# leekwoon/nav-gym

Measured on AMD Instinct MI355X. Metric: env steps/sec (whole node), 4096 envs x 1081-beam lidar, higher is better.
Workload: dtype f32

## Files before the change

include/navsim.h:

```cpp
#ifndef NAVSIM_H
#define NAVSIM_H

#include <stddef.h>
#include <stdint.h>

#ifdef __cplusplus
extern "C" {
#endif

#define NAVSIM_ABI_VERSION 7

#define NAVSIM_OK            0
#define NAVSIM_E_ARG        -1
#define NAVSIM_E_LAUNCH     -2
#define NAVSIM_E_UNSUPPORTED -3
#define NAVSIM_E_NODEVICE   -4

#define NAVSIM_PED_NONE      0
#define NAVSIM_PED_EXTERNAL  1
#define NAVSIM_PED_SFM       2

#define NAVSIM_FIELD_F32     0
#define NAVSIM_FIELD_U16T    1
#define NAVSIM_FIELD_TILE    8
// ... 159 lines not shown
#define NAVSIM_COUNTER_REGEN_SHORT     6
#define NAVSIM_COUNTER_REGEN_LATE      7

#define NAVSIM_DRAWS_PER_ARENA      464
#define NAVSIM_DRAW_KIND            0
#define NAVSIM_DRAW_OBSTACLE_NUMBER 1
#define NAVSIM_DRAW_NUM_HUMANS      2
#define NAVSIM_DRAW_SCAN_NOISE_STD  3
#define NAVSIM_DRAW_OBSTACLE_WIDTH  4
#define NAVSIM_DRAW_CORRIDOR_WIDTH  5
#define NAVSIM_DRAW_ITERATIONS      6
#define NAVSIM_DRAW_MAP             8

typedef struct navsim_step_io {
    const double* action;
    const float*  obs_prev;
    float*   obs;
    float*   achieved_goal;
    float*   desired_goal;
    double*  reward;
    uint8_t* done;
    float*   is_success;
    float*   is_crash;
    double*  distance;
    float*   final_obs;
    float*   final_goals;
    const uint8_t* reset_mask;
    uint8_t* truncated;
} navsim_step_io;

int         navsim_abi_version(void);
const char* navsim_error_string(int code);
int         navsim_default_config(navsim_config* cfg);
const char* navsim_last_hip_error(void);

size_t navsim_build_dt_workspace_bytes(int32_t n_maps, int32_t map_h, int32_t map_w);
int    navsim_build_dt(const uint8_t* occ, int32_t n_maps, int32_t map_h, int32_t map_w,
                       float* field, void* workspace, size_t workspace_bytes, void* stream);

size_t navsim_field_bytes(int32_t n_maps, int32_t map_h, int32_t map_w, int32_t format);
int    navsim_build_field(const uint8_t* occ, int32_t n_maps, int32_t map_h, int32_t map_w, int32_t format,
                          void* field, float* overflow, int32_t* n_saturated,
                          void* workspace, size_t workspace_bytes, void* stream);

size_t navsim_rect_table_bytes(int32_t n_maps, int32_t map_h, int32_t map_w);
size_t navsim_rect_index_bytes(int32_t n_maps, int32_t map_h, int32_t map_w);
int    navsim_build_rect_index(const void* table, int32_t n_maps, int32_t map_h, int32_t map_w, void* index,
                               int32_t* n_rects, void* stream);
int    navsim_maps_closed(const uint8_t* occ, int32_t n_maps, int32_t map_h, int32_t map_w, int32_t* closed, void* stream);
int    navsim_world_closed(const navsim_config* cfg, const navsim_state* st, int32_t* n_open, void* stream);
size_t navsim_build_rects_workspace_bytes(int32_t n_maps, int32_t map_h, int32_t map_w);
int    navsim_build_rects(const uint8_t* occ, int32_t n_maps, int32_t map_h, int32_t map_w, const void* field,
                          int32_t format, const float* overflow, void* table, void* workspace, size_t workspace_bytes,
                          void* stream);

int navsim_cast_static(const float* field, int32_t n_envs, int32_t map_h, int32_t map_w,
                       const float* queries, int32_t n_per_env, float max_range, int32_t march_rule,
                       float* out, void* stream);

int navsim_render_polys(float* ranges, const double* angles, int32_t n_envs, int32_t n_beams,
                        const float* verts, const int32_t* n_verts, int32_t max_verts,
                        const float* origin, void* stream);

int navsim_render_legs(float* ranges, const double* angles, int32_t n_envs, int32_t n_beams,
                       const float* agents, const int32_t* n_agents, int32_t max_agents,
                       const float* origin, void* stream);

int navsim_integrate(double* pose, const double* cmd, double* vel_out, int32_t n,
                     double time_step, double axle_offset, void* stream);

int navsim_reward_done(const navsim_config* cfg, const void* obs, const void* goals,
                       int32_t obs_is_f64, int32_t n,
                       const float* scan_threshold, const float* scan_discomfort,
                       double* reward, uint8_t* done, float* is_success, float* is_crash,
                       double* distance, void* stream);

int navsim_scan_threshold(const navsim_config* cfg, const float* footprint, int32_t n_vert,
                          float* out, void* stream);

int navsim_beam_table(const navsim_config* cfg, double* table, void* stream);

int navsim_step(const navsim_config* cfg, const navsim_state* st, const navsim_step_io* io,
                void* stream);

#define NAVSIM_STEP_ALL     0
#define NAVSIM_STEP_NOT_DUE 1
#define NAVSIM_STEP_DUE     2
int navsim_step_part(const navsim_config* cfg, const navsim_state* st, const navsim_step_io* io, int32_t part,
                     void* stream);

int navsim_ped_scans(const navsim_config* cfg, const navsim_state* st, float* out, void* stream);
int navsim_ped_scans_part(const navsim_config* cfg, const navsim_state* st, float* out, int32_t e0, int32_t n_e, void* stream);

size_t navsim_regen_workspace_bytes(const navsim_config* cfg);
int    navsim_regen_swap(const navsim_config* cfg, const navsim_state* live, const navsim_state* stage,
                         const navsim_step_io* io, const float* stage_obs, const uint8_t* want, uint8_t* mark,
                         const long long* ready, void* stream);
int    navsim_regen_stage(const navsim_config* cfg, const navsim_state* stage, const navsim_step_io* io, uint8_t* want,
                          uint8_t* mark, long long* ready, void* workspace, size_t workspace_bytes, void* stream);
int    navsim_regen_stage_part(const navsim_config* cfg, const navsim_state* stage, const navsim_step_io* io, uint8_t* want,
                               uint8_t* mark, long long* ready, void* workspace, size_t workspace_bytes, int32_t part,
                               int32_t n_parts, void* stream);
int    navsim_step_install(const navsim_config* cfg, const navsim_state* st, const navsim_step_io* io,
                           const navsim_state* stage, const float* stage_obs, uint8_t* mark, const long long* ready,
                           uint8_t* late, void* stream);
int    navsim_step_install_replan(const navsim_config* cfg, const navsim_state* st, const navsim_step_io* io,
                                  const navsim_state* stage, const float* stage_obs, uint8_t* mark, const long long* ready,
                                  uint8_t* late, int32_t max_queries, void* stream);
int    navsim_step_install_next(const navsim_config* cfg, const navsim_state* st, const navsim_step_io* io,
                                const navsim_state* stage, const float* stage_obs, uint8_t* mark, const long long* ready,
                                uint8_t* late_next, const uint8_t* late_prev, int32_t max_queries, void* stream);
int    navsim_regen_helper(void* stream);
int    navsim_regen(const navsim_config* cfg, const navsim_state* st, const navsim_step_io* io,
                    void* workspace, size_t workspace_bytes, void* stream);

int navsim_costmap(const uint8_t* occ, int32_t n_maps, int32_t map_h, int32_t map_w, uint8_t* cost, void* stream);
int    navsim_plan(const uint8_t* cost, const int32_t* map_index, int32_t n_queries, int32_t cost_h, int32_t cost_w,
                   double cost_resolution, double origin_x, double origin_y, const double* start, const double* goal,
                   double interval, int32_t max_wp, double* wp, int32_t* n_wp, int32_t* path_cells, double* path_len,
                   void* stream);

size_t navsim_replan_workspace_bytes(const navsim_config* cfg, int32_t max_queries);
int    navsim_replan(const navsim_config* cfg, const navsim_state* st, int32_t max_queries, void* workspace,
                     size_t workspace_bytes, void* stream);

typedef struct navsim_policy_weights {
    const float* cv1_w;
    const float* cv1_b;
    const float* cv2_w;
    const float* cv2_b;
    const float* fc1_w;
    const float* fc1_b;
    const float* fc2_w;
    const float* fc2_b;
    const float* a1_w;
    const float* a1_b;
    const float* a2_w;
    const float* a2_b;
} navsim_policy_weights;

size_t navsim_ped_policy_workspace_bytes(const navsim_config* cfg);
int    navsim_ped_policy(const navsim_config* cfg, const navsim_state* st, const navsim_policy_weights* w,
                         const float* ped_scans, float* prev_actions, double* ped_cmd, void* workspace,
                         size_t workspace_bytes, void* stream);
int    navsim_ped_policy_part(const navsim_config* cfg, const navsim_state* st, const navsim_policy_weights* w,
                              const float* ped_scans, float* prev_actions, double* ped_cmd, void* workspace,
                              size_t workspace_bytes, int32_t e0, int32_t n_e, void* stream);
int    navsim_ped_scan_policy(const navsim_config* cfg, const navsim_state* st, const navsim_policy_weights* w,
                              float* scans_out, float* prev_actions, double* ped_cmd, void* workspace,
                              size_t workspace_bytes, void* stream);

int navsim_launch_order(const uint32_t* cost, int32_t* order, int32_t n, void* stream);

typedef struct navsim_crowd_params {
    double time_step, discomfort_dist, map_size_m, map_resolution;
    double success_reward, collision_penalty, discomfort_penalty_factor, rotation_penalty_factor, timeout_penalty;
    double time_limit;
} navsim_crowd_params;
#define NAVSIM_CROWD_NOTHING 0
#define NAVSIM_CROWD_TIMEOUT 1
#define NAVSIM_CROWD_REACH_GOAL 2
#define NAVSIM_CROWD_COLLISION 3
#define NAVSIM_CROWD_COLLISION_OTHER 4
#define NAVSIM_CROWD_DANGER 5
int navsim_crowd_check(const navsim_crowd_params* p, int32_t n_envs, int32_t max_agents, int32_t grid,
                       const uint8_t* free_map, const double* robot, const double* agents, const int32_t* n_agents,
                       const double* global_time, double* reward, uint8_t* done, int32_t* info, double* min_dist,
                       void* stream);

#define NAVSIM_CROWD_MAX_VERTS 8
typedef struct navsim_crowd_map_params {
    double angular_min, angular_max;
    double angular_max_range;
    int32_t angular_dim;
    int32_t normalize;
    double map_size_m, map_resolution, submap_size_m;
} navsim_crowd_map_params;
int navsim_crowd_angular_map(const navsim_crowd_map_params* p, int32_t n_envs, int32_t max_obst, int32_t n_vert,
                             const double* robot, const double* verts, const int32_t* n_obst, double* out, void* stream);
int navsim_crowd_local_map(const navsim_crowd_map_params* p, int32_t n_envs, int32_t grid, const uint8_t* free_map,
                           const double* robot, int32_t rotate, uint8_t* out, void* stream);

#define NAVSIM_ORCA_MAX_AGENTS 64
#define NAVSIM_ORCA_MAX_EDGES  128
typedef struct navsim_orca_params {
    float time_step;
    float neighbor_dist;
    float time_horizon;
    float time_horizon_obst;
    int32_t max_neighbors;
} navsim_orca_params;
int navsim_crowd_orca(const navsim_orca_params* p, int32_t n_queries, int32_t max_agents, const double* agents,
                      const int32_t* n_agents, const double* pref_vel, int32_t max_obst, int32_t n_vert,
                      const double* verts, const int32_t* n_obst, const int32_t* obst_set, const double* theta,
                      double* out_vel, double* out_action, void* stream);
typedef struct navsim_ped_orca_params {
    navsim_orca_params orca;
    double ped_radius, robot_radius, safety_space;
    int32_t robot_visible;
} navsim_ped_orca_params;
int navsim_ped_orca(const navsim_config* cfg, const navsim_state* st, const navsim_ped_orca_params* p,
                    double* ped_cmd , void* stream);
int navsim_crowd_agent_step(double* pose, const double* action, double* vel, int32_t n, double time_step, void* stream);

int navsim_step_replan(const navsim_config* cfg, const navsim_state* st, const navsim_step_io* io, int32_t max_queries,
                       void* stream);

int navsim_prepare(const navsim_config* cfg, const navsim_state* st, const navsim_step_io* io);

int navsim_reset_obs(const navsim_config* cfg, const navsim_state* st, const navsim_step_io* io,
                     const uint8_t* mask, void* stream);

int navsim_restart(const navsim_config* cfg, const navsim_state* st, const uint8_t* mask, void* stream);

const char* navsim_step_kernel_name(void);

size_t navsim_sizeof_config(void);
size_t navsim_sizeof_state(void);
size_t navsim_sizeof_step_io(void);
int navsim_debug_math(int32_t fn, const double* x, const double* x2, double* out, int32_t n, void* stream);
int navsim_debug_xy_to_ij(const navsim_config* cfg, const double* xy, int32_t as_f32, int32_t* ij, int32_t n, void* stream);

int navsim_debug_spawn_decisions(const navsim_config* cfg, const uint8_t* cost, int32_t Hc, int32_t Wc, int32_t n,
                                 const int32_t* kind, const double* start, const double* goal, const double* robot,
                                 double* wp_scratch, int32_t* code, void* stream);

int navsim_debug_gather(const float* x, uint64_t n_words, int32_t mode, int32_t iters, int32_t n_threads,
                        float* out, void* stream);
int navsim_debug_set_stamps(unsigned long long* buf);
int navsim_debug_kernarg_layout(void* stream);

#ifdef __cplusplus
}
#endif
#endif
```

nav-gym_amd/csrc/kernels_step.hpp:

```cpp

struct StepShared {
    double rp[3];
    double old_rp[3];
    double act[2];
    float lx, ly, lth;
    int steps_now;
    double cT, sT;
    int i0, j0;
    int nseg, ndisc;
    int rescan;
    int respawn;
    float t1;
    float r_all;
    unsigned long long step_key;
    unsigned long long rescan_key;
    int next_chunk;
    int park_count, park_next;
    int pair_done;
    int term;
    double wave_ratio[kMaxWaves];
};
struct PedShared {
    double *ax, *ay, *avx, *avy;
    float (*seg)[4];
// ... 186 lines not shown
    (void)r_all; (void)res;
    if (culled) {
#ifndef NAVSIM_DIAG_NO_MERGE
        merge_prims_culled<BLOCK>(c, sh, pr, dir, rng_rw);
#endif
        __syncthreads();
    }
    for (int k = (int)threadIdx.x; k < B; k += BLOCK) {
        float rr = rng[k];
        if (!culled && (nseg | ndisc)) {
            float dx, dy;
            if (dir) { float2 d = dir[k]; dx = d.x; dy = d.y; }
            else beam_dir_k(c, tab, k, step, (double)sh.lth, sh.cT, sh.sT, dx, dy);
            for (int p = 0; p < nseg; ++p)
                nv::seg_merge(rr, lx, ly, dx, dy, pr.seg[p][0], pr.seg[p][1], pr.seg[p][2], pr.seg[p][3]);
            for (int p = 0; p < ndisc; ++p)
                nv::circle_merge(rr, lx, ly, dx, dy, pr.disc[p][0], pr.disc[p][1], nv::kLegRadius);
        }
        rr = rr < 0.0f ? 0.0f : rr;
        rr = rr > rmax ? rmax : rr;
        if (noise_std > 0.0f && rr != rmax)
            rr = rr + noise_std * nv::gauss_noise(nkey, (uint32_t)k);
        cr |= (rr < thr[k]);
        dc |= (rr < dthr[k]);
        obs_row[(size_t)(S - 1) * B + k] = rr;
        for (int j = 0; j < S - 1; ++j)
            if (S - 1 - j > n_hist) obs_row[(size_t)j * B + k] = rr;
    }
    crash = cr;
    discomfort = dc;
}

typedef unsigned long long lanemask_t;
__device__ __forceinline__ lanemask_t mask_of(bool p) { return __builtin_amdgcn_ballot_w64(p); }
__device__ __forceinline__ lanemask_t mask_ult(unsigned a, unsigned b) { return __builtin_amdgcn_uicmp(a, b, 36); }
__device__ __forceinline__ lanemask_t mask_eq(unsigned a, unsigned b) { return __builtin_amdgcn_uicmp(a, b, 32); }
__device__ __forceinline__ lanemask_t mask_flt(float a, float b) { return __builtin_amdgcn_fcmpf(a, b, 4); }
__device__ __forceinline__ float mask_sel(lanemask_t m, float a, float b) {
    float r;
    asm("v_cndmask_b32_e64 %0, %1, %2, %3" : "=v"(r) : "v"(b), "v"(a), "s"(m));
    return r;
}
__device__ __forceinline__ int mask_sel(lanemask_t m, int a, int b) {
    int r;
    asm("v_cndmask_b32_e64 %0, %1, %2, %3" : "=v"(r) : "v"(b), "v"(a), "s"(m));
    return r;
}
__device__ __forceinline__ bool mask_lane(lanemask_t m) { return mask_sel(m, 1, 0) != 0; }

template <typename Field, int RULE, int RECT>
__device__ __forceinline__ void probe_round(const Field& field, const char* __restrict__ rects, unsigned tpr,
                                            float x0, float y0, float dx, float dy, unsigned uW, unsigned uH,
                                            float max_range, float& t, lanemask_t& active, lanemask_t& hit) {
    typedef float f32x2 __attribute__((ext_vector_type(2)));
    const f32x2 org = {x0, y0}, dir = {dx, dy};
    f32x2 pos;
    if constexpr (RULE == NAVSIM_MARCH_F32_FMA) pos = __builtin_elementwise_fma(dir, (f32x2){t, t}, org);
    else pos = org + dir * t;
    int px = (int)pos.x, py = (int)pos.y;
    const lanemask_t live = (RECT == 2) ? active : (active & mask_ult((unsigned)px, uW) & mask_ult((unsigned)py, uH));
    lanemask_t occ;
    float d;
    if constexpr (RECT == 0) {
        px = mask_sel(live, px, 0);
        py = mask_sel(live, py, 0);
    }
    if constexpr (RECT != 0) {
        const unsigned cell = rect_cell(px, py);
        unsigned tile = __umul24((unsigned)py >> kRectShift, tpr) + ((unsigned)px >> kRectShift);
        if constexpr (RECT != 2) tile = (unsigned)mask_sel(live, (int)tile, 0);
        typedef unsigned u32x4 __attribute__((ext_vector_type(4)));
        u32x4 rec;
        lanemask_t inval;
        if constexpr (RECT == 2) {
            typedef __attribute__((address_space(3))) const unsigned char lds_u8;
            typedef unsigned u32x2 __attribute__((ext_vector_type(2)));
            typedef __attribute__((address_space(3))) const u32x2 lds_u2;
            lds_u8* row = (lds_u8*)rects;
            const unsigned ia = row[kRectListLen * 8 + tile * 2u], ib = row[kRectListLen * 8 + 1 + tile * 2u];
            const u32x2 ra = *(lds_u2*)(row + ia * 8u);
            const u32x2 rb = *(lds_u2*)(row + ib * 8u);
            rec.x = ra.x; rec.y = ra.y; rec.z = rb.x; rec.w = rb.y;
            inval = live & mask_eq(ia, 0xFFu);
        } else {
            const unsigned off = tile * (unsigned)sizeof(uint4);
            unsigned long long base;
            asm volatile("s_mov_b64 %1, %3\n\tglobal_load_dwordx4 %0, %2, %1\n\ts_waitcnt vmcnt(0)"
                         : "=&v"(rec), "=&s"(base) : "v"(off), "s"(rects) : "memory");
            inval = live & mask_eq(rec.x & 0xFFFFu, (unsigned)kRectInvalid);
        }
        const int da = rect_dist2(rec.x, rec.y, cell), db = rect_dist2(rec.z, rec.w, cell);
        const int d2 = da < db ? da : db;
        occ = live & mask_eq((unsigned)d2, 0u);
        d = Field::sqrt_d2(d2);
        if (inval != 0) {
            typename Field::raw_t raw = (typename Field::raw_t)1;
            if (mask_lane(inval)) raw = field.load(px, py);
            occ = (occ & ~inval) | (inval & mask_of(field.occupied(raw)));
            d = mask_sel(inval, field.decode_nz(raw, px, py), d);
        }
    } else {
        typename Field::raw_t raw = field.load(px, py);
        occ = live & mask_of(field.occupied(raw));
        d = field.decode_nz(raw, px, py);
    }
    hit |= occ;
    const float tn = t + march_step<RULE>(d);
    const lanemask_t go = live & ~occ;
    t = mask_sel(go, tn, t);
    active = go & mask_flt(tn, max_range);
}

constexpr int kIntRangeMaxSide = 1448;
__host__ __device__ __forceinline__ bool int_range_ok(int H, int W) { return H <= kIntRangeMaxSide && W <= kIntRangeMaxSide; }
__device__ __forceinline__ float hit_range_int(int ix, int iy) {
    return nv::sqrt_small_int((float)(__mul24(ix, ix) + __mul24(iy, iy)));
}
template <int RULE>
__device__ __forceinline__ float ray_result(lanemask_t hit, bool int_range, int i0, int j0, float x0, float y0, float dx, float dy,
                                            float t, float miss) {
    const int px = (int)march_pos<RULE>(x0, dx, t), py = (int)march_pos<RULE>(y0, dy, t);
    float r;
    if (int_range) {
        r = hit_range_int(px - i0, py - j0);
    } else {
        const float xd = (float)px - x0, yd = (float)py - y0;
        r = sqrtf(xd * xd + yd * yd);
    }
    return mask_sel(hit, r, miss);
}

#ifndef NAVSIM_PARK_LANES
#define NAVSIM_PARK_LANES 16
#endif
#ifndef NAVSIM_PAIR_SHARE_MIN_BLOCK
#define NAVSIM_PAIR_SHARE_MIN_BLOCK 512
#endif
constexpr int kParkLanesMax = NAVSIM_PARK_LANES;
#ifndef NAVSIM_PARK_LANES_PEDS
#define NAVSIM_PARK_LANES_PEDS 16
#endif
#ifdef NAVSIM_PARK_512
__host__ __device__ constexpr bool step_parks(int block, bool peds) { return (block == 256 && (!peds || NAVSIM_PARK_LANES_PEDS > 0)) || (block == 512 && !peds); }
#else
__host__ __device__ constexpr bool step_parks(int block, bool peds) { return block == 256 && (!peds || NAVSIM_PARK_LANES_PEDS > 0); }
#endif
__host__ __device__ inline size_t park_lds_bytes(int B, int park_lanes, bool peds) {
    return (((size_t)((B + 63) / 64) * park_lanes * (peds ? 2 : 16)) + 15) & ~(size_t)15;
}
__device__ __forceinline__ int lanes_below(lanemask_t m) {
    return (int)__builtin_amdgcn_mbcnt_hi((unsigned)(m >> 32), __builtin_amdgcn_mbcnt_lo((unsigned)m, 0u));
}

template <int BLOCK, typename Field, bool TO_LDS, int RULE, int RECT>
__device__ __forceinline__ void scan_beams_pred(const navsim_config& c, StepShared& sh,
                                                const Field& field, const uint4* __restrict__ rects,
                                                const double* __restrict__ tab,
                                                const Prims pr, float2* __restrict__ dir_lds, float* __restrict__ rng_lds,
                                                float4* __restrict__ park, const int park_lanes,
                                                const float* __restrict__ thr, const float* __restrict__ dthr,
                                                float* __restrict__ obs_row, int n_hist, float noise_std,
                                                uint64_t noise_key, uint64_t genv,
                                                int& crash, int& discomfort, bool prepare_prims = true) {
    const int B = c.n_beams, S = c.n_scan_stack, H = c.map_h, W = c.map_w;
    const float max_range = march_limit(H, W, c.range_max, c.resolution);
    const float res = (float)c.resolution;
    const float rmax = (float)c.range_max;
    const double step = nv::linspace_step(c);
    const int i0 = sh.i0, j0 = sh.j0;
    const float x0 = (float)i0, y0 = (float)j0;
    const bool int_range = int_range_ok(H, W);
    const float lx = sh.lx, ly = sh.ly;
    const int nseg = sh.nseg, ndisc = sh.ndisc;
    const unsigned uW = (unsigned)W, uH = (unsigned)H;
    const unsigned tpr = (unsigned)((W + 7) >> kRectShift);
    const float t1 = sh.t1, r_all = sh.r_all;
    const uint64_t nkey = (noise_std > 0.0f) ? nv::noise_stream(c.seed, genv, noise_key) : 0;
    int cr = 0, dc = 0;
    auto finish = [&](int k, float dx, float dy, float rr) {
        if (TO_LDS) {
            rng_lds[k] = rr * res;
            dir_lds[k] = make_float2(dx, dy);
            return;
        }
        rr = rr * res;
        for (int p = 0; p < nseg; ++p)
            nv::seg_merge(rr, lx, ly, dx, dy, pr.seg[p][0], pr.seg[p][1], pr.seg[p][2], pr.seg[p][3]);
        for (int p = 0; p < ndisc; ++p)
            nv::circle_merge(rr, lx, ly, dx, dy, pr.disc[p][0], pr.disc[p][1], nv::kLegRadius);
        rr = rr < 0.0f ? 0.0f : rr;
        rr = rr > rmax ? rmax : rr;
        if (noise_std > 0.0f && rr != rmax)
            rr = rr + noise_std * nv::gauss_noise(nkey, (uint32_t)k);
        cr |= (rr < thr[k]);
        dc |= (rr < dthr[k]);
        obs_row[(size_t)(S - 1) * B + k] = rr;
        for (int j = 0; j < S - 1; ++j)
            if (S - 1 - j > n_hist) obs_row[(size_t)j * B + k] = rr;
    };
    const float miss = (r_all >= 0.0f) ? r_all : max_range;
    if constexpr (TO_LDS) { if (prepare_prims) prims_prepare<BLOCK>(c, sh, pr); }
    constexpr bool kPark = step_parks(BLOCK, TO_LDS);
    int own_chunk = 0;
    const int lane = (int)threadIdx.x & 63;
    for (;;) {
        int chunk = 0;
        if (BLOCK > 64) {
            if (lane == 0) chunk = atomicAdd(&sh.next_chunk, 1);
            chunk = __builtin_amdgcn_readfirstlane(chunk);
        } else {
            chunk = own_chunk++;
        }
        if (chunk * 64 >= B) break;
        const int k = chunk * 64 + lane;
        const bool valid = k < B;
        float dx, dy;
        beam_dir_k(c, tab, valid ? k : B - 1, step, (double)sh.lth, sh.cT, sh.sT, dx, dy);
        float t = t1;
        lanemask_t active = mask_of(valid & (r_all < 0.0f));
        lanemask_t hit = 0;
        if constexpr (!kPark) {
            while (active != 0)
                probe_round<Field, RULE, RECT>(field, (const char*)rects, tpr, x0, y0, dx, dy, uW, uH, max_range, t, active, hit);
            if (valid) finish(k, dx, dy, ray_result<RULE>(hit, int_range, i0, j0, x0, y0, dx, dy, t, miss));
        } else {
            while ((int)__builtin_popcountll(active) > park_lanes)
                probe_round<Field, RULE, RECT>(field, (const char*)rects, tpr, x0, y0, dx, dy, uW, uH, max_range, t, active, hit);
            const bool marching = mask_lane(active);
            if (active != 0) {
                int base = 0;
                if (lane == 0) base = atomicAdd(&sh.park_count, (int)__builtin_popcountll(active));
                base = __builtin_amdgcn_readfirstlane(base);
                if (marching) {
                    if constexpr (TO_LDS) {
                        ((unsigned short*)park)[base + lanes_below(active)] = (unsigned short)k;
                        rng_lds[k] = t;
                        dir_lds[k] = make_float2(dx, dy);
                    } else {
                        park[base + lanes_below(active)] = make_float4(__int_as_float(k), t, dx, dy);
                    }
                }
            }
            if (valid & !marching) finish(k, dx, dy, ray_result<RULE>(hit, int_range, i0, j0, x0, y0, dx, dy, t, miss));
        }
    }
    if constexpr (kPark) __syncthreads();
    const int n_parked = kPark ? sh.park_count : 0;
    for (;;) {
        if (!kPark || n_parked == 0) break;
        int g = 0;
        if (lane == 0) g = atomicAdd(&sh.park_next, 64);
        g = __builtin_amdgcn_readfirstlane(g);
        if (g >= n_parked) break;
        const bool valid = g + lane < n_parked;
        int k;
        float t, dx, dy;
        if constexpr (TO_LDS) {
            k = (int)((const unsigned short*)park)[valid ? g + lane : g];
            t = rng_lds[k];
            const float2 d = dir_lds[k];
            dx = d.x; dy = d.y;
        } else {
            const float4 r = park[valid ? g + lane : g];
            k = __float_as_int(r.x);
            t = r.y; dx = r.z; dy = r.w;
        }
        lanemask_t active = mask_of(valid);
        lanemask_t hit = 0;
        while (active != 0)
            probe_round<Field, RULE, RECT>(field, (const char*)rects, tpr, x0, y0, dx, dy, uW, uH, max_range, t, active, hit);
        if (valid) finish(k, dx, dy, ray_result<RULE>(hit, int_range, i0, j0, x0, y0, dx, dy, t, miss));
    }
    if (TO_LDS) {
        __syncthreads();
        finish_beams<BLOCK>(c, sh, pr, tab, dir_lds, rng_lds, rng_lds, thr, dthr, obs_row, n_hist, noise_std,
                            noise_key, genv, cr, dc);
    }
    crash = cr;
    discomfort = dc;
}

__device__ __forceinline__ int ped_pop_waypoints(const double* wp, int head, int nw, const double (&pp)[3]) {
    while (head + 1 < nw) {
        double ddx = pp[0] - wp[2 * head], ddy = pp[1] - wp[2 * head + 1];
        if (sqrt(ddx * ddx + ddy * ddy) < 1.0) ++head;
        else break;
    }
    return head;
}
__device__ __forceinline__ void ped_pair_index(int t, int n, int& i, int& j) {
    const int n_pp = n * (n - 1) / 2;
    if (t < n_pp) {
        i = 0;
        int rem = t;
        while (rem >= n - 1 - i) { rem -= n - 1 - i; ++i; }
        j = i + 1 + rem;
    } else {
        i = t - n_pp; j = n;
    }
}
__device__ __forceinline__ void ped_pair_term(const navsim_config& c, const PedShared& ps, double2* pair, int n, int t) {
    int i, j;
    ped_pair_index(t, n, i, j);
    double fx, fy;
    sfm_pair(c, ps.ax[i], ps.ay[i], ps.avx[i], ps.avy[i], ps.ax[j], ps.ay[j], ps.avx[j], ps.avy[j], fx, fy);
    pair[t] = make_double2(fx, fy);
}
template <typename Field>
__device__ __forceinline__ void ped_sfm_step(const navsim_config& c, const Field& field, const PedShared& ps,
                                             const double2* pair, int n, int i, double vpref, const double* wp, double dt,
                                             double (&pp)[3], double (&pvel)[2]) {
    double ex = wp[0] - ps.ax[i], ey = wp[1] - ps.ay[i];
    double L = sqrt(ex * ex + ey * ey);
    if (L > 1e-9) { ex = ex / L; ey = ey / L; } else { ex = 0.0; ey = 0.0; }
    double fdx = (vpref * ex - ps.avx[i]) / c.sfm_tau;
    double fdy = (vpref * ey - ps.avy[i]) / c.sfm_tau;
    double fsx = 0.0, fsy = 0.0;
    {
        int slot = i - 1;
        for (int j = 0; j < i; ++j) {
            const double2 f = pair[slot];
            fsx -= f.x;
            fsy -= f.y;
            slot += n - 2 - j;
        }
        slot = i * (n - 1) - i * (i - 1) / 2;
        for (int j = i + 1; j < n; ++j, ++slot) {
            const double2 f = pair[slot];
            fsx += f.x;
            fsy += f.y;
        }
        const double2 f = pair[n * (n - 1) / 2 + i];
        fsx += f.x;
        fsy += f.y;
    }
    double fox = 0.0, foy = 0.0;
    {
        const int H = c.map_h, W = c.map_w;
        int ci, cj;
        nv::xy_to_ij(ps.ax[i], ps.ay[i], c, ci, cj);
        ci = ci > W - 1 ? W - 1 : ci;
        cj = cj > H - 1 ? H - 1 : cj;
        int il_ = ci > 0 ? ci - 1 : 0, ir = ci < W - 1 ? ci + 1 : W - 1;
        int jl = cj > 0 ? cj - 1 : 0, jr = cj < H - 1 ? cj + 1 : H - 1;
        double d = (double)field.at(ci, cj) * c.resolution;
        double gx = (double)field.at(ir, cj) - (double)field.at(il_, cj);
        double gy = (double)field.at(ci, jr) - (double)field.at(ci, jl);
        double gl = sqrt(gx * gx + gy * gy);
        if (gl > 0.0) {
            double mag = nv::exp_neg(-(d - c.sfm_agent_radius) / c.sfm_sigma_obstacle);
            fox = mag * (gx / gl);
            foy = mag * (gy / gl);
        }
    }
    double accx = c.sfm_k_desired * fdx + c.sfm_k_social * fsx + c.sfm_k_obstacle * fox;
    double accy = c.sfm_k_desired * fdy + c.sfm_k_social * fsy + c.sfm_k_obstacle * foy;
    double vx = ps.avx[i] + accx * dt;
    double vy = ps.avy[i] + accy * dt;
    double sp = sqrt(vx * vx + vy * vy);
    if (sp > vpref) {
        double k = (sp > 0.0) ? vpref / sp : 0.0;
        vx = vx * k; vy = vy * k;
    }
    pp[0] = pp[0] + vx * dt;
    pp[1] = pp[1] + vy * dt;
    double sp2 = sqrt(vx * vx + vy * vy);
    if (sp2 > 1e-6) pp[2] = nv::mod_2pi(nv::atan2_(vy, vx));
    pvel[0] = vx; pvel[1] = vy;
}
__device__ __forceinline__ bool ped_finish(const navsim_config& c, const navsim_state& st, int e, int i, size_t pq, double* wp,
                                           int head, int nw, double dt, uint64_t genv, uint64_t steps_now, const double (&pp)[3],
                                           const double (&pvel)[2]) {
    double ddx = pp[0] - wp[2 * (nw - 1)], ddy = pp[1] - wp[2 * (nw - 1) + 1];
    const bool at_final = sqrt(ddx * ddx + ddy * ddy) < 0.5;
    if (at_final && c.n_spawn > 0 && st.spawn_pose && !st.costmap) {
        uint64_t h = nv::hash4(c.seed, genv, (uint64_t)i + 1000, steps_now);
        for (int tries = 0; tries < c.n_spawn; ++tries) {
            int idx = (int)((h + (uint64_t)tries) % (uint64_t)c.n_spawn);
            const double* cand = st.spawn_pose + ((size_t)e * c.n_spawn + idx) * 3;
            double gx = cand[0] - pp[0], gy = cand[1] - pp[1];
            if (sqrt(gx * gx + gy * gy) > 10.0) {
                wp[0] = cand[0]; wp[1] = cand[1]; head = 0;
                st.ped_n_waypoints[pq] = 1;
                if (st.ped_goal) { st.ped_goal[pq * 2] = cand[0]; st.ped_goal[pq * 2 + 1] = cand[1]; }
                break;
            }
        }
    }
    st.ped_wp_head[pq] = head;
    double dist[3] = {st.ped_dist[pq * 3], st.ped_dist[pq * 3 + 1], st.ped_dist[pq * 3 + 2]};
    nv::leg_odometry(pp, pvel, st.ped_prev_yaw[pq], dt, dist);
    st.ped_dist[pq * 3] = dist[0]; st.ped_dist[pq * 3 + 1] = dist[1]; st.ped_dist[pq * 3 + 2] = dist[2];
    st.ped_prev_yaw[pq] = nv::wrap_pi(pp[2]);
    st.ped_pose[pq * 3] = pp[0]; st.ped_pose[pq * 3 + 1] = pp[1]; st.ped_pose[pq * 3 + 2] = pp[2];
    st.ped_vel[pq * 2] = pvel[0]; st.ped_vel[pq * 2 + 1] = pvel[1];
    return at_final;
}

__device__ __forceinline__ void wave_lds_sync() {
    __builtin_amdgcn_fence(__ATOMIC_RELEASE, "workgroup");
    __builtin_amdgcn_wave_barrier();
    __builtin_amdgcn_fence(__ATOMIC_ACQUIRE, "workgroup");
}

__device__ __forceinline__ int ped_stage_wave(const navsim_config& c, const navsim_state& st, int n, int lane, bool is_ped,
                                              size_t pq, const double* rp_t, double prev_v, const PedShared& ps,
                                              const double (&pp)[3], const double (&pvel)[2], int& nw) {
    const int P = c.max_waypoints;
    const double* wp = st.ped_waypoints + (pq * P) * 2;
    int head = 0;
    nw = 1;
    if (is_ped) {
        nw = st.ped_n_waypoints[pq];
        head = ped_pop_waypoints(wp, st.ped_wp_head[pq], nw, pp);
    }
    if (c.ped_model == NAVSIM_PED_SFM) {
        if (is_ped) { ps.ax[lane] = pp[0]; ps.ay[lane] = pp[1]; ps.avx[lane] = pvel[0]; ps.avy[lane] = pvel[1]; }
        if (lane == 0) {
            double s, cs;
            nv::sincos(rp_t[2], s, cs);
            ps.ax[n] = rp_t[0]; ps.ay[n] = rp_t[1];
            ps.avx[n] = prev_v * cs; ps.avy[n] = prev_v * s;
        }
    }
// ... 145 lines not shown
            if (w == 0ull) continue;
            if (pos++ == slot) { e_s = e; before_s = pos_p; break; }
            pos_p += __popcll(w);
        }
    __syncthreads();
    const int e = e_s;
    if (peds_before) *peds_before = before_s;
    if (n_peds) *n_peds = all_p;
    __syncthreads();
    return e;
}

template <int BLOCK>
__device__ __forceinline__ int due_arena_rank(const unsigned long long* __restrict__ due, int e, int* peds_before) {
    __shared__ int wave_a[kMaxWaves], wave_p[kMaxWaves];
    const int tid = threadIdx.x, lane = tid & 63, nthr = block_threads<BLOCK>();
    int n = 0, m = 0;
    for (int k = tid; k < e; k += nthr) { const unsigned long long w = due[k]; n += w != 0ull; m += __popcll(w); }
    for (int off = 32; off > 0; off >>= 1) { n += __shfl_down(n, off, 64); m += __shfl_down(m, off, 64); }
    if (lane == 0) { wave_a[tid >> 6] = n; wave_p[tid >> 6] = m; }
    __syncthreads();
    int rank = 0, before = 0;
    for (int w = 0; w < (nthr + 63) / 64; ++w) { rank += wave_a[w]; before += wave_p[w]; }
    *peds_before = before;
    __syncthreads();
    return rank;
}

#ifndef NAVSIM_INSTALL_UNROLL
#define NAVSIM_INSTALL_UNROLL 8
#endif
struct StepInstallBig { char* dst; const char* src; size_t bytes; };
struct StepInstall {
    navsim_state stage;
    const float* stage_obs;
    uint8_t* mark;
    const long long* ready;
    uint8_t* late_next;
    const uint8_t* late_prev;
    int lone;
    uint8_t* late;
    StepInstallBig big[5];
};
__device__ __forceinline__ void stage_request(int64_t* stage_episode, uint8_t* mark, int e, int64_t ep) {
    __hip_atomic_store(&stage_episode[e], ep, __ATOMIC_RELAXED, __HIP_MEMORY_SCOPE_AGENT);
    __threadfence();
    atomicOr((unsigned*)(mark + (e & ~3)), 1u << (8 * (e & 3)));
}
__device__ __forceinline__ long long stage_ready(const long long* ready, int e) {
    return __hip_atomic_load(&ready[e], __ATOMIC_ACQUIRE, __HIP_MEMORY_SCOPE_AGENT);
}
__device__ __forceinline__ void install_publish(const StepInstall& in, const navsim_state& live, int e) {
    __syncthreads();
    if (threadIdx.x == 0) {
        __threadfence();
        stage_request(in.stage.episode, in.mark, e, live.episode[e] + 1);
    }
}
template <int BLOCK>
__device__ __forceinline__ void install_arena(const navsim_config& c, const navsim_state& live, const navsim_step_io& io,
                                              const StepInstall& in, const int e, float* __restrict__ obs_row) {
    const int tid = threadIdx.x;
    const bool by_slot = live.map_slot && in.stage.map_slot;
    if (by_slot && tid == 0) {
        const int32_t a = live.map_slot[e], b = in.stage.map_slot[e];
        live.map_slot[e] = b; in.stage.map_slot[e] = a;
    }
    for (int k = 0; k < 5 && !by_slot; ++k) {
        if (!in.big[k].dst) continue;
        const size_t bytes = in.big[k].bytes;
        const char* src = in.big[k].src + (size_t)e * bytes;
        char* dst = in.big[k].dst + (size_t)e * bytes;
        if ((((size_t)(uintptr_t)src | (size_t)(uintptr_t)dst | bytes) & 15) == 0) {
            const size_t n16 = bytes / 16;
            size_t i = tid;
#ifndef NAVSIM_DIAG_INSTALL_NO_BIG
            constexpr int U = NAVSIM_INSTALL_UNROLL;
            for (; i + (U - 1) * BLOCK < n16; i += U * BLOCK) {
                typedef unsigned int u32x4 __attribute__((ext_vector_type(4)));
                u32x4 v[U];
#pragma unroll
                for (int u = 0; u < U; ++u) v[u] = __builtin_nontemporal_load((const u32x4*)src + i + u * BLOCK);
#pragma unroll
                for (int u = 0; u < U; ++u) ((u32x4*)dst)[i + u * BLOCK] = v[u];
            }
            for (; i < n16; i += BLOCK) ((uint4*)dst)[i] = ((const uint4*)src)[i];
#endif
        } else {
            for (size_t i = tid; i < bytes; i += BLOCK) dst[i] = src[i];
        }
    }
    const navsim_state& stage = in.stage;
    const int N = c.max_peds, K = c.n_spawn, P = c.max_waypoints, D = c.n_scan_stack * c.n_beams + NAVSIM_OBS_TAIL;
    const bool peds = c.ped_model != NAVSIM_PED_NONE;
#define NAVSIM_ROW_LOAD(name, dstp, srcp, cnt) \
    const size_t n_##name = ((dstp) && (srcp)) ? (size_t)(cnt) : 0; \
    auto v_##name = (srcp)[tid < (int)n_##name ? (size_t)e * n_##name + tid : 0];
#define NAVSIM_ROW_STORE(name, dstp, srcp) \
    if (tid < (int)n_##name) (dstp)[(size_t)e * n_##name + tid] = v_##name; \
    for (size_t i = (size_t)tid + BLOCK; i < n_##name; i += BLOCK) (dstp)[(size_t)e * n_##name + i] = (srcp)[(size_t)e * n_##name + i];
#define NAVSIM_ROW_SRC(p) ((p) ? (p) : (decltype(p))live.steps)
    NAVSIM_ROW_LOAD(noise, live.scan_noise_std, NAVSIM_ROW_SRC(stage.scan_noise_std), 1)
    NAVSIM_ROW_LOAD(pose, live.robot_pose, NAVSIM_ROW_SRC(stage.robot_pose), 3)
    NAVSIM_ROW_LOAD(goal, live.robot_goal, NAVSIM_ROW_SRC(stage.robot_goal), 2)
    NAVSIM_ROW_LOAD(pact, live.prev_action, NAVSIM_ROW_SRC(stage.prev_action), 2)
    NAVSIM_ROW_LOAD(ppose, live.prev_pose, NAVSIM_ROW_SRC(stage.prev_pose), 3)
    NAVSIM_ROW_LOAD(nhist, live.n_hist, NAVSIM_ROW_SRC(stage.n_hist), 1)
    NAVSIM_ROW_LOAD(steps, live.steps, NAVSIM_ROW_SRC(stage.steps), 1)
    NAVSIM_ROW_LOAD(spose, live.spawn_pose, NAVSIM_ROW_SRC(stage.spawn_pose), (size_t)K * 3)
    NAVSIM_ROW_LOAD(sgoal, live.spawn_goal, NAVSIM_ROW_SRC(stage.spawn_goal), (size_t)K * 2)
    NAVSIM_ROW_LOAD(npeds, peds ? live.n_peds : nullptr, NAVSIM_ROW_SRC(stage.n_peds), 1)
    NAVSIM_ROW_LOAD(ppos, peds ? live.ped_pose : nullptr, NAVSIM_ROW_SRC(stage.ped_pose), (size_t)N * 3)
    NAVSIM_ROW_LOAD(pvel, peds ? live.ped_vel : nullptr, NAVSIM_ROW_SRC(stage.ped_vel), (size_t)N * 2)
    NAVSIM_ROW_LOAD(pyaw, peds ? live.ped_prev_yaw : nullptr, NAVSIM_ROW_SRC(stage.ped_prev_yaw), N)
    NAVSIM_ROW_LOAD(pdist, peds ? live.ped_dist : nullptr, NAVSIM_ROW_SRC(stage.ped_dist), (size_t)N * 3)
    NAVSIM_ROW_LOAD(pvpref, peds ? (double*)live.ped_v_pref : nullptr, NAVSIM_ROW_SRC(stage.ped_v_pref), N)
    NAVSIM_ROW_LOAD(plegs, peds ? (uint8_t*)live.ped_has_legs : nullptr, NAVSIM_ROW_SRC(stage.ped_has_legs), N)
    NAVSIM_ROW_LOAD(pwp, peds ? live.ped_waypoints : nullptr, NAVSIM_ROW_SRC(stage.ped_waypoints), (size_t)N * P * 2)
    NAVSIM_ROW_LOAD(pnwp, peds ? live.ped_n_waypoints : nullptr, NAVSIM_ROW_SRC(stage.ped_n_waypoints), N)
    NAVSIM_ROW_LOAD(phead, peds ? live.ped_wp_head : nullptr, NAVSIM_ROW_SRC(stage.ped_wp_head), N)
    NAVSIM_ROW_LOAD(pgoal, peds ? live.ped_goal : nullptr, NAVSIM_ROW_SRC(stage.ped_goal), (size_t)N * 2)
    NAVSIM_ROW_LOAD(obs, obs_row - (size_t)e * D, in.stage_obs, D)
    NAVSIM_ROW_STORE(noise, live.scan_noise_std, stage.scan_noise_std)
    NAVSIM_ROW_STORE(pose, live.robot_pose, stage.robot_pose)
    NAVSIM_ROW_STORE(goal, live.robot_goal, stage.robot_goal)
    NAVSIM_ROW_STORE(pact, live.prev_action, stage.prev_action)
    NAVSIM_ROW_STORE(ppose, live.prev_pose, stage.prev_pose)
    NAVSIM_ROW_STORE(nhist, live.n_hist, stage.n_hist)
    NAVSIM_ROW_STORE(steps, live.steps, stage.steps)
    NAVSIM_ROW_STORE(spose, (double*)live.spawn_pose, stage.spawn_pose)
    NAVSIM_ROW_STORE(sgoal, (double*)live.spawn_goal, stage.spawn_goal)
    NAVSIM_ROW_STORE(npeds, live.n_peds, stage.n_peds)
    NAVSIM_ROW_STORE(ppos, live.ped_pose, stage.ped_pose)
    NAVSIM_ROW_STORE(pvel, live.ped_vel, stage.ped_vel)
    NAVSIM_ROW_STORE(pyaw, live.ped_prev_yaw, stage.ped_prev_yaw)
    NAVSIM_ROW_STORE(pdist, live.ped_dist, stage.ped_dist)
    NAVSIM_ROW_STORE(pvpref, (double*)live.ped_v_pref, stage.ped_v_pref)
    NAVSIM_ROW_STORE(plegs, (uint8_t*)live.ped_has_legs, stage.ped_has_legs)
    NAVSIM_ROW_STORE(pwp, live.ped_waypoints, stage.ped_waypoints)
    NAVSIM_ROW_STORE(pnwp, live.ped_n_waypoints, stage.ped_n_waypoints)
    NAVSIM_ROW_STORE(phead, live.ped_wp_head, stage.ped_wp_head)
    NAVSIM_ROW_STORE(pgoal, live.ped_goal, stage.ped_goal)
    NAVSIM_ROW_STORE(obs, obs_row - (size_t)e * D, in.stage_obs)
#undef NAVSIM_ROW_LOAD
#undef NAVSIM_ROW_STORE
#undef NAVSIM_ROW_SRC
    if (tid == 0) {
        if (io.achieved_goal) { io.achieved_goal[2 * e] = (float)stage.robot_pose[3 * (size_t)e]; io.achieved_goal[2 * e + 1] = (float)stage.robot_pose[3 * (size_t)e + 1]; }
        if (io.desired_goal) { io.desired_goal[2 * e] = (float)stage.robot_goal[2 * (size_t)e]; io.desired_goal[2 * e + 1] = (float)stage.robot_goal[2 * (size_t)e + 1]; }
        if (live.ped_due) live.ped_due[e] = 0ull;
    }
}

template <int BLOCK, bool PEDS, typename Field, int RULE, int RECT, bool PINL, bool INSTALL = false, bool FEAT = true>
__device__ __forceinline__ void step_arena(const navsim_config& c, const navsim_state& st, const navsim_step_io& io, const int e,
                                           int reset_only, const int peds_done, const uint8_t* __restrict__ reset_mask,
                                           unsigned dyn_lds_bytes, int park_lanes, unsigned rect_lds_offset,
                                           const StepInstall* in = nullptr, const int base_prio = 0) {
    __shared__ StepShared sh;
    extern __shared__ __attribute__((aligned(16))) char dyn_lds_all[];
    char* dyn_lds = dyn_lds_all + (RECT == 2 ? rect_lds_offset : 0u);
    PedShared ps = {};
    if constexpr (PEDS) ps = ped_lds_carve(dyn_lds + ((dyn_lds_bytes + 15u) & ~15u), c.max_peds);
    const Prims prims = {ps.seg, ps.disc, ps.info};
    const int tid = threadIdx.x;
    constexpr int kMarchPrio = (BLOCK == 256 && !PEDS) ? 2 : 0;
    __builtin_amdgcn_s_setprio(3);
    unsigned long long t_begin = 0;
    if (st.arena_cost && tid == 0) t_begin = __builtin_amdgcn_s_memrealtime();
    const int B = c.n_beams, S = c.n_scan_stack, N = c.max_peds, D = S * B + 7;
    const double dt = c.time_step;
    const uint64_t genv = (uint64_t)(c.env_index_base + e);
    const int ms = INSTALL ? map_slot_of(c, st, e) : (c.shared_field ? 0 : e);
    const Field field(st.field, st.field_overflow, ms, c.map_h, c.map_w);
    const uint4* rects = RECT ? (const uint4*)st.rect_table + (size_t)ms * rect_tiles_per_map(c.map_h, c.map_w)
                              : nullptr;
    if constexpr (RECT == 2) {
        const size_t row_bytes = rect_index_row_bytes(c.map_h, c.map_w);
        const uint4* src = (const uint4*)((const char*)st.rect_index + (size_t)ms * row_bytes);
        uint4* tab_lds = (uint4*)dyn_lds_all;
        for (int i = threadIdx.x; i < (int)(row_bytes / 16); i += BLOCK) tab_lds[i] = src[i];
        rects = tab_lds;
    }
    float* obs_row = io.obs + (size_t)e * D;
    const float* obs_prev = io.obs_prev ? io.obs_prev + (size_t)e * D : nullptr;
    double* rp_g = st.robot_pose + 3 * (size_t)e;
    double* goal_g = st.robot_goal + 2 * (size_t)e;
    double* pa_g = st.prev_action + 2 * (size_t)e;
    double* pv_g = st.prev_pose + 3 * (size_t)e;

    constexpr bool kFeat = PEDS || FEAT;
    const bool pending = kFeat && !reset_only && io.reset_mask && io.reset_mask[e] != 0;
    if (pending) {
        reset_only = 1;
        if (tid == 0) {
            io.reward[e] = 0.0; io.done[e] = 0; io.is_success[e] = 0.0f; io.is_crash[e] = 0.0f; io.distance[e] = 0.0;
            if (c.max_episode_steps > 0 && io.truncated) io.truncated[e] = 0;
            if (st.ped_due) st.ped_due[e] = 0ull;
        }
        if (c.defer_reset_scan) return;
        if constexpr (INSTALL && BLOCK >= 256 && RULE == NAVSIM_MARCH_F32) {
            if (in->lone && in->ready) {
                if (tid == 0) {
                    const bool lng = c.regen_min_steps <= 0 || st.done_steps[e] >= c.regen_min_steps;
                    const bool rdy = stage_ready(in->ready, e) == (long long)st.episode[e];
                    sh.respawn = lng ? (rdy ? 3 : 5) : 0;
                    if (!(lng && rdy)) stage_request(in->stage.episode, in->mark, e, st.episode[e] + 1);
                    if (st.counters) {
                        atomicAdd(&st.counters[lng ? (rdy ? NAVSIM_COUNTER_REGEN_SERVED : NAVSIM_COUNTER_REGEN_LATE) : NAVSIM_COUNTER_REGEN_SHORT], 1ull);
                        if (lng && !rdy) atomicAdd(&st.counters[NAVSIM_COUNTER_REGEN_SERVED], 1ull);
                    }
                }
                __syncthreads();
                const int verdict = sh.respawn;
                __syncthreads();
                if (verdict == 3) {
                    install_arena<BLOCK>(c, st, io, *in, e, obs_row);
                    install_publish(*in, st, e);
                    return;
                }
                if (verdict == 5) {
                    regen_lone<Field, BLOCK>(c, st, e);
                    if constexpr (RECT == 2) {
                        const size_t row_bytes = rect_index_row_bytes(c.map_h, c.map_w);
                        const uint4* src = (const uint4*)((const char*)st.rect_index + (size_t)ms * row_bytes);
                        uint4* tab_lds = (uint4*)dyn_lds_all;
                        for (int i = threadIdx.x; i < (int)(row_bytes / 16); i += BLOCK) tab_lds[i] = src[i];
                    }
                }
            }
        }
    }
    if (reset_only && reset_mask && !reset_mask[e]) {
        if (obs_prev && obs_prev != obs_row)
            for (int k = tid; k < D; k += BLOCK) obs_row[k] = obs_prev[k];
        return;
    }

    int n = (!PEDS || c.ped_model == NAVSIM_PED_NONE) ? 0 : st.n_peds[e];
    n = n > N ? N : n;
    const float noise_std = (c.add_scan_noise && st.scan_noise_std) ? st.scan_noise_std[e] : 0.0f;

    NAVSIM_STAMP(0);
    double pp[3] = {0.0, 0.0, 0.0};
    double pvel[2] = {0.0, 0.0};
    const bool is_ped = PEDS && tid < n;
    const size_t pq = (size_t)e * N + (is_ped ? tid : 0);
    const bool ped_advance = PEDS && PINL && !reset_only && !peds_done;
    int ped_head = 0, ped_nw = 1;
    if constexpr (PEDS) {
        if (tid < 64) {
            if (is_ped) {
                pp[0] = st.ped_pose[pq * 3]; pp[1] = st.ped_pose[pq * 3 + 1]; pp[2] = st.ped_pose[pq * 3 + 2];
                pvel[0] = st.ped_vel[pq * 2]; pvel[1] = st.ped_vel[pq * 2 + 1];
            }
            if constexpr (PINL) {
                if (ped_advance) ped_head = ped_stage_wave(c, st, n, tid, is_ped, pq, rp_g, pa_g[0], ps, pp, pvel, ped_nw);
            }
        }
    }
    constexpr int kPhase0Thread = (PEDS && BLOCK > 64) ? 64 : 0;
    const int l0 = tid - kPhase0Thread;
    if (l0 >= 0 && l0 < 3) {
        const double th_old = rp_g[2];
        double a0 = 0.0, a1 = 0.0;
        if (!reset_only) {
            a0 = io.action[2 * e]; a1 = io.action[2 * e + 1];
            if (c.action_kind == NAVSIM_ACTION_WHEELS) {
                const double wl = a0, wr = a1;
                a0 = c.wheel_radius * (wl + wr) * 0.5;
                a1 = c.wheel_radius * (wr - wl) / c.wheel_track;
            }
            if (c.clamp_action) {
                a0 = a0 < c.linvel_lo ? c.linvel_lo : (a0 > c.linvel_hi ? c.linvel_hi : a0);
                a1 = a1 < c.rotvel_lo ? c.rotvel_lo : (a1 > c.rotvel_hi ? c.rotvel_hi : a1);
            }
            if (c.min_turning_radius > 0.0) {
                double lim = fabs(a1) * c.min_turning_radius;
                if (a0 >= 0.0) a0 = (a0 > lim) ? a0 : lim;
                else           a0 = (a0 < -lim) ? a0 : -lim;
            }
        }
        const double th = th_old + a1 * dt;
        const double th_new = reset_only ? th_old : nv::mod_2pi(th);
        const float lth = (float)th_new;
        const double ang = (l0 == 0) ? th_old : ((l0 == 1) ? th : (double)lth);
        double sn, cs;
        nv::sincos(ang, sn, cs);
        const int w0 = kPhase0Thread & 63;
        const double s0 = __shfl(sn, w0), c0 = __shfl(cs, w0), s1 = __shfl(sn, w0 + 1), c1 = __shfl(cs, w0 + 1);
        const double sT = __shfl(sn, w0 + 2), cT = __shfl(cs, w0 + 2);
        if (l0 == 0) {
            sh.old_rp[0] = rp_g[0]; sh.old_rp[1] = rp_g[1]; sh.old_rp[2] = th_old;
            sh.nseg = 0; sh.ndisc = 0; sh.rescan = 0; sh.respawn = 0; sh.term = 0;
            if constexpr (INSTALL) {
                if (pending && !in->lone) {
                    if (in->late) in->late[e] = 0;
                    if (in->late_next) in->late_next[e] = 0;
                    if (in->late_prev && in->late_prev[e]) {
                        sh.respawn = 4;
                        stage_request(in->stage.episode, in->mark, e, st.episode[e] + 1);
                        if (st.counters) atomicAdd(&st.counters[NAVSIM_COUNTER_REGEN_LATE], 1ull);
                    } else if (in->ready) {
                        const bool lng = c.regen_min_steps <= 0 || st.done_steps[e] >= c.regen_min_steps;
                        const bool rdy = stage_ready(in->ready, e) == (long long)st.episode[e];
                        if (lng && rdy) sh.respawn = 3;
                        else {
                            if (lng && in->late) in->late[e] = 1;
                            stage_request(in->stage.episode, in->mark, e, st.episode[e] + 1);
                        }
                        if (st.counters)
                            atomicAdd(&st.counters[lng ? (rdy ? NAVSIM_COUNTER_REGEN_SERVED : NAVSIM_COUNTER_REGEN_LATE) : NAVSIM_COUNTER_REGEN_SHORT], 1ull);
                    }
                }
            }
            if (!reset_only) {
                const int64_t steps_now = st.steps[e] + 1;
                st.steps[e] = steps_now;
                sh.steps_now = (int)steps_now;
                sh.act[0] = a0; sh.act[1] = a1;
                double p[3] = {sh.old_rp[0], sh.old_rp[1], sh.old_rp[2]};
                nv::set_vel_with(p, a0, a1, dt, c.axle_offset, s0, c0, s1, c1, nullptr);
                sh.rp[0] = p[0]; sh.rp[1] = p[1]; sh.rp[2] = p[2];
            } else {
                sh.rp[0] = sh.old_rp[0]; sh.rp[1] = sh.old_rp[1]; sh.rp[2] = sh.old_rp[2];
            }
            sh.lx = (float)sh.rp[0]; sh.ly = (float)sh.rp[1]; sh.lth = (float)sh.rp[2];
            nv::xy_to_ij_f32(sh.lx, sh.ly, c, sh.i0, sh.j0);
            sh.sT = sT; sh.cT = cT;
            first_probe<RULE>(field, sh.i0, sh.j0, (float)((long long)c.map_h * c.map_w), sh.t1, sh.r_all);
            sh.step_key = (unsigned long long)st.episode[e] * 0x100000000ULL +
                          (unsigned long long)(reset_only ? 0 : st.steps[e]) * 2ULL;
            sh.rescan_key = sh.step_key + 1;
            sh.next_chunk = 0; sh.park_count = 0; sh.park_next = 0; sh.pair_done = 0;
        }
    }
    __syncthreads();
    if constexpr (INSTALL) {
        if (pending && sh.respawn == 3) {
            install_arena<BLOCK>(c, st, io, *in, e, obs_row);
            install_publish(*in, st, e);
            return;
        }
        if (pending && sh.respawn == 4) return;
    }

    NAVSIM_STAMP(1);
    if constexpr (PEDS) {
        double2* pair = (double2*)(dyn_lds + ((dyn_lds_bytes + 15u) & ~15u) + ((ped_lds_bytes(N) + 15) & ~(size_t)15));
#ifdef NAVSIM_PAIR_SHARE_ALL
        constexpr int kPairWaves = (BLOCK >= NAVSIM_PAIR_SHARE_MIN_BLOCK) ? 4 : 1;
#else
        constexpr int kPairWaves = (INSTALL && BLOCK >= NAVSIM_PAIR_SHARE_MIN_BLOCK) ? 4 : 1;
#endif
        const bool pair_shared = PINL && kPairWaves > 1 && ped_advance && c.ped_model == NAVSIM_PED_SFM;
        if constexpr (PINL && kPairWaves > 1) {
            if (pair_shared && tid < kPairWaves * 64) ped_pair_share(c, ps, pair, n, tid, kPairWaves, &sh.pair_done);
        }
        if (tid < 64) {
            const int lane = tid;
            if constexpr (PINL) {
                if (ped_advance)
                    ped_advance_wave<Field>(c, st, field, e, n, lane, is_ped, pq, dt, genv, (uint64_t)st.steps[e], ps, pair,
                                            ped_head, ped_nw, pp, pvel, &sh.pair_done, pair_shared ? kPairWaves : 1);
            }
            if (reset_only && is_ped) {
                st.ped_dist[pq * 3] = 0.0; st.ped_dist[pq * 3 + 1] = 0.0; st.ped_dist[pq * 3 + 2] = 0.0;
                st.ped_prev_yaw[pq] = nv::wrap_pi(pp[2]);
            }
            if (is_ped) {
                float dist3[3];
                if (reset_only) { dist3[0] = dist3[1] = dist3[2] = 0.0f; }
                else { dist3[0] = (float)st.ped_dist[pq * 3]; dist3[1] = (float)st.ped_dist[pq * 3 + 1];
                       dist3[2] = (float)st.ped_dist[pq * 3 + 2]; }
                if (st.ped_has_legs[pq] && c.lidar_legs) {
                    float cc[4];
                    nv::leg_centres((float)pp[0], (float)pp[1], (float)pp[2], dist3[0], dist3[1], dist3[2], cc);
                    int q = atomicAdd(&sh.ndisc, 2);
                    ps.disc[q][0] = cc[0]; ps.disc[q][1] = cc[1];
                    ps.disc[q + 1][0] = cc[2]; ps.disc[q + 1][1] = cc[3];
                } else {
                    const double fpx[4] = {0.22, -0.22, -0.22, 0.22};
                    const double fpy[4] = {0.19, 0.19, -0.19, -0.19};
                    double s, cs;
                    nv::sincos(pp[2], s, cs);
                    float vx[4], vy[4];
#pragma unroll
                    for (int v = 0; v < 4; ++v) {
                        vx[v] = (float)((cs * fpx[v] - s * fpy[v]) + pp[0]);
                        vy[v] = (float)((s * fpx[v] + cs * fpy[v]) + pp[1]);
                    }
                    int q = atomicAdd(&sh.nseg, 4);
#pragma unroll
                    for (int v = 0; v < 4; ++v) {
                        int w = (v + 1) & 3;
                        ps.seg[q + v][0] = vx[v]; ps.seg[q + v][1] = vy[v];
                        ps.seg[q + v][2] = vx[w]; ps.seg[q + v][3] = vy[w];
                    }
                }
            }
            wave_lds_sync();
            prims_prepare<64>(c, sh, prims);
        }
    }

    NAVSIM_STAMP(2);
    if (kMarchPrio == 2 || base_prio == 2) __builtin_amdgcn_s_setprio(2);
    else if (base_prio == 1) __builtin_amdgcn_s_setprio(1);
    else __builtin_amdgcn_s_setprio(0);
    int n_hist = reset_only ? 0 : st.n_hist[e];
    int crash = 0, discomfort = 0;
    const uint64_t step_key = sh.step_key;
    float4* park = (float4*)dyn_lds;
    char* scan_lds = dyn_lds + park_lds_bytes(B, park_lanes, PEDS);
    float2* dir_lds = (float2*)scan_lds;
    float* rng_lds = (float*)(scan_lds + sizeof(float2) * (size_t)B);
    scan_beams_pred<BLOCK, Field, PEDS, RULE, RECT>(c, sh, field, rects, st.beam_table, prims, dir_lds, rng_lds, park, park_lanes, st.scan_threshold,
                                                         st.scan_discomfort, obs_row, n_hist, noise_std, step_key, genv, crash, discomfort, false);

    NAVSIM_STAMP(3);
    bool restart_next = false;
    if (!reset_only) {
        crash = __syncthreads_or(crash);
        discomfort = __syncthreads_or(discomfort);
        double rmin = 1.0e300;
        if (discomfort && !crash) {
            for (int k = tid; k < B; k += BLOCK)
            {
                double ratio = nv::discomfort_ratio((double)obs_row[(size_t)(S - 1) * B + k],
                                                    st.scan_threshold[k], st.scan_discomfort[k]);
                rmin = ratio < rmin ? ratio : rmin;
            }
            rmin = wave_min_f64(rmin);
            if ((tid & 63) == 0) sh.wave_ratio[tid >> 6] = rmin;
            __syncthreads();
        }
        NAVSIM_STAMP(4);
        if (tid == 0) {
            if (discomfort && !crash)
                for (int w = 1; w < (BLOCK + 63) / 64; ++w) rmin = sh.wave_ratio[w] < rmin ? sh.wave_ratio[w] : rmin;
            double prev_xy[2] = {pv_g[0], pv_g[1]};
            double pose[2] = {sh.rp[0], sh.rp[1]};
            double vel[2] = {pa_g[0], pa_g[1]};
            double goal[2] = {goal_g[0], goal_g[1]};
            nv::RewardOut o = nv::reward_scalar(c, prev_xy, pose, vel, goal, crash != 0, discomfort != 0, rmin);
            if constexpr (kFeat) {
                if (c.max_episode_steps > 0) {
                    const bool trunc = !o.done && sh.steps_now >= c.max_episode_steps;
                    if (io.truncated) io.truncated[e] = (uint8_t)trunc;
                    if (trunc) o.done = 1;
                }
            }
            io.reward[e] = o.reward;
            io.done[e] = (uint8_t)o.done;
            if constexpr (INSTALL) { if (in->late) in->late[e] = 0; if (in->late_next) in->late_next[e] = 0; }
            io.is_success[e] = o.success;
            io.is_crash[e] = o.crash;
            io.distance[e] = o.distance;
            const bool restart = o.done && c.auto_reset != NAVSIM_AUTORESET_NONE && c.n_spawn > 0;
            if (restart && c.auto_reset == NAVSIM_AUTORESET_SAME_STEP) {
                if (kFeat && io.final_obs) {
                    const bool crashed = o.crash != 0.0f;
                    const double tx = crashed ? pv_g[0] : sh.rp[0], ty = crashed ? pv_g[1] : sh.rp[1];
                    const double tyaw = nv::wrap_pi(crashed ? pv_g[2] : sh.rp[2]);
                    float* ft = io.final_obs + (size_t)e * D + (size_t)S * B;
                    ft[0] = (float)pv_g[0]; ft[1] = (float)pv_g[1];
                    ft[2] = (float)tx; ft[3] = (float)ty;
                    ft[4] = (float)pa_g[0]; ft[5] = (float)pa_g[1];
                    ft[6] = (float)tyaw;
                    if (io.final_goals) {
                        float* fg = io.final_goals + 4 * (size_t)e;
                        fg[0] = (float)tx; fg[1] = (float)ty; fg[2] = (float)goal_g[0]; fg[3] = (float)goal_g[1];
                    }
                    sh.term = crashed ? 2 : 1;
                }
                uint64_t h = nv::hash4(c.seed, genv, (uint64_t)st.episode[e], 0x5eedULL);
                int idx = (int)(h % (uint64_t)c.n_spawn);
                const double* sp = st.spawn_pose + ((size_t)e * c.n_spawn + idx) * 3;
                const double* sg = st.spawn_goal + ((size_t)e * c.n_spawn + idx) * 2;
                sh.rp[0] = sp[0]; sh.rp[1] = sp[1]; sh.rp[2] = sp[2];
                goal_g[0] = sg[0]; goal_g[1] = sg[1];
#ifndef NAVSIM_DIAG_NO_DONE_STEPS
                if (st.done_steps) st.done_steps[e] = sh.steps_now;
#endif
                st.episode[e] += 1;
                st.steps[e] = 0;
                sh.rescan_key = (unsigned long long)st.episode[e] * 0x100000000ULL;
                sh.respawn = 1; sh.rescan = c.defer_reset_scan ? 0 : 1;
                if constexpr (INSTALL) if (in->ready) {
                    const bool lng = c.regen_min_steps <= 0 || st.done_steps[e] >= c.regen_min_steps;
                    const bool rdy = stage_ready(in->ready, e) == (long long)st.episode[e];
                    if (lng && rdy) { sh.respawn = 3; sh.rescan = 0; }
                    else if (lng && in->late) in->late[e] = 1;
                    if (st.counters)
                        atomicAdd(&st.counters[lng ? (rdy ? NAVSIM_COUNTER_REGEN_SERVED : NAVSIM_COUNTER_REGEN_LATE) : NAVSIM_COUNTER_REGEN_SHORT], 1ull);
                    if (!(lng && rdy)) stage_request(in->stage.episode, in->mark, e, st.episode[e] + 1);
                }
            } else {
                restart_next = kFeat && restart;
                if (o.crash != 0.0f) {
                    sh.rp[0] = pv_g[0]; sh.rp[1] = pv_g[1]; sh.rp[2] = pv_g[2];
                    sh.rescan = 1;
                }
            }
#ifdef NAVSIM_DIAG_NO_RESCAN
            sh.rescan = 0;
#endif
            if constexpr (!kFeat) {
                if (sh.rescan) {
                    sh.next_chunk = 0; sh.park_count = 0; sh.park_next = 0;
                    sh.lx = (float)sh.rp[0]; sh.ly = (float)sh.rp[1]; sh.lth = (float)sh.rp[2];
                    nv::xy_to_ij_f32(sh.lx, sh.ly, c, sh.i0, sh.j0);
                    nv::sincos((double)sh.lth, sh.sT, sh.cT);
                    first_probe<RULE>(field, sh.i0, sh.j0, (float)((long long)c.map_h * c.map_w), sh.t1, sh.r_all);
                }
            }
        }
        __syncthreads();
        if constexpr (!kFeat) {
            if (sh.rescan) {
                if (sh.respawn) n_hist = 0;
                int c2, d2;
                scan_beams_pred<BLOCK, Field, PEDS, RULE, RECT>(c, sh, field, rects, st.beam_table, prims, dir_lds, rng_lds, park, park_lanes, st.scan_threshold,
                                                                     st.scan_discomfort, obs_row, n_hist, noise_std, sh.rescan_key, genv, c2, d2);
            }
        } else {
            float* final_row = io.final_obs ? io.final_obs + (size_t)e * D : nullptr;
            const int term = sh.term;
            if (term == 1) {
                for (int j = 0; j < S; ++j) {
                    const bool old = j < S - 1 && S - 1 - j <= n_hist;
                    for (int k = tid; k < B; k += BLOCK)
                        final_row[(size_t)j * B + k] = old ? obs_prev[(size_t)(j + 1) * B + k] : obs_row[(size_t)(S - 1) * B + k];
                }
                __syncthreads();
            }
            for (int pass = (term == 2) ? 0 : 1; pass < 2; ++pass) {
                if (pass == 1 && !sh.rescan) break;
                if (tid == 0) {
                    const double* at = (pass == 0) ? pv_g : sh.rp;
                    sh.next_chunk = 0; sh.park_count = 0; sh.park_next = 0;
                    sh.lx = (float)at[0]; sh.ly = (float)at[1]; sh.lth = (float)at[2];
                    nv::xy_to_ij_f32(sh.lx, sh.ly, c, sh.i0, sh.j0);
                    nv::sincos((double)sh.lth, sh.sT, sh.cT);
                    first_probe<RULE>(field, sh.i0, sh.j0, (float)((long long)c.map_h * c.map_w), sh.t1, sh.r_all);
                }
                __syncthreads();
                if (pass == 1 && sh.respawn) n_hist = 0;
                int c2, d2;
                scan_beams_pred<BLOCK, Field, PEDS, RULE, RECT>(c, sh, field, rects, st.beam_table, prims, dir_lds, rng_lds, park, park_lanes, st.scan_threshold,
                                                                     st.scan_discomfort, pass == 0 ? final_row : obs_row, n_hist, noise_std,
                                                                     pass == 0 ? step_key + 1 : sh.rescan_key, genv, c2, d2);
                if (pass == 0) {
                    for (int j = 0; j < S - 1; ++j)
                        if (S - 1 - j <= n_hist)
                            for (int k = tid; k < B; k += BLOCK) final_row[(size_t)j * B + k] = obs_prev[(size_t)(j + 1) * B + k];
                    __syncthreads();
                }
            }
        }
    }

    NAVSIM_STAMP(5);
    if (kMarchPrio != 0 && base_prio < kMarchPrio) {
        if (base_prio == 1) __builtin_amdgcn_s_setprio(1);
        else __builtin_amdgcn_s_setprio(0);
    }
    const bool fresh = reset_only || sh.respawn;
    if (!fresh && obs_prev) {
        for (int j = 0; j < S - 1; ++j)
            if (S - 1 - j <= n_hist)
                for (int k = tid; k < B; k += BLOCK) obs_row[(size_t)j * B + k] = obs_prev[(size_t)(j + 1) * B + k];
    }
    if (tid == 0) {
        float* tail = obs_row + (size_t)S * B;
        double yaw = nv::wrap_pi(sh.rp[2]);
        double pxy0 = fresh ? sh.rp[0] : pv_g[0];
        double pxy1 = fresh ? sh.rp[1] : pv_g[1];
        double v0 = fresh ? 0.0 : pa_g[0], v1 = fresh ? 0.0 : pa_g[1];
        tail[0] = (float)pxy0; tail[1] = (float)pxy1;
        tail[2] = (float)sh.rp[0]; tail[3] = (float)sh.rp[1];
        tail[4] = (float)v0; tail[5] = (float)v1;
        tail[6] = (float)yaw;
        if (io.achieved_goal) { io.achieved_goal[2 * e] = (float)sh.rp[0]; io.achieved_goal[2 * e + 1] = (float)sh.rp[1]; }
        if (io.desired_goal) { io.desired_goal[2 * e] = (float)goal_g[0]; io.desired_goal[2 * e + 1] = (float)goal_g[1]; }
        rp_g[0] = sh.rp[0]; rp_g[1] = sh.rp[1]; rp_g[2] = sh.rp[2];
        if (fresh) { pa_g[0] = 0.0; pa_g[1] = 0.0; st.n_hist[e] = (S - 1 < 1) ? S - 1 : 1; }
        else       { pa_g[0] = sh.act[0]; pa_g[1] = sh.act[1]; st.n_hist[e] = (n_hist + 1 < S - 1) ? n_hist + 1 : S - 1; }
        if (reset_only) st.steps[e] = 0;
        pv_g[0] = sh.rp[0]; pv_g[1] = sh.rp[1]; pv_g[2] = yaw;
        if (restart_next) {
            uint64_t h = nv::hash4(c.seed, genv, (uint64_t)st.episode[e], 0x5eedULL);
            int idx = (int)(h % (uint64_t)c.n_spawn);
            const double* sp = st.spawn_pose + ((size_t)e * c.n_spawn + idx) * 3;
            const double* sg = st.spawn_goal + ((size_t)e * c.n_spawn + idx) * 2;
            rp_g[0] = sp[0]; rp_g[1] = sp[1]; rp_g[2] = sp[2];
            goal_g[0] = sg[0]; goal_g[1] = sg[1];
            if (st.done_steps) st.done_steps[e] = sh.steps_now;
            st.episode[e] += 1;
            st.steps[e] = 0;
            if constexpr (INSTALL) {
                if (in->late_next && in->ready) {
                    const bool lng = c.regen_min_steps <= 0 || sh.steps_now >= c.regen_min_steps;
                    const bool rdy = stage_ready(in->ready, e) == (long long)st.episode[e];
                    in->late_next[e] = (lng && !rdy) ? 1 : 0;
                }
            }
        }
        if (st.arena_cost && !reset_only)
            st.arena_cost[e] = (uint32_t)(__builtin_amdgcn_s_memrealtime() - t_begin);
    }
    NAVSIM_STAMP(6);
    if constexpr (INSTALL) {
        __syncthreads();
        if (sh.respawn == 3) {
            install_arena<BLOCK>(c, st, io, *in, e, obs_row);
            install_publish(*in, st, e);
        }
        NAVSIM_STAMP(7);
    }
}

#ifndef NAVSIM_KARG_VIEW
#define NAVSIM_KARG_VIEW 1
#endif
struct StepKernargs { navsim_config c; navsim_state st; navsim_step_io io; };
struct StepInstallKernargs { navsim_config c; navsim_state st; navsim_step_io io; StepInstall in; };
#if NAVSIM_KARG_VIEW
#define NAVSIM_KERNARGS(View, ...) const View& ka = *(const View*)__builtin_amdgcn_kernarg_segment_ptr()
#else
#define NAVSIM_KERNARGS(View, ...) const View ka = {__VA_ARGS__}
#endif
constexpr int kStepWordResetOnly = 1, kStepWordPedsDoneBit = 1, kStepWordPartShift = 2, kStepWordPartMask = 3;
constexpr int kStepPartReplan = 3;
template <int BLOCK, bool PEDS, typename Field, int RULE, int RECT, bool PINL, bool FEAT = true>
#ifndef NAVSIM_PEDS_WAVES_MIN
#define NAVSIM_PEDS_WAVES_MIN 5
#endif
#ifndef NAVSIM_NOPEDS_WAVES_MIN
#define NAVSIM_NOPEDS_WAVES_MIN 8
#endif
__global__ __launch_bounds__(BLOCK) __attribute__((amdgpu_waves_per_eu((PEDS && PINL && RECT == 2 && BLOCK == 256) ? NAVSIM_PEDS_WAVES_MIN : (!PEDS ? NAVSIM_NOPEDS_WAVES_MIN : 8), 8)))
void navsim_step_kernel(navsim_config c_, navsim_state st_,
                                                            navsim_step_io io_, int reset_only,
                                                            const uint8_t* __restrict__ reset_mask,
                                                            unsigned dyn_lds_bytes, int park_lanes, unsigned rect_lds_offset) {
    NAVSIM_KERNARGS(StepKernargs, c_, st_, io_);
    const navsim_config& c = ka.c; const navsim_state& st = ka.st; const navsim_step_io& io = ka.io;
    const int peds_done = (reset_only >> kStepWordPedsDoneBit) & 1;
    const int part = (reset_only >> kStepWordPartShift) & kStepWordPartMask;
    reset_only &= kStepWordResetOnly;
    const int e = st.launch_order ? st.launch_order[blockIdx.x] : (int)blockIdx.x;
    if (e < 0) return;
    if (part == NAVSIM_STEP_NOT_DUE && st.ped_due_prev[e] != 0ull) return;
    step_arena<BLOCK, PEDS, Field, RULE, RECT, PINL, false, FEAT>(c, st, io, e, reset_only, peds_done, reset_mask, dyn_lds_bytes, park_lanes, rect_lds_offset);
}

template <int BLOCK, bool PEDS, typename Field, int RULE, int RECT>
__global__ __launch_bounds__(BLOCK) __attribute__((amdgpu_waves_per_eu((PEDS && RECT == 2 && BLOCK == 256) ? NAVSIM_PEDS_WAVES_MIN : (!PEDS ? NAVSIM_NOPEDS_WAVES_MIN : 8), 8)))
void navsim_step_install_kernel(navsim_config c_, navsim_state st_, navsim_step_io io_, StepInstall in_, int reset_only,
                                const uint8_t* __restrict__ reset_mask,
                                unsigned dyn_lds_bytes, int park_lanes, unsigned rect_lds_offset) {
    NAVSIM_KERNARGS(StepInstallKernargs, c_, st_, io_, in_);
    const navsim_config& c = ka.c; const navsim_state& st = ka.st; const navsim_step_io& io = ka.io; const StepInstall& in = ka.in;
    const int e = st.launch_order ? st.launch_order[blockIdx.x] : (int)blockIdx.x;
    if (e < 0) return;
    step_arena<BLOCK, PEDS, Field, RULE, RECT, PEDS, true>(c, st, io, e, reset_only & kStepWordResetOnly, 0, reset_mask, dyn_lds_bytes, park_lanes, rect_lds_offset, &in);
}

template <int BLOCK, typename Field, int RULE, int RECT>
__global__ __launch_bounds__(BLOCK) __attribute__((amdgpu_waves_per_eu(8, 8))) void navsim_step_due_kernel(navsim_config c_, navsim_state st_,
                                                            navsim_step_io io_, unsigned dyn_lds_bytes, int park_lanes,
                                                            unsigned rect_lds_offset) {
    NAVSIM_KERNARGS(StepKernargs, c_, st_, io_);
    const navsim_config& c = ka.c; const navsim_state& st = ka.st; const navsim_step_io& io = ka.io;
    __builtin_amdgcn_s_setprio(2);
    for (int slot = (int)blockIdx.x;; slot += (int)gridDim.x) {
        const int e = due_arena_pick<BLOCK>(st.ped_due_prev, c.n_envs, slot);
        if (e < 0) return;
        step_arena<BLOCK, true, Field, RULE, RECT, true>(c, st, io, e, 0, 0, nullptr, dyn_lds_bytes, park_lanes, rect_lds_offset, nullptr, 2);
        __syncthreads();
    }
}

template <int BLOCK>
__device__ __forceinline__ bool step_replan_pick(const navsim_config& c, const navsim_state& st, int G, int cap, int& e, bool& plan, int& before) {
    before = 0;
    plan = false;
    if ((int)blockIdx.x < G) {
        int n_peds;
        e = due_arena_pick<BLOCK>(st.ped_due_prev, c.n_envs, (int)blockIdx.x, &before, &n_peds);
        if (blockIdx.x == 0 && threadIdx.x == 0 && st.counters && n_peds > 0) {
            const int served = n_peds < cap ? n_peds : cap;
            if (served > 0) atomicAdd(&st.counters[NAVSIM_COUNTER_REPLAN_SERVED], (unsigned long long)served);
            if (n_peds > served) atomicAdd(&st.counters[NAVSIM_COUNTER_REPLAN_UNSERVED], (unsigned long long)(n_peds - served));
        }
        if (e < 0) return false;
        plan = true;
    } else {
        const int b = (int)blockIdx.x - G;
        e = st.launch_order ? st.launch_order[b] : b;
        if (e < 0) return false;
        if (st.ped_due_prev[e] != 0ull) {
            if (due_arena_rank<BLOCK>(st.ped_due_prev, e, &before) < G) return false;
            plan = true;
        }
    }
    return true;
}
template <int BLOCK, typename Field, int RULE, int RECT>
__global__ __launch_bounds__(BLOCK) __attribute__((amdgpu_waves_per_eu((RECT == 2 && BLOCK == 256) ? NAVSIM_PEDS_WAVES_MIN : 8, 8)))
void navsim_step_replan_kernel(navsim_config c_, navsim_state st_, navsim_step_io io_, unsigned dyn_lds_bytes, int park_lanes,
                               unsigned rect_lds_offset, int G, int cap) {
    NAVSIM_KERNARGS(StepKernargs, c_, st_, io_);
    const navsim_config& c = ka.c; const navsim_state& st = ka.st; const navsim_step_io& io = ka.io;
    int e, before;
    bool plan;
    if (!step_replan_pick<BLOCK>(c, st, G, cap, e, plan, before)) return;
    if (plan) {
        for (unsigned long long m = st.ped_due_prev[e]; m != 0ull; m &= m - 1ull, ++before) {
            if (before < cap) replan_one<BLOCK, 1>(c, st, e, (int)__builtin_ctzll(m));
            __syncthreads();
        }
    }
    step_arena<BLOCK, true, Field, RULE, RECT, true>(c, st, io, e, 0, 0, nullptr, dyn_lds_bytes, park_lanes, rect_lds_offset);
}
template <int BLOCK, typename Field, int RULE, int RECT>
__global__ __launch_bounds__(BLOCK) __attribute__((amdgpu_waves_per_eu((RECT == 2 && BLOCK == 256) ? NAVSIM_PEDS_WAVES_MIN : 8, 8)))
void navsim_step_replan_install_kernel(navsim_config c_, navsim_state st_, navsim_step_io io_, StepInstall in_, unsigned dyn_lds_bytes,
                                       int park_lanes, unsigned rect_lds_offset, int G, int cap) {
    NAVSIM_KERNARGS(StepInstallKernargs, c_, st_, io_, in_);
    const navsim_config& c = ka.c; const navsim_state& st = ka.st; const navsim_step_io& io = ka.io; const StepInstall& in = ka.in;
    int e, before;
    bool plan;
    if (!step_replan_pick<BLOCK>(c, st, G, cap, e, plan, before)) return;
    if (plan) {
        for (unsigned long long m = st.ped_due_prev[e]; m != 0ull; m &= m - 1ull, ++before) {
            if (before < cap) replan_one<BLOCK, 1>(c, st, e, (int)__builtin_ctzll(m));
            __syncthreads();
        }
    }
    step_arena<BLOCK, true, Field, RULE, RECT, true, true>(c, st, io, e, 0, 0, nullptr, dyn_lds_bytes, park_lanes, rect_lds_offset, &in);
}

__global__ __launch_bounds__(1024) void launch_order_kernel(const uint32_t* __restrict__ cost, int32_t* __restrict__ order,
                                                            int n) {
    __shared__ unsigned hist[1024], base[1024], wave_tot[16];
    __shared__ unsigned max_s;
    __shared__ unsigned long long sum_s;
    const int tid = threadIdx.x;
    hist[tid] = 0;
    if (tid == 0) { max_s = 1; sum_s = 0; }
    __syncthreads();
    unsigned mx = 0;
    unsigned long long sm = 0;
    for (int e = tid; e < n; e += 1024) { mx = cost[e] > mx ? cost[e] : mx; sm += cost[e]; }
    atomicMax(&max_s, mx);
    atomicAdd(&sum_s, sm);
    __syncthreads();
    unsigned long long m = max_s;
    const unsigned long long cap = 4ull * (sum_s / (unsigned long long)n) + 1ull;
    m = m < cap ? m : cap;
    const float scale = 1023.0f / (float)m;
    auto bucket = [&](unsigned cst) {
        const unsigned long long cc = cst < m ? cst : m;
        const int b = (int)((float)cc * scale);
        return 1023 - (b > 1023 ? 1023 : b);
    };
    for (int e = tid; e < n; e += 1024) atomicAdd(&hist[bucket(cost[e])], 1u);
    __syncthreads();
    const unsigned mine = hist[tid];
    unsigned incl = mine;
    const int lane = tid & 63;
    for (int off = 1; off < 64; off <<= 1) {
        const unsigned v = __shfl_up(incl, off, 64);
        if (lane >= off) incl += v;
    }
    if (lane == 63) wave_tot[tid >> 6] = incl;
    __syncthreads();
    if (tid < 64) {
        const unsigned t = tid < 16 ? wave_tot[tid] : 0u;
        unsigned ti = t;
        for (int off = 1; off < 16; off <<= 1) {
            const unsigned v = __shfl_up(ti, off, 64);
            if (tid >= off) ti += v;
        }
        if (tid < 16) wave_tot[tid] = ti - t;
    }
    __syncthreads();
    base[tid] = wave_tot[tid >> 6] + incl - mine;
    __syncthreads();
    for (int e = tid; e < n; e += 1024) order[atomicAdd(&base[bucket(cost[e])], 1u)] = e;
}
```

nav-gym_amd/csrc/navsim_kernels.hip:

```cpp
#include "preamble.hpp"

namespace {

#include "kernels_field.hpp"
#include "kernels_rect.hpp"
#include "kernels_plan.hpp"
#include "kernels_regen_dev.hpp"
#include "kernels_step.hpp"
#include "kernels_reset.hpp"
#include "kernels_policy.hpp"
#include "kernels_pedscan.hpp"
#include "kernels_crowd_maps.hpp"
#include "kernels_crowd_orca.hpp"
#include "kernels_ped_orca.hpp"

}
#include "step_plan.hpp"

#define NAVSIM_STEP_FAMILY(B, P) \
    extern "C" int navsim_step_launch_##B##_##P(const navsim_config*, const navsim_state*, const navsim_step_io*, \
                                                const StepLaunch*, const StepPlan*); \
    extern "C" int navsim_step_set_stamps_##B##_##P(unsigned long long*);
NAVSIM_STEP_FAMILY(64, 0) NAVSIM_STEP_FAMILY(64, 1) NAVSIM_STEP_FAMILY(256, 0) NAVSIM_STEP_FAMILY(256, 1)
NAVSIM_STEP_FAMILY(512, 0) NAVSIM_STEP_FAMILY(512, 1) NAVSIM_STEP_FAMILY(1024, 0) NAVSIM_STEP_FAMILY(1024, 1)
#undef NAVSIM_STEP_FAMILY

#ifndef NAVSIM_PLAN_MANY_SEARCHES
#define NAVSIM_PLAN_MANY_SEARCHES 4096
#endif

namespace {

__global__ void kernarg_layout_probe_kernel(navsim_config c_, navsim_state st_, navsim_step_io io_, StepInstall in_, int tail, int* out) {
    const StepInstallKernargs& ka = *(const StepInstallKernargs*)__builtin_amdgcn_kernarg_segment_ptr();
    if (threadIdx.x != 0) return;
    auto same = [](const void* a, const void* b, size_t n) {
        const unsigned char* x = (const unsigned char*)a;
        const unsigned char* y = (const unsigned char*)b;
        for (size_t i = 0; i < n; ++i) if (x[i] != y[i]) return false;
        return true;
    };
    const int tail_view = *(const int*)((const char*)&ka + sizeof(StepInstallKernargs));
    *out = (same(&c_, &ka.c, sizeof(c_)) && same(&st_, &ka.st, sizeof(st_)) && same(&io_, &ka.io, sizeof(io_)) &&
            same(&in_, &ka.in, sizeof(in_)) && tail_view == tail && tail == 0x1234567) ? 1 : 0;
}

int dispatch_step(const navsim_config* c, const navsim_state* st, const navsim_step_io* io, StepLaunch l) {
    const StepPlan p = plan_step(c, st, l.part == NAVSIM_STEP_DUE || l.part == kStepPartReplan ? 0 : l.grid);
    const bool peds = c->ped_model != NAVSIM_PED_NONE;
    const bool split = peds && !l.reset_only && ped_split_on(c);
    const StepInstall no_install = {};
    if (st->map_slot && !l.install) {
        if (l.part != NAVSIM_STEP_ALL || c->field_format != NAVSIM_FIELD_U16T || split)
            return NAVSIM_E_UNSUPPORTED;
        l.install = &no_install;
    }
    if (split && !l.prepare_only) {
        const size_t pl = ped_update_lds_bytes(c);
        const int G = ped_pack(c->max_peds), pgrid = (c->n_envs + G - 1) / G;
        if (c->field_format == NAVSIM_FIELD_U16T) ped_update_kernel<FieldU16T><<<pgrid, kPedUpdateBlock, pl, l.stream>>>(*c, *st);
        else                                      ped_update_kernel<FieldF32><<<pgrid, kPedUpdateBlock, pl, l.stream>>>(*c, *st);
        l.peds_done = true;
    }
    int rc;
#define NAVSIM_STEP_CASE(B) \
    case B: rc = peds ? navsim_step_launch_##B##_1(c, st, io, &l, &p) : navsim_step_launch_##B##_0(c, st, io, &l, &p); break;
    switch (p.block) {
        NAVSIM_STEP_CASE(64) NAVSIM_STEP_CASE(256) NAVSIM_STEP_CASE(512) NAVSIM_STEP_CASE(1024)
        default:   return NAVSIM_E_UNSUPPORTED;
    }
#undef NAVSIM_STEP_CASE
    return rc != NAVSIM_OK ? rc : launch_status();
}

int compact_grid(const navsim_config* c) {
    const int g = c->n_envs / 16 < 32 ? 32 : (c->n_envs / 16 > 1024 ? 1024 : c->n_envs / 16);
    return g > c->n_envs ? c->n_envs : g;
}

int replan_in_step(const navsim_config* c, const navsim_state* st, bool strict) {
    if (c->ped_model == NAVSIM_PED_NONE || !st->costmap) return NAVSIM_E_ARG;
    if (strict && (!st->ped_due_prev || !st->ped_due || st->ped_due == st->ped_due_prev)) return NAVSIM_E_ARG;
    if (ped_split_on(c)) return NAVSIM_E_UNSUPPORTED;
    const int Hc = c->map_h / 5, Wc = c->map_w / 5;
    if (!plan_fits(Hc, Wc) || (strict && (Hc < 1 || Wc < 1 || plan_lds(Hc, Wc) > 64 * 1024))) return NAVSIM_E_UNSUPPORTED;
    return (int)plan_words(Hc, Wc) > plan_step(c, st).block ? NAVSIM_E_UNSUPPORTED : NAVSIM_OK;
}

int check_step_args(const navsim_config* c, const navsim_state* st, const navsim_step_io* io, int reset_only) {
    if (!c || !st || !io) return NAVSIM_E_ARG;
    if (c->n_envs < 0 || c->n_beams < 1 || c->n_scan_stack < 1 || c->map_h < 1 || c->map_w < 1) return NAVSIM_E_ARG;
    if (c->max_peds > NAVSIM_MAX_PEDS) return NAVSIM_E_UNSUPPORTED;
    if (c->field_format != NAVSIM_FIELD_F32 && c->field_format != NAVSIM_FIELD_U16T) return NAVSIM_E_UNSUPPORTED;
    if (c->march_rule < NAVSIM_MARCH_F64 || c->march_rule > NAVSIM_MARCH_F32_FMA) return NAVSIM_E_ARG;
    if (c->action_kind != NAVSIM_ACTION_TWIST && c->action_kind != NAVSIM_ACTION_WHEELS) return NAVSIM_E_ARG;
    if (c->action_kind == NAVSIM_ACTION_WHEELS && !(c->wheel_track > 0.0)) return NAVSIM_E_ARG;
    if (c->defer_reset_scan != 0 && c->defer_reset_scan != 1) return NAVSIM_E_ARG;
    if (c->auto_reset < NAVSIM_AUTORESET_NONE || c->auto_reset > NAVSIM_AUTORESET_NEXT_STEP) return NAVSIM_E_ARG;
    if (io->final_goals && !io->final_obs) return NAVSIM_E_ARG;
    if (io->reset_mask && !reset_only) {
        if (io->reset_mask == io->done) return NAVSIM_E_ARG;
        if (c->ped_model != NAVSIM_PED_NONE && ped_split_on(c)) return NAVSIM_E_UNSUPPORTED;
    }
    if (c->regen_min_steps < 0 || c->max_episode_steps < 0) return NAVSIM_E_ARG;
    if (st->map_slot && c->shared_field) return NAVSIM_E_ARG;
    if (c->ped_model != NAVSIM_PED_NONE && (c->max_waypoints < 1 || c->max_waypoints > NAVSIM_MAX_WAYPOINTS)) return NAVSIM_E_ARG;
    if (st->rect_table && (c->field_format != NAVSIM_FIELD_U16T || c->map_h > 1024 || c->map_w > 1024)) return NAVSIM_E_UNSUPPORTED;
    if (st->rect_index && !st->rect_table) return NAVSIM_E_ARG;
    if (c->step_block != 0 && c->step_block != 64 && c->step_block != 256 && c->step_block != 512 &&
        c->step_block != 1024) return NAVSIM_E_ARG;
    if (c->ped_split < 0 || c->ped_split > 2 || c->rect_lds < 0 || c->rect_lds > 2) return NAVSIM_E_ARG;
    if (c->ped_model != NAVSIM_PED_NONE && c->max_peds < 1) return NAVSIM_E_ARG;
    if (plan_step(c, st).lds > kLdsPerCu) return NAVSIM_E_UNSUPPORTED;
    if (c->regen_cap > 0 && plan_step(c, st, c->regen_cap).lds > kLdsPerCu) return NAVSIM_E_UNSUPPORTED;
    if (!st->field || !st->scan_threshold || !st->scan_discomfort || !st->robot_pose || !st->robot_goal ||
        !st->prev_action || !st->prev_pose || !st->n_hist || !st->episode || !st->steps || !io->obs)
        return NAVSIM_E_ARG;
    if (!reset_only && (!io->action || !io->reward || !io->done || !io->is_success || !io->is_crash ||
                        !io->distance))
        return NAVSIM_E_ARG;
    if (!reset_only && c->n_scan_stack > 1 && !io->obs_prev) return NAVSIM_E_ARG;
    if (c->ped_model != NAVSIM_PED_NONE) {
        if (!st->n_peds || !st->ped_pose || !st->ped_vel || !st->ped_prev_yaw || !st->ped_dist ||
            !st->ped_has_legs || !st->ped_waypoints || !st->ped_n_waypoints || !st->ped_wp_head)
            return NAVSIM_E_ARG;
        if (c->ped_model == NAVSIM_PED_EXTERNAL && !st->ped_cmd && !reset_only) return NAVSIM_E_ARG;
        if (c->ped_model == NAVSIM_PED_SFM && !st->ped_v_pref) return NAVSIM_E_ARG;
    }
    if (c->auto_reset && c->n_spawn > 0 && (!st->spawn_pose || !st->spawn_goal)) return NAVSIM_E_ARG;
    return NAVSIM_OK;
}

int check_stage_pair(const navsim_config* c, const navsim_state* live, const navsim_state* stage) {
    if (c->regen_cap < 1 || c->n_spawn < 1 || !c->auto_reset) return NAVSIM_E_ARG;
    if (c->defer_reset_scan) return NAVSIM_E_UNSUPPORTED;
    if (!live->field || !stage->field || !live->episode || !stage->episode || !live->spawn_pose || !stage->spawn_pose ||
        !live->spawn_goal || !stage->spawn_goal || !stage->robot_pose || !stage->robot_goal)
        return NAVSIM_E_ARG;
    if ((live->field_overflow != nullptr) != (stage->field_overflow != nullptr) ||
        (live->rect_table != nullptr) != (stage->rect_table != nullptr) || (live->rect_index != nullptr) != (stage->rect_index != nullptr) ||
        (live->costmap != nullptr) != (stage->costmap != nullptr) || (live->ped_goal != nullptr) != (stage->ped_goal != nullptr))
        return NAVSIM_E_ARG;
    return NAVSIM_OK;
}
int check_map_slots(const navsim_state* live, const navsim_state* stage) {
    if ((live->map_slot != nullptr) != (stage->map_slot != nullptr)) return NAVSIM_E_ARG;
    if (live->map_slot && (live->map_slot == stage->map_slot || live->field != stage->field || live->field_overflow != stage->field_overflow ||
                           live->rect_table != stage->rect_table || live->rect_index != stage->rect_index || live->costmap != stage->costmap))
        return NAVSIM_E_ARG;
    return NAVSIM_OK;
}
template <typename Big>
void stage_big_buffers(const navsim_config* c, const navsim_state* live, const navsim_state* stage, Big big[5]) {
    const int H = c->map_h, W = c->map_w;
    big[0] = {(char*)live->field, (const char*)stage->field, navsim_field_bytes(1, H, W, c->field_format)};
    if (live->field_overflow) big[1] = {(char*)live->field_overflow, (const char*)stage->field_overflow, (size_t)H * W * sizeof(float)};
    if (live->rect_table) big[2] = {(char*)live->rect_table, (const char*)stage->rect_table, navsim_rect_table_bytes(1, H, W)};
    if (live->costmap) big[3] = {(char*)live->costmap, (const char*)stage->costmap, (size_t)(H / 5) * (W / 5)};
    if (live->rect_index) big[4] = {(char*)live->rect_index, (const char*)stage->rect_index, rect_index_row_bytes(H, W)};
}

int step_install_impl(const navsim_config* c, const navsim_state* st, const navsim_step_io* io, const navsim_state* stage,
                      const float* stage_obs, uint8_t* mark, const long long* ready, uint8_t* late, uint8_t* late_next,
                      const uint8_t* late_prev, int32_t max_queries, void* stream) {
    (void)hipGetLastError();
    int rc = check_step_args(c, st, io, 0);
    if (rc != NAVSIM_OK) return rc;
    if (!stage || !stage_obs || !mark || !ready || ((uintptr_t)mark & 3) != 0 || !st->done_steps) return NAVSIM_E_ARG;
    const bool lone = c->auto_reset == NAVSIM_AUTORESET_NEXT_STEP && !late && !late_next && c->regen_min_steps < 1;
    if (lone && (c->regen_indoor_ratio > 0.0 || c->regen_plan || st->costmap || plan_step(c, st).block < 256 || c->map_h != c->map_w ||
                 march_rule_variant(c) != NAVSIM_MARCH_F32 ||
                 c->obstacle_number > 64 || c->obstacle_number_hi > 64))
        return NAVSIM_E_UNSUPPORTED;
    if (c->regen_min_steps < 1 && !late && !late_next && !lone) return NAVSIM_E_ARG;
    rc = check_stage_pair(c, st, stage);
    if (rc != NAVSIM_OK) return rc;
    if (c->regen_cap < c->n_envs) return NAVSIM_E_UNSUPPORTED;
    if (c->field_format != NAVSIM_FIELD_U16T || (c->ped_model != NAVSIM_PED_NONE && ped_split_on(c))) return NAVSIM_E_UNSUPPORTED;
    if (c->n_envs == 0) return NAVSIM_OK;
    rc = check_map_slots(st, stage);
    if (rc != NAVSIM_OK) return rc;
    StepInstall in = {};
    in.stage = *stage; in.stage_obs = stage_obs; in.mark = mark; in.ready = ready; in.late = late;
    in.late_next = late_next; in.late_prev = late_prev; in.lone = lone ? 1 : 0;
    if (!st->map_slot) stage_big_buffers(c, st, stage, in.big);
    StepLaunch l;
    l.install = &in;
    l.stream = (hipStream_t)stream;
    if (max_queries >= 0) {
        rc = replan_in_step(c, st, true);
        if (rc != NAVSIM_OK) return rc;
        l.part = kStepPartReplan;
        l.grid = compact_grid(c);
        l.max_queries = max_queries;
    }
    return dispatch_step(c, st, io, l);
}

struct RegenFork { int device = -1; hipStream_t side = nullptr; hipEvent_t forked = nullptr, joined = nullptr; };
thread_local hipStream_t g_regen_helper = nullptr;
RegenFork* regen_fork() {
    thread_local RegenFork f;
    int dev = 0;
    if (hipGetDevice(&dev) != hipSuccess) return nullptr;
    if (f.device == dev && g_regen_helper && f.side != g_regen_helper) f.side = g_regen_helper;
    if (f.device != dev) {
        RegenFork n;
        if (g_regen_helper) n.side = g_regen_helper;
        else if (hipStreamCreateWithFlags(&n.side, hipStreamNonBlocking) != hipSuccess) return nullptr;
        if (hipEventCreateWithFlags(&n.forked, hipEventDisableTiming) != hipSuccess ||
            hipEventCreateWithFlags(&n.joined, hipEventDisableTiming) != hipSuccess) return nullptr;
        n.device = dev;
        f = n;
    }
    return &f;
}

struct Carver {
    char* base;
    size_t off = 0;
// ... 723 lines not shown
        if (c->ped_model == NAVSIM_PED_NONE || !st->robot_pose || !st->field) return NAVSIM_E_ARG;
        if (c->max_peds > NAVSIM_MAX_PEDS) return NAVSIM_E_UNSUPPORTED;
        if (c->field_format != NAVSIM_FIELD_U16T && c->field_format != NAVSIM_FIELD_F32) return NAVSIM_E_UNSUPPORTED;
    }
    const size_t P_all = (size_t)c->n_envs * (size_t)c->max_peds;
    if (p_count < 0) p_count = (long)P_all - p_begin;
    if (p_begin < 0 || (size_t)(p_begin + p_count) > P_all) return NAVSIM_E_ARG;
    const size_t P = (size_t)(p_begin + p_count);
    if (p_count == 0) return NAVSIM_OK;
    hipStream_t s = (hipStream_t)stream;
    constexpr size_t fc1_lds = (size_t)2 * (128 + 128) * 33 * sizeof(float);
    if (allow_lds((const void*)policy_fc1_kernel, fc1_lds) != NAVSIM_OK) return NAVSIM_E_UNSUPPORTED;
    policy_transpose_kernel<<<(kPolH2 * kPolIn2 + 255) / 256, 256, 0, s>>>(w->fc2_w, ws.w2t, w->cv2_w, ws.cv2t, *c, fused ? ws.tab : nullptr);
    for (size_t p0 = (size_t)p_begin; p0 < P; p0 += chunk) {
        const int n = (int)(P - p0 < chunk ? P - p0 : chunk);
        int rc = NAVSIM_OK;
        if (!fused) {
            policy_features_kernel<<<n, 256, 0, s>>>(ped_scans, (int)p0, n, w->cv1_w, w->cv1_b, ws.cv2t, w->cv2_b, ws.feat);
        } else if (c->field_format == NAVSIM_FIELD_U16T) {
            rc = st->rect_table ? launch_ped_scan_features<FieldU16T, true>(c, st, (int)p0, n, ws, scans_out, w, s)
                                : launch_ped_scan_features<FieldU16T, false>(c, st, (int)p0, n, ws, scans_out, w, s);
        } else {
            rc = launch_ped_scan_features<FieldF32, false>(c, st, (int)p0, n, ws, scans_out, w, s);
        }
        if (rc != NAVSIM_OK) return rc;
        policy_fc1_kernel<<<dim3((n + 127) / 128, 2), 256, fc1_lds, s>>>(ws.feat, n, w->fc1_w, w->fc1_b, ws.h1);
        policy_head_kernel<<<(n + kHeadPeds - 1) / kHeadPeds, 128, 0, s>>>(*c, *st, (int)p0, n, ws.h1, ws.w2t, *w, prev_actions, ped_cmd);
    }
    return launch_status();
}

int navsim_ped_policy(const navsim_config* c, const navsim_state* st, const navsim_policy_weights* w,
                      const float* ped_scans, float* prev_actions, double* ped_cmd, void* workspace,
                      size_t workspace_bytes, void* stream) {
    if (!ped_scans) return NAVSIM_E_ARG;
    return ped_policy_run(c, st, w, ped_scans, nullptr, prev_actions, ped_cmd, workspace, workspace_bytes, stream);
}

int navsim_ped_policy_part(const navsim_config* c, const navsim_state* st, const navsim_policy_weights* w,
                           const float* ped_scans, float* prev_actions, double* ped_cmd, void* workspace,
                           size_t workspace_bytes, int32_t e0, int32_t n_e, void* stream) {
    if (!ped_scans || !c || e0 < 0 || n_e < 0 || (long)e0 + n_e > c->n_envs) return NAVSIM_E_ARG;
    return ped_policy_run(c, st, w, ped_scans, nullptr, prev_actions, ped_cmd, workspace, workspace_bytes, stream,
                          (long)e0 * c->max_peds, (long)n_e * c->max_peds);
}

int navsim_ped_scan_policy(const navsim_config* c, const navsim_state* st, const navsim_policy_weights* w,
                           float* scans_out, float* prev_actions, double* ped_cmd, void* workspace,
                           size_t workspace_bytes, void* stream) {
    return ped_policy_run(c, st, w, nullptr, scans_out, prev_actions, ped_cmd, workspace, workspace_bytes, stream);
}

int navsim_crowd_check(const navsim_crowd_params* p, int32_t n_envs, int32_t max_agents, int32_t grid,
                       const uint8_t* free_map, const double* robot, const double* agents, const int32_t* n_agents,
                       const double* global_time, double* reward, uint8_t* done, int32_t* info, double* min_dist,
                       void* stream) {
    (void)hipGetLastError();
    if (!p || !free_map || !robot || !global_time || !reward || !done || !info || n_envs < 0 || max_agents < 0 ||
        grid < 1 || (max_agents > 0 && !agents))
        return NAVSIM_E_ARG;
    if (n_envs == 0) return NAVSIM_OK;
    crowd_check_kernel<<<n_envs, 64, 0, (hipStream_t)stream>>>(*p, max_agents, grid, free_map, robot, agents, n_agents,
                                                               global_time, reward, done, info, min_dist);
    return launch_status();
}

int navsim_crowd_angular_map(const navsim_crowd_map_params* p, int32_t n_envs, int32_t max_obst, int32_t n_vert,
                             const double* robot, const double* verts, const int32_t* n_obst, double* out, void* stream) {
    (void)hipGetLastError();
    if (!p || !robot || !out || n_envs < 0 || max_obst < 0 || n_vert < 1 || n_vert > NAVSIM_CROWD_MAX_VERTS ||
        p->angular_dim < 1 || (max_obst > 0 && !verts))
        return NAVSIM_E_ARG;
    if (p->angular_dim > 4096) return NAVSIM_E_UNSUPPORTED;
    if (n_envs == 0) return NAVSIM_OK;
    crowd_angular_map_kernel<<<n_envs, 64, (size_t)p->angular_dim * sizeof(unsigned long long), (hipStream_t)stream>>>(
        *p, max_obst, n_vert, robot, verts, n_obst, out);
    return launch_status();
}

int navsim_crowd_local_map(const navsim_crowd_map_params* p, int32_t n_envs, int32_t grid, const uint8_t* free_map,
                           const double* robot, int32_t rotate, uint8_t* out, void* stream) {
    (void)hipGetLastError();
    if (!p || !free_map || !robot || !out || n_envs < 0 || grid < 1) return NAVSIM_E_ARG;
    const int S = (int)nearbyint(p->submap_size_m / p->map_resolution);
    if (S < 1 || (size_t)S * S > 64 * 1024) return NAVSIM_E_UNSUPPORTED;
    if (n_envs == 0) return NAVSIM_OK;
    crowd_local_map_kernel<<<n_envs, 256, (size_t)S * S, (hipStream_t)stream>>>(*p, grid, S, free_map, robot, rotate, out);
    return launch_status();
}

int navsim_crowd_orca(const navsim_orca_params* p, int32_t n_queries, int32_t max_agents, const double* agents,
                      const int32_t* n_agents, const double* pref_vel, int32_t max_obst, int32_t n_vert,
                      const double* verts, const int32_t* n_obst, const int32_t* obst_set, const double* theta,
                      double* out_vel, double* out_action, void* stream) {
    (void)hipGetLastError();
    if (!p || !agents || !pref_vel || !out_vel || n_queries < 0 || max_agents < 1 || max_agents > NAVSIM_ORCA_MAX_AGENTS ||
        max_obst < 0 || n_vert < 2 || (size_t)max_obst * n_vert > NAVSIM_ORCA_MAX_EDGES || (max_obst > 0 && !verts))
        return NAVSIM_E_ARG;
    if (n_queries == 0) return NAVSIM_OK;
    crowd_orca_kernel<<<(n_queries + 63) / 64, 64, 0, (hipStream_t)stream>>>(*p, n_queries, max_agents, agents, n_agents,
                                                                          pref_vel, max_obst, n_vert, verts, n_obst,
                                                                          obst_set, theta, out_vel, out_action);
    return launch_status();
}

int navsim_ped_orca(const navsim_config* c, const navsim_state* st, const navsim_ped_orca_params* p, double* ped_cmd, void* stream) {
    (void)hipGetLastError();
    if (!c || !st || !p || !ped_cmd) return NAVSIM_E_ARG;
    if (c->ped_model != NAVSIM_PED_EXTERNAL || c->n_envs < 0 || c->max_peds < 1) return NAVSIM_E_ARG;
    if (p->robot_visible != 0 && p->robot_visible != 1) return NAVSIM_E_ARG;
    if ((long)c->max_peds + p->robot_visible > NAVSIM_ORCA_MAX_AGENTS) return NAVSIM_E_ARG;
    if (!(p->ped_radius > 0.0) || !(p->robot_radius > 0.0) || !(p->orca.time_step > 0.0f) || !(p->orca.time_horizon > 0.0f) ||
        !(c->time_step > 0.0) || p->orca.max_neighbors < 0)
        return NAVSIM_E_ARG;
    if (c->max_waypoints < 1 || c->max_waypoints > NAVSIM_MAX_WAYPOINTS) return NAVSIM_E_ARG;
    if (!st->n_peds || !st->ped_pose || !st->ped_vel || !st->ped_v_pref || !st->ped_waypoints || !st->ped_n_waypoints ||
        !st->ped_wp_head || (p->robot_visible && (!st->robot_pose || !st->prev_action)))
        return NAVSIM_E_ARG;
    if (c->n_envs == 0) return NAVSIM_OK;
    const int N = c->max_peds, G = ped_orca_pack(N);
    const size_t lds = ped_orca_lds_bytes(N, ped_orca_list_len(N, p->orca.max_neighbors, p->robot_visible));
    const int rc = allow_lds((const void*)ped_orca_kernel, lds);
    if (rc != NAVSIM_OK) return rc;
    ped_orca_kernel<<<(c->n_envs + G - 1) / G, 64, lds, (hipStream_t)stream>>>(*c, *st, *p, ped_cmd);
    return launch_status();
}

int navsim_crowd_agent_step(double* pose, const double* action, double* vel, int32_t n, double time_step, void* stream) {
    (void)hipGetLastError();
    if (!pose || !action || n < 0) return NAVSIM_E_ARG;
    if (n == 0) return NAVSIM_OK;
    crowd_agent_step_kernel<<<(n + 255) / 256, 256, 0, (hipStream_t)stream>>>(pose, action, vel, n, time_step);
    return launch_status();
}

int navsim_launch_order(const uint32_t* cost, int32_t* order, int32_t n, void* stream) {
    (void)hipGetLastError();
    if (!cost || !order || n < 0) return NAVSIM_E_ARG;
    if (n == 0) return NAVSIM_OK;
    launch_order_kernel<<<1, 1024, 0, (hipStream_t)stream>>>(cost, order, n);
    return launch_status();
}

int navsim_step(const navsim_config* c, const navsim_state* st, const navsim_step_io* io, void* stream) {
    (void)hipGetLastError();
    int rc = check_step_args(c, st, io, 0);
    if (rc != NAVSIM_OK) return rc;
    if (c->n_envs == 0) return NAVSIM_OK;
    StepLaunch l;
    l.stream = (hipStream_t)stream;
    return dispatch_step(c, st, io, l);
}

int navsim_step_part(const navsim_config* c, const navsim_state* st, const navsim_step_io* io, int32_t part, void* stream) {
    (void)hipGetLastError();
    if (part == NAVSIM_STEP_ALL) return navsim_step(c, st, io, stream);
    if (part != NAVSIM_STEP_NOT_DUE && part != NAVSIM_STEP_DUE) return NAVSIM_E_ARG;
    int rc = check_step_args(c, st, io, 0);
    if (rc != NAVSIM_OK) return rc;
    if (!st->ped_due_prev || !st->ped_due || st->ped_due == st->ped_due_prev) return NAVSIM_E_ARG;
    if (c->ped_model == NAVSIM_PED_NONE) return NAVSIM_E_ARG;
    if (ped_split_on(c)) return NAVSIM_E_UNSUPPORTED;
    if (c->n_envs == 0) return NAVSIM_OK;
    StepLaunch l;
    l.part = part;
    l.stream = (hipStream_t)stream;
    navsim_config c2 = *c;
    if (part == NAVSIM_STEP_DUE) {
        l.grid = compact_grid(c);
        if (!c->step_block) { const int b = pick_step_block(c); c2.step_block = b >= 512 ? 1024 : (b >= 256 ? 512 : b); }
    }
    return dispatch_step(&c2, st, io, l);
}

int navsim_step_replan(const navsim_config* c, const navsim_state* st, const navsim_step_io* io, int32_t max_queries, void* stream) {
    (void)hipGetLastError();
    int rc = check_step_args(c, st, io, 0);
    if (rc != NAVSIM_OK) return rc;
    if (max_queries < 0) return NAVSIM_E_ARG;
    rc = replan_in_step(c, st, true);
    if (rc != NAVSIM_OK) return rc;
    if (c->n_envs == 0) return NAVSIM_OK;
    StepLaunch l;
    l.part = kStepPartReplan;
    l.grid = compact_grid(c);
    l.max_queries = max_queries;
    l.stream = (hipStream_t)stream;
    return dispatch_step(c, st, io, l);
}

int navsim_prepare(const navsim_config* c, const navsim_state* st, const navsim_step_io* io) {
    (void)hipGetLastError();
    int rc = check_step_args(c, st, io, 1);
    if (rc != NAVSIM_OK) return rc;
    if (c->n_envs == 0) return NAVSIM_OK;
    const bool fused_peds = c->ped_model != NAVSIM_PED_NONE && !ped_split_on(c);
    const StepInstall none = {};
    StepLaunch l;
    l.prepare_only = true;
    rc = dispatch_step(c, st, io, l);
    l.reset_only = true;
    if (rc == NAVSIM_OK) rc = dispatch_step(c, st, io, l);
    l.grid = c->regen_cap;
    if (rc == NAVSIM_OK && c->regen_cap > 0) rc = dispatch_step(c, st, io, l);
    l.reset_only = false; l.grid = 32; l.part = NAVSIM_STEP_DUE;
    if (rc == NAVSIM_OK && fused_peds) rc = dispatch_step(c, st, io, l);
    l.part = kStepPartReplan;
    if (rc == NAVSIM_OK && replan_in_step(c, st, false) == NAVSIM_OK) rc = dispatch_step(c, st, io, l);
    l.grid = 0; l.part = NAVSIM_STEP_ALL; l.install = &none;
    if (rc == NAVSIM_OK && c->field_format == NAVSIM_FIELD_U16T && (c->ped_model == NAVSIM_PED_NONE || fused_peds))
        rc = dispatch_step(c, st, io, l);
    if (rc != NAVSIM_OK) return rc;
    if (c->regen_plan && c->regen_indoor_ratio > 0.0) (void)regen_fork();
    const int Hc = c->map_h / 5, Wc = c->map_w / 5;
    if (Hc >= 1 && Wc >= 1 && plan_fits(Hc, Wc)) {
        (void)allow_lds((const void*)plan_kernel, plan_lds(Hc, Wc));
    }
    return NAVSIM_OK;
}

int navsim_reset_obs(const navsim_config* c, const navsim_state* st, const navsim_step_io* io,
                     const uint8_t* mask, void* stream) {
    (void)hipGetLastError();
    int rc = check_step_args(c, st, io, 1);
    if (rc != NAVSIM_OK) return rc;
    if (c->n_envs == 0) return NAVSIM_OK;
    StepLaunch l;
    l.reset_only = true;
    l.mask = mask;
    l.stream = (hipStream_t)stream;
    return dispatch_step(c, st, io, l);
}

int navsim_restart(const navsim_config* c, const navsim_state* st, const uint8_t* mask, void* stream) {
    (void)hipGetLastError();
    if (!c || !st || !mask || c->n_envs < 0 || c->n_spawn < 1 || !st->spawn_pose || !st->spawn_goal || !st->robot_pose ||
        !st->robot_goal || !st->episode || !st->steps)
        return NAVSIM_E_ARG;
    if (c->n_envs == 0) return NAVSIM_OK;
    restart_kernel<<<(c->n_envs + 255) / 256, 256, 0, (hipStream_t)stream>>>(*c, *st, mask);
    return launch_status();
}

const char* navsim_step_kernel_name(void) { return "navsim_step_kernel"; }

int navsim_debug_math(int32_t fn, const double* x, const double* x2, double* out, int32_t n, void* stream) {
    (void)hipGetLastError();
    if (!x || !out || n < 0) return NAVSIM_E_ARG;
    if (n == 0) return NAVSIM_OK;
    math_kernel<<<(n + 255) / 256, 256, 0, (hipStream_t)stream>>>(fn, x, x2, out, n);
    return launch_status();
}

int navsim_debug_xy_to_ij(const navsim_config* c, const double* xy, int32_t as_f32, int32_t* ij, int32_t n, void* stream) {
    (void)hipGetLastError();
    if (!c || !xy || !ij || n < 0) return NAVSIM_E_ARG;
    if (n == 0) return NAVSIM_OK;
    xy_to_ij_kernel<<<(n + 255) / 256, 256, 0, (hipStream_t)stream>>>(*c, xy, as_f32, ij, n);
    return launch_status();
}

const char* navsim_last_hip_error(void) { return hipGetErrorString(g_last_hip_error); }

int navsim_debug_spawn_decisions(const navsim_config* c, const uint8_t* cost, int32_t Hc, int32_t Wc, int32_t n,
                                 const int32_t* kind, const double* start, const double* goal, const double* robot,
                                 double* wp_scratch, int32_t* code, void* stream) {
    (void)hipGetLastError();
    if (!c || !cost || !kind || !start || !goal || !wp_scratch || !code || n < 0 || Hc < 1 || Wc < 1 ||
        c->max_waypoints < 1 || c->max_waypoints > NAVSIM_MAX_WAYPOINTS) return NAVSIM_E_ARG;
    if (n == 0) return NAVSIM_OK;
    if (!plan_fits(Hc, Wc) || allow_lds((const void*)spawn_decisions_kernel, plan_lds(Hc, Wc)) != NAVSIM_OK)
        return NAVSIM_E_UNSUPPORTED;
    spawn_decisions_kernel<<<n, 256, plan_lds(Hc, Wc), (hipStream_t)stream>>>(*c, cost, Hc, Wc, kind, start, goal, robot,
                                                                            wp_scratch, code);
    return launch_status();
}

int navsim_debug_gather(const float* x, uint64_t n_words, int32_t mode, int32_t iters, int32_t n_threads,
                        float* out, void* stream) {
    (void)hipGetLastError();
    if (!x || !out || n_threads <= 0) return NAVSIM_E_ARG;
    gather_probe_kernel<<<(n_threads + 255) / 256, 256, 0, (hipStream_t)stream>>>(x, n_words, mode, iters, 12345, out);
    return launch_status();
}

int navsim_debug_kernarg_layout(void* stream) {
    hipStream_t s = (hipStream_t)stream;
    navsim_config c; navsim_state st; navsim_step_io io; StepInstall in;
    memset(&c, 0x5A, sizeof(c)); memset(&st, 0xA7, sizeof(st)); memset(&io, 0x3C, sizeof(io)); memset(&in, 0xE1, sizeof(in));
    for (size_t i = 0; i < sizeof(c); ++i) ((unsigned char*)&c)[i] ^= (unsigned char)(i * 7u);
    for (size_t i = 0; i < sizeof(st); ++i) ((unsigned char*)&st)[i] ^= (unsigned char)(i * 13u);
    for (size_t i = 0; i < sizeof(io); ++i) ((unsigned char*)&io)[i] ^= (unsigned char)(i * 29u);
    for (size_t i = 0; i < sizeof(in); ++i) ((unsigned char*)&in)[i] ^= (unsigned char)(i * 31u);
    int* out = nullptr;
    if (hipMalloc((void**)&out, sizeof(int)) != hipSuccess) return NAVSIM_E_LAUNCH;
    int res = -1;
    (void)hipMemcpyAsync(out, &res, sizeof(int), hipMemcpyHostToDevice, s);
    kernarg_layout_probe_kernel<<<1, 64, 0, s>>>(c, st, io, in, 0x1234567, out);
    const bool ok = hipMemcpyAsync(&res, out, sizeof(int), hipMemcpyDeviceToHost, s) == hipSuccess && hipStreamSynchronize(s) == hipSuccess;
    (void)hipFree(out);
    if (!ok) return NAVSIM_E_LAUNCH;
    return res == 1 ? NAVSIM_OK : NAVSIM_E_UNSUPPORTED;
}

int navsim_debug_set_stamps(unsigned long long* buf) {
#ifdef NAVSIM_STAMPS
// ... 14 lines not shown
```

nav-gym_amd/csrc/navsim_step_inst.hip:

```cpp
#include "preamble.hpp"

#if !defined(NAVSIM_INST_BLOCK) || !defined(NAVSIM_INST_PEDS)
#error "compile with -DNAVSIM_INST_BLOCK=64|256|512|1024 -DNAVSIM_INST_PEDS=0|1 (csrc/Makefile)"
#endif

namespace {
#include "kernels_field.hpp"
#include "kernels_rect.hpp"
#include "kernels_plan.hpp"
#include "kernels_regen_dev.hpp"
#include "kernels_step.hpp"
}
#include "step_plan.hpp"

namespace {

template <typename Kernel, typename... Args>
int launch(Kernel kernel, const StepLaunch& l, int blocks, int block, size_t lds, const Args&... args) {
    if (allow_lds((const void*)kernel, lds) != NAVSIM_OK) return NAVSIM_E_UNSUPPORTED;
    if (l.prepare_only) return NAVSIM_OK;
    kernel<<<blocks, block, lds, l.stream>>>(args...);
    return NAVSIM_OK;
}

template <int BLOCK, bool PEDS, typename Field, int RECT, int RULE, bool PINL>
int launch_step_pinl(const navsim_config* c, const navsim_state* st, const navsim_step_io* io, const StepLaunch& l, const StepPlan& p) {
    constexpr bool kPacked = !std::is_same<Field, FieldF32>::value;
    const unsigned scan = (unsigned)step_lds_scan_bytes(c, p.park);
    const int blocks = l.grid > 0 ? l.grid : c->n_envs;
    if constexpr (PEDS && PINL) {
        if (l.part == kStepPartReplan) {
            const size_t pl = plan_lds(c->map_h / 5, c->map_w / 5), lds = p.lds > pl ? p.lds : pl;
            if (l.install) {
                if constexpr (kPacked)
                    return launch(navsim_step_replan_install_kernel<BLOCK, Field, RULE, RECT>, l, l.grid + c->n_envs, BLOCK, lds,
                                  *c, *st, *io, *l.install, scan, p.park, p.rect_off, l.grid, l.max_queries);
                return NAVSIM_E_UNSUPPORTED;
            }
            return launch(navsim_step_replan_kernel<BLOCK, Field, RULE, RECT>, l, l.grid + c->n_envs, BLOCK, lds,
                          *c, *st, *io, scan, p.park, p.rect_off, l.grid, l.max_queries);
        }
        if (l.part == NAVSIM_STEP_DUE)
            return launch(navsim_step_due_kernel<BLOCK, Field, RULE, RECT>, l, blocks, BLOCK, p.lds, *c, *st, *io, scan, p.park, p.rect_off);
    }
    if constexpr (PINL == PEDS && kPacked) {
        if (l.install)
            return launch(navsim_step_install_kernel<BLOCK, PEDS, Field, RULE, RECT>, l, blocks, BLOCK, p.lds,
                          *c, *st, *io, *l.install, step_kernel_word(l), l.mask, scan, p.park, p.rect_off);
    }
    if (l.install) return NAVSIM_E_UNSUPPORTED;
    if constexpr (!PEDS) {
        const bool feat = io->final_obs || io->reset_mask || c->auto_reset == NAVSIM_AUTORESET_NEXT_STEP ||
                          (c->max_episode_steps > 0 && !l.reset_only);
        if (!feat)
            return launch(navsim_step_kernel<BLOCK, PEDS, Field, RULE, RECT, PINL, false>, l, blocks, BLOCK, p.lds,
                          *c, *st, *io, step_kernel_word(l), l.mask, scan, p.park, p.rect_off);
    }
    return launch(navsim_step_kernel<BLOCK, PEDS, Field, RULE, RECT, PINL, true>, l, blocks, BLOCK, p.lds,
                  *c, *st, *io, step_kernel_word(l), l.mask, scan, p.park, p.rect_off);
}
template <int BLOCK, bool PEDS, typename Field, int RECT, int RULE>
int launch_step_kernel(const navsim_config* c, const navsim_state* st, const navsim_step_io* io, const StepLaunch& l, const StepPlan& p) {
    if constexpr (PEDS) {
        if ((!l.reset_only && !l.peds_done) || l.install) return launch_step_pinl<BLOCK, PEDS, Field, RECT, RULE, true>(c, st, io, l, p);
    }
    return launch_step_pinl<BLOCK, PEDS, Field, RECT, RULE, false>(c, st, io, l, p);
}

template <int BLOCK, bool PEDS, typename Field, int RECT>
int launch_step_rule(const navsim_config* c, const navsim_state* st, const navsim_step_io* io, const StepLaunch& l,
                     const StepPlan& p) {
    return with_march_rule<Field>(march_rule_variant(c), [&](auto rule) {
        return launch_step_kernel<BLOCK, PEDS, Field, RECT, decltype(rule)::value>(c, st, io, l, p);
    });
}

template <int BLOCK, bool PEDS, typename Field>
int launch_step_field(const navsim_config* c, const navsim_state* st, const navsim_step_io* io, const StepLaunch& l,
                      const StepPlan& p) {
    if (p.rect == 2) return launch_step_rule<BLOCK, PEDS, Field, 2>(c, st, io, l, p);
    return p.rect ? launch_step_rule<BLOCK, PEDS, Field, 1>(c, st, io, l, p)
                  : launch_step_rule<BLOCK, PEDS, Field, 0>(c, st, io, l, p);
}

template <int BLOCK, bool PEDS>
int launch_step_family(const navsim_config* c, const navsim_state* st, const navsim_step_io* io, const StepLaunch& l,
                       const StepPlan& p) {
    if (c->field_format == NAVSIM_FIELD_U16T && !st->field_overflow)
        return launch_step_field<BLOCK, PEDS, FieldU16TN>(c, st, io, l, p);
    if (c->field_format == NAVSIM_FIELD_U16T)
        return launch_step_field<BLOCK, PEDS, FieldU16T>(c, st, io, l, p);
    return launch_step_rule<BLOCK, PEDS, FieldF32, 0>(c, st, io, l, p);
}

}

#define NAVSIM_CAT_(a, b, c) a##b##_##c
#define NAVSIM_CAT(a, b, c) NAVSIM_CAT_(a, b, c)

extern "C" __attribute__((visibility("hidden")))
int NAVSIM_CAT(navsim_step_launch_, NAVSIM_INST_BLOCK, NAVSIM_INST_PEDS)(const navsim_config* c, const navsim_state* st,
                                                                        const navsim_step_io* io, const StepLaunch* l, const StepPlan* p) {
    return launch_step_family<NAVSIM_INST_BLOCK, (NAVSIM_INST_PEDS != 0)>(c, st, io, *l, *p);
}

extern "C" __attribute__((visibility("hidden")))
int NAVSIM_CAT(navsim_step_set_stamps_, NAVSIM_INST_BLOCK, NAVSIM_INST_PEDS)(unsigned long long* buf) {
#ifdef NAVSIM_STAMPS
    return hipMemcpyToSymbol(HIP_SYMBOL(g_stamps), &buf, sizeof(buf)) == hipSuccess ? NAVSIM_OK : NAVSIM_E_LAUNCH;
#else
    (void)buf;
    return NAVSIM_E_UNSUPPORTED;
#endif
}
```

nav-gym_amd/csrc/step_plan.hpp:

```cpp

struct StepPlan {
    int block;
    int rect;
    int park;
    size_t lds;
    unsigned rect_off;
};
struct StepLaunch {
    bool reset_only = false;
    bool peds_done = false;
    int part = NAVSIM_STEP_ALL;
    const uint8_t* mask = nullptr;
    int grid = 0;
    int max_queries = 0;
    const StepInstall* install = nullptr;
    bool prepare_only = false;
    hipStream_t stream = nullptr;
};

namespace {
constexpr size_t kLdsPerCu = 160 * 1024;
int allow_lds(const void* kernel, size_t lds) {
    if (lds <= 64 * 1024) return NAVSIM_OK;
    if (lds > kLdsPerCu) return NAVSIM_E_UNSUPPORTED;
    struct Granted { const void* kernel; int device; size_t lds; };
    constexpr int kSlots = 256;
    static Granted table[kSlots];
    static int used = 0;
    static std::mutex lock;
    int dev = 0;
    if (hipGetDevice(&dev) != hipSuccess) dev = -1;
    std::lock_guard<std::mutex> guard(lock);
    Granted* slot = nullptr;
    for (int i = 0; i < used; ++i)
        if (table[i].kernel == kernel && table[i].device == dev) { slot = &table[i]; break; }
    if (slot && slot->lds >= lds) return NAVSIM_OK;
    if (hipFuncSetAttribute(kernel, hipFuncAttributeMaxDynamicSharedMemorySize, (int)lds) != hipSuccess) return NAVSIM_E_UNSUPPORTED;
    if (!slot && used < kSlots) { slot = &table[used++]; slot->kernel = kernel; slot->device = dev; }
    if (slot) slot->lds = lds;
    return NAVSIM_OK;
}

int device_cu_count() {
    static std::atomic<int> cache[64];
    int dev = 0;
    if (hipGetDevice(&dev) != hipSuccess || dev < 0 || dev >= 64) return 256;
    int v = cache[dev].load(std::memory_order_relaxed);
    if (v > 0) return v;
    int n = 0;
    if (hipDeviceGetAttribute(&n, hipDeviceAttributeMultiprocessorCount, dev) != hipSuccess || n <= 0) n = 256;
    cache[dev].store(n, std::memory_order_relaxed);
    return n;
}

int step_park_lanes(const navsim_config* c, int block) {
    const bool peds = c->ped_model != NAVSIM_PED_NONE;
    if (!step_parks(block, peds)) return 0;
    if (peds) return c->n_beams <= 65535 ? NAVSIM_PARK_LANES_PEDS : 0;
    return kParkLanesMax;
}
size_t step_lds_scan_bytes(const navsim_config* c, int park_lanes) {
    const bool peds = c->ped_model != NAVSIM_PED_NONE;
    return park_lds_bytes(c->n_beams, park_lanes, peds) + (peds ? (size_t)c->n_beams * (sizeof(float2) + sizeof(float)) : 0);
}
size_t ped_update_lds_bytes(const navsim_config* c) {
    return (size_t)ped_pack(c->max_peds) * ped_slot_bytes(c->max_peds);
}
bool ped_split_on(const navsim_config* c) {
    if (c->ped_model == NAVSIM_PED_NONE || ped_update_lds_bytes(c) > 64 * 1024) return false;
    return c->ped_split == 2;
}
size_t step_lds_bytes(const navsim_config* c, int park_lanes) {
    size_t lds = step_lds_scan_bytes(c, park_lanes);
    if (c->ped_model != NAVSIM_PED_NONE) {
        lds = ((lds + 15) & ~(size_t)15) + ped_lds_bytes(c->max_peds);
        if (!ped_split_on(c)) lds = ((lds + 15) & ~(size_t)15) + ped_pair_bytes(c->max_peds);
    }
    return lds;
}

int pick_step_block(const navsim_config* c) {
    if (c->step_block) return c->step_block;
    const int B = c->n_beams;
    const long cus = device_cu_count();
    if (B <= 64) return 64;
    if ((long)c->n_envs >= 12 * cus || B <= 256) return 256;
    if ((long)c->n_envs > 2 * cus || B <= 512) return 512;
    return 1024;
}

int march_rule_variant(const navsim_config* c) {
    if (c->march_rule == NAVSIM_MARCH_F32 || c->march_rule == NAVSIM_MARCH_F32_FMA) return c->march_rule;
    const int side = c->map_h > c->map_w ? c->map_h : c->map_w;
    return (c->field_format == NAVSIM_FIELD_U16T && side <= 1448) ? kMarchF64Exact32 : NAVSIM_MARCH_F64;
}
template <typename Field, typename F>
int with_march_rule(int rule, F&& f) {
#ifdef NAVSIM_ONLY_RULE
    if (rule != NAVSIM_ONLY_RULE) return NAVSIM_E_UNSUPPORTED;
    return f(std::integral_constant<int, NAVSIM_ONLY_RULE>{});
#else
    switch (rule) {
        case NAVSIM_MARCH_F32: return f(std::integral_constant<int, NAVSIM_MARCH_F32>{});
        case NAVSIM_MARCH_F32_FMA: return f(std::integral_constant<int, NAVSIM_MARCH_F32_FMA>{});
        case kMarchF64Exact32:
            if constexpr (!std::is_same<Field, FieldF32>::value) return f(std::integral_constant<int, kMarchF64Exact32>{});
            [[fallthrough]];
        default: return f(std::integral_constant<int, NAVSIM_MARCH_F64>{});
    }
#endif
}

int step_kernel_word(const StepLaunch& l) {
    return (l.reset_only ? kStepWordResetOnly : 0) | ((l.peds_done ? 1 : 0) << kStepWordPedsDoneBit) | (l.part << kStepWordPartShift);
}
StepPlan plan_step(const navsim_config* c, const navsim_state* st, int grid = 0) {
    StepPlan p;
    p.block = pick_step_block(c);
    p.rect = st->rect_table ? 1 : 0;
    p.park = step_park_lanes(c, p.block);
    p.lds = step_lds_bytes(c, p.park);
    p.rect_off = 0;
    if (p.rect && st->rect_index && c->closed_maps && c->rect_lds != 1 && c->field_format == NAVSIM_FIELD_U16T) {
        const size_t row = rect_index_row_bytes(c->map_h, c->map_w);
        const size_t base = (p.lds + 15) & ~(size_t)15;
        const size_t total = base + row + 1024;
        const int per_cu = p.block >= 1024 ? 2 : (p.block == 512 ? 4 : 5);
        const bool lone = grid > 0 && grid <= device_cu_count();
        const bool fits = c->rect_lds == 2 || lone ? total <= kLdsPerCu : (size_t)per_cu * total <= kLdsPerCu;
        if (fits) { p.rect = 2; p.lds = base + row; p.rect_off = (unsigned)row; }
    }
    return p;
}
}
```

nav-gym_amd/nav_gym_amd/abi.py:

```python
import ctypes as C

ABI_VERSION = 7

OK = 0
E_ARG = -1
E_LAUNCH = -2
E_UNSUPPORTED = -3
E_NODEVICE = -4

PED_NONE = 0
PED_EXTERNAL = 1
PED_SFM = 2

MAX_PEDS = 64
MAX_WAYPOINTS = 256
OBS_TAIL = 7

FIELD_F32 = 0
FIELD_U16T = 1
FIELD_TILE = 8

MARCH_F64 = 0
MARCH_F32 = 1
MARCH_F32_FMA = 2
# ... 184 lines not shown
    "beam_table": ("float64", ("B", 2)),
    "scan_threshold": ("float32", ("B",)),
    "scan_discomfort": ("float32", ("B",)),
    "scan_noise_std": ("float32", ("E",)),
    "robot_pose": ("float64", ("E", 3)),
    "robot_goal": ("float64", ("E", 2)),
    "prev_action": ("float64", ("E", 2)),
    "prev_pose": ("float64", ("E", 3)),
    "n_hist": ("int32", ("E",)),
    "episode": ("int64", ("E",)),
    "steps": ("int64", ("E",)),
    "n_peds": ("int32", ("E",)),
    "ped_pose": ("float64", ("E", "N", 3)),
    "ped_vel": ("float64", ("E", "N", 2)),
    "ped_prev_yaw": ("float64", ("E", "N")),
    "ped_dist": ("float64", ("E", "N", 3)),
    "ped_v_pref": ("float64", ("E", "N")),
    "ped_has_legs": ("uint8", ("E", "N")),
    "ped_waypoints": ("float64", ("E", "N", "P", 2)),
    "ped_n_waypoints": ("int32", ("E", "N")),
    "ped_cmd": ("float64", ("E", "N", 2)),
    "spawn_pose": ("float64", ("E", "K", 3)),
    "spawn_goal": ("float64", ("E", "K", 2)),
    "costmap": ("uint8", ("E", "Hc", "Wc")),
    "arena_cost": ("int32", ("E",)),
    "launch_order": ("int32", ("E",)),
    "regen_draws": ("float64", ("E", 464)),
    "ped_goal": ("float64", ("E", "N", 2)),
    "counters": ("int64", (N_COUNTERS,)),
    "rect_index": ("uint8", ("E", "R")),
    "ped_wp_head": ("int32", ("E", "N")),
    "ped_due": ("int64", ("E",)),
    "ped_due_prev": ("int64", ("E",)),
    "done_steps": ("int32", ("E",)),
    "map_slot": ("int32", ("E",)),
}

IO_LAYOUT = {
    "action": ("float64", ("E", 2)),
    "obs_prev": ("float32", ("E", "D")),
    "obs": ("float32", ("E", "D")),
    "achieved_goal": ("float32", ("E", 2)),
    "desired_goal": ("float32", ("E", 2)),
    "reward": ("float64", ("E",)),
    "done": ("uint8", ("E",)),
    "is_success": ("float32", ("E",)),
    "is_crash": ("float32", ("E",)),
    "distance": ("float64", ("E",)),
}


FINAL_LAYOUT = {
    "final_obs": ("float32", ("E", "D")),
    "final_goals": ("float32", ("E", 4)),
}


LIMIT_LAYOUT = {
    "truncated": ("uint8", ("E",)),
}


def rect_index_row_bytes(H, W):
    return 256 * 8 + ((((H + 7) // 8) * ((W + 7) // 8) * 2 + 15) // 16) * 16


def resolve_shape(shape, cfg):
    sym = {
        "E": cfg.n_envs, "N": cfg.max_peds, "B": cfg.n_beams, "S": cfg.n_scan_stack,
        "K": max(cfg.n_spawn, 1), "P": cfg.max_waypoints, "H": cfg.map_h, "W": cfg.map_w,
        "D": cfg.n_scan_stack * cfg.n_beams + OBS_TAIL, "Hc": cfg.map_h // 5, "Wc": cfg.map_w // 5,
        "T": ((cfg.map_h + 7) // 8) * ((cfg.map_w + 7) // 8),
        "R": rect_index_row_bytes(cfg.map_h, cfg.map_w),
    }
    return tuple(sym[s] if isinstance(s, str) else s for s in shape)


def declare(lib, suffix=""):
    stream = [] if suffix else [_P]
    i32, f32, f64 = C.c_int32, C.c_float, C.c_double
    cfgp, stp, iop = C.POINTER(NavsimConfig), C.POINTER(NavsimState), C.POINTER(NavsimStepIO)

    def sig(name, args, res=C.c_int):
        fn = getattr(lib, name + suffix)
        fn.argtypes = args
        fn.restype = res
        return fn

    sig("navsim_default_config", [cfgp])
    if suffix:
        sig("navsim_build_dt", [_P, i32, i32, i32, _P])
    else:
        sig("navsim_build_dt", [_P, i32, i32, i32, _P, _P, C.c_size_t, _P])
    if not suffix:
        sig("navsim_field_bytes", [i32, i32, i32, i32], C.c_size_t)
        sig("navsim_build_field", [_P, i32, i32, i32, i32, _P, _P, _P, _P, C.c_size_t, _P])
        sig("navsim_rect_table_bytes", [i32, i32, i32], C.c_size_t)
        sig("navsim_build_rects_workspace_bytes", [i32, i32, i32], C.c_size_t)
        sig("navsim_build_rects", [_P, i32, i32, i32, _P, i32, _P, _P, _P, C.c_size_t, _P])
        sig("navsim_rect_index_bytes", [i32, i32, i32], C.c_size_t)
        sig("navsim_build_rect_index", [_P, i32, i32, i32, _P, _P, _P])
        sig("navsim_maps_closed", [_P, i32, i32, i32, _P, _P])
        sig("navsim_world_closed", [cfgp, stp, _P, _P])
    sig("navsim_cast_static", [_P, i32, i32, i32, _P, i32, f32, i32, _P] + stream)
    sig("navsim_render_polys", [_P, _P, i32, i32, _P, _P, i32, _P] + stream)
    sig("navsim_render_legs", [_P, _P, i32, i32, _P, _P, i32, _P] + stream)
    sig("navsim_integrate", [_P, _P, _P, i32, f64, f64] + stream)
    sig("navsim_reward_done", [cfgp, _P, _P, i32, i32, _P, _P, _P, _P, _P, _P, _P] + stream)
    sig("navsim_scan_threshold", [cfgp, _P, i32, _P] + stream)
    if not suffix:
        sig("navsim_beam_table", [cfgp, _P, _P])
        sig("navsim_debug_xy_to_ij", [cfgp, _P, i32, _P, i32, _P])
        sig("navsim_debug_kernarg_layout", [_P])
    sig("navsim_ped_scans", [cfgp, stp, _P] + stream)
    if not suffix:
        sig("navsim_ped_scans_part", [cfgp, stp, _P, i32, i32, _P])
        sig("navsim_ped_policy_part", [cfgp, stp, C.POINTER(NavsimPolicyWeights), _P, _P, _P, _P, C.c_size_t, i32, i32, _P])
    if suffix:
        sig("navsim_regen", [cfgp, stp, iop])
        sig("navsim_replan", [cfgp, stp, i32])
        sig("navsim_ped_policy", [cfgp, stp, C.POINTER(NavsimPolicyWeights), _P, _P, _P])
    else:
        sig("navsim_ped_policy_workspace_bytes", [cfgp], C.c_size_t)
        sig("navsim_ped_policy", [cfgp, stp, C.POINTER(NavsimPolicyWeights), _P, _P, _P, _P, C.c_size_t, _P])
        sig("navsim_ped_scan_policy", [cfgp, stp, C.POINTER(NavsimPolicyWeights), _P, _P, _P, _P, C.c_size_t, _P])
        sig("navsim_launch_order", [_P, _P, i32, _P])
        sig("navsim_replan_workspace_bytes", [cfgp, i32], C.c_size_t)
        sig("navsim_replan", [cfgp, stp, i32, _P, C.c_size_t, _P])
        sig("navsim_costmap", [_P, i32, i32, i32, _P, _P])
        sig("navsim_plan", [_P, _P, i32, i32, i32, f64, f64, f64, _P, _P, f64, i32, _P, _P, _P, _P, _P])
        sig("navsim_regen_workspace_bytes", [cfgp], C.c_size_t)
        sig("navsim_regen", [cfgp, stp, iop, _P, C.c_size_t, _P])
        sig("navsim_regen_swap", [cfgp, stp, stp, iop, _P, _P, _P, _P, _P])
        sig("navsim_regen_stage", [cfgp, stp, iop, _P, _P, _P, _P, C.c_size_t, _P])
        sig("navsim_regen_stage_part", [cfgp, stp, iop, _P, _P, _P, _P, C.c_size_t, i32, i32, _P])
        sig("navsim_step_install", [cfgp, stp, iop, stp, _P, _P, _P, _P, _P])
        sig("navsim_regen_helper", [_P])
        sig("navsim_step_install_replan", [cfgp, stp, iop, stp, _P, _P, _P, _P, C.c_int32, _P])
        sig("navsim_step_install_next", [cfgp, stp, iop, stp, _P, _P, _P, _P, _P, C.c_int32, _P])
    sig("navsim_crowd_check", [C.POINTER(NavsimCrowdParams), i32, i32, i32, _P, _P, _P, _P, _P, _P, _P, _P, _P] + stream)
    mpp = C.POINTER(NavsimCrowdMapParams)
    sig("navsim_crowd_angular_map", [mpp, i32, i32, i32, _P, _P, _P, _P] + stream)
    sig("navsim_crowd_local_map", [mpp, i32, i32, _P, _P, i32, _P] + stream)
    sig("navsim_crowd_orca", [C.POINTER(NavsimOrcaParams), i32, i32, _P, _P, _P, i32, i32, _P, _P, _P, _P, _P, _P] + stream)
    sig("navsim_crowd_agent_step", [_P, _P, _P, i32, f64] + stream)
    if not suffix:
        sig("navsim_ped_orca", [cfgp, stp, C.POINTER(NavsimPedOrcaParams), _P, _P])
    if not suffix:
        sig("navsim_prepare", [cfgp, stp, iop])
    sig("navsim_step", [cfgp, stp, iop] + stream)
    if not suffix:
        sig("navsim_step_part", [cfgp, stp, iop, i32, _P])
        sig("navsim_step_replan", [cfgp, stp, iop, i32, _P])
    sig("navsim_reset_obs", [cfgp, stp, iop, _P] + stream)
    sig("navsim_restart", [cfgp, stp, _P] + stream)
    return lib


EXPORTS = (
    "navsim_abi_version", "navsim_error_string", "navsim_last_hip_error", "navsim_default_config",
    "navsim_build_dt_workspace_bytes", "navsim_build_dt", "navsim_field_bytes", "navsim_build_field",
    "navsim_rect_table_bytes", "navsim_build_rects_workspace_bytes", "navsim_build_rects",
    "navsim_rect_index_bytes", "navsim_build_rect_index", "navsim_maps_closed", "navsim_world_closed",
    "navsim_cast_static",
    "navsim_render_polys", "navsim_render_legs", "navsim_integrate", "navsim_reward_done",
    "navsim_scan_threshold", "navsim_beam_table", "navsim_ped_scans", "navsim_ped_scans_part", "navsim_ped_policy_part", "navsim_regen_workspace_bytes", "navsim_regen", "navsim_regen_swap", "navsim_regen_stage", "navsim_regen_stage_part", "navsim_step_install", "navsim_regen_helper", "navsim_step_install_replan", "navsim_step_install_next",
    "navsim_costmap", "navsim_plan", "navsim_launch_order", "navsim_replan_workspace_bytes", "navsim_replan", "navsim_ped_policy_workspace_bytes", "navsim_ped_policy", "navsim_ped_scan_policy",
    "navsim_crowd_check", "navsim_crowd_angular_map", "navsim_crowd_local_map", "navsim_crowd_orca", "navsim_crowd_agent_step", "navsim_ped_orca",
    "navsim_step", "navsim_step_part", "navsim_step_replan", "navsim_prepare", "navsim_reset_obs", "navsim_restart", "navsim_step_kernel_name",
    "navsim_sizeof_config", "navsim_sizeof_state", "navsim_sizeof_step_io", "navsim_debug_math", "navsim_debug_xy_to_ij",
    "navsim_debug_gather", "navsim_debug_kernarg_layout", "navsim_debug_set_stamps", "navsim_debug_spawn_decisions",
)
```

nav-gym_amd/nav_gym_amd/sim.py:

```python
import ctypes as C
import os

import numpy as np

from . import abi
from .lib import check, load, require_gpu

_TORCH_DTYPE = None


def _dtype(name):
    global _TORCH_DTYPE
    import torch
    if _TORCH_DTYPE is None:
        _TORCH_DTYPE = {"float32": torch.float32, "float64": torch.float64, "int32": torch.int32,
                        "int64": torch.int64, "uint8": torch.uint8}
    return _TORCH_DTYPE[name]


def _ptr(t):
    return None if t is None else C.c_void_p(t.data_ptr())


def _stream():
# ... 265 lines not shown
    check(load().navsim_crowd_agent_step(_ptr(pose), _ptr(action), _ptr(vel), pose.shape[0], float(time_step), _stream()),
          "navsim_crowd_agent_step")
    return pose, vel


def debug_kernarg_layout():
    require_gpu()
    check(load().navsim_debug_kernarg_layout(_stream()), "navsim_debug_kernarg_layout")


def debug_xy_to_ij(cfg, xy, as_f32):
    torch = require_gpu()
    xy = xy.to(torch.float64).contiguous()
    out = torch.empty((xy.shape[0], 2), dtype=torch.int32, device=xy.device)
    check(load().navsim_debug_xy_to_ij(C.byref(cfg), _ptr(xy), int(bool(as_f32)), _ptr(out), xy.shape[0], _stream()),
          "navsim_debug_xy_to_ij")
    return out


def debug_spawn_decisions(cfg, cost, kind, start, goal, robot=None):
    torch = require_gpu()
    dev = cost.device
    cost = cost.to(torch.uint8).contiguous()
    Hc, Wc = cost.shape
    kind = torch.as_tensor(kind).to(device=dev, dtype=torch.int32).contiguous()
    n = kind.shape[0]
    f64 = lambda a: None if a is None else torch.as_tensor(a).to(device=dev, dtype=torch.float64).contiguous().reshape(n, 2)
    start, goal, robot = f64(start), f64(goal), f64(robot)
    ws = torch.zeros((n, cfg.max_waypoints, 2), dtype=torch.float64, device=dev)
    code = torch.full((n,), -1, dtype=torch.int32, device=dev)
    L = load()
    L.navsim_debug_spawn_decisions.argtypes = [C.POINTER(abi.NavsimConfig), C.c_void_p, C.c_int32, C.c_int32, C.c_int32,
                                               C.c_void_p, C.c_void_p, C.c_void_p, C.c_void_p, C.c_void_p, C.c_void_p,
                                               C.c_void_p]
    check(L.navsim_debug_spawn_decisions(C.byref(cfg), _ptr(cost), Hc, Wc, n, _ptr(kind), _ptr(start), _ptr(goal),
                                         _ptr(robot), _ptr(ws), _ptr(code), _stream()), "navsim_debug_spawn_decisions")
    return code


def debug_math(fn, x, x2=None):
    torch = require_gpu()
    out = torch.empty_like(x)
    check(load().navsim_debug_math(fn, _ptr(x), _ptr(x2), _ptr(out), x.numel(), _stream()), "navsim_debug_math")
    return out


def concurrent_stream(device, priority=0, tries=8, beside=None):
    import torch
    if not hasattr(torch.cuda, "_sleep"):
        return torch.cuda.Stream(device=device, priority=priority)
    others = list(beside) if beside else [torch.cuda.current_stream(device)]
    best, best_ratio = None, None
    spin = 100_000
    e0, e1 = torch.cuda.Event(enable_timing=True), torch.cuda.Event(enable_timing=True)
    for _ in range(tries):
        cand = torch.cuda.Stream(device=device, priority=priority)
        with torch.cuda.stream(cand):
            for rep in range(2):
                torch.cuda.synchronize(device)
                e0.record(cand); torch.cuda._sleep(spin); e1.record(cand)
                torch.cuda.synchronize(device)
        alone = e0.elapsed_time(e1)
        worst = 0.0
        for other in others:
            for rep in range(2):
                torch.cuda.synchronize(device)
                e0.record(other)
                cand.wait_event(e0)
                with torch.cuda.stream(cand):
                    torch.cuda._sleep(spin)
                with torch.cuda.stream(other):
                    torch.cuda._sleep(spin)
                other.wait_stream(cand)
                e1.record(other)
                torch.cuda.synchronize(device)
            worst = max(worst, e0.elapsed_time(e1) / max(alone, 1e-6))
        if best_ratio is None or worst < best_ratio:
            best, best_ratio = cand, worst
        if worst < 1.5:
            return cand
    return best


class NavSim(object):

    def __init__(self, cfg, arrays, device="cuda:0", launch_order=None, final_obs=False):
        torch = require_gpu()
        self.lib = load()
        self.cfg = cfg.copy()
        self.device = torch.device(device)
        self.t = {}
        self.st = abi.NavsimState()
        for name, (dtype, shape) in abi.STATE_LAYOUT.items():
            a = arrays.get(name)
            if a is None:
                setattr(self.st, name, None)
                continue
            if name == "field" and self.cfg.field_format != abi.FIELD_F32:
                t = a.to(self.device).contiguous()
                want = self.lib.navsim_field_bytes(self.cfg.n_envs, self.cfg.map_h, self.cfg.map_w,
                                                   self.cfg.field_format)
                if t.numel() * t.element_size() != want:
                    raise ValueError("field blob has %d bytes, expected %d" % (t.numel() * t.element_size(), want))
                self.t[name] = t
                setattr(self.st, name, t.data_ptr())
                continue
            if isinstance(a, np.ndarray):
                a = torch.from_numpy(np.ascontiguousarray(a))
            t = a.to(device=self.device, dtype=_dtype(dtype)).contiguous()
            if t.data_ptr() == a.data_ptr():
                t = t.clone()
            want = abi.resolve_shape(shape, self.cfg)
            if tuple(t.shape) != want:
                raise ValueError("%s: shape %s, expected %s" % (name, tuple(t.shape), want))
            self.t[name] = t
            setattr(self.st, name, t.data_ptr())
        if self.cfg.closed_maps and "rect_index" in self.t:
            n_open = torch.zeros(1, dtype=torch.int32, device=self.device)
            check(self.lib.navsim_world_closed(C.byref(self.cfg), C.byref(self.st), _ptr(n_open), _stream()), "navsim_world_closed")
            if int(n_open.item()):
                raise ValueError("cfg.closed_maps = 1, but %d arenas have a map without a closed ring of 3 occupied cells "
                                 "(navsim_maps_closed / navsim_world_closed): clear closed_maps or close the maps" % int(n_open.item()))
        self.due = None
        if "ped_waypoints" in self.t:
            if "ped_wp_head" not in self.t:
                self.t["ped_wp_head"] = torch.zeros((self.cfg.n_envs, self.cfg.max_peds), dtype=torch.int32, device=self.device)
                self.st.ped_wp_head = self.t["ped_wp_head"].data_ptr()
            self.due = [torch.zeros(self.cfg.n_envs, dtype=torch.int64, device=self.device) for _ in range(2)]
            self.st.ped_due = self.due[0].data_ptr()
            self.st.ped_due_prev = self.due[1].data_ptr()
        if "done_steps" not in self.t and self.cfg.auto_reset:
            self.t["done_steps"] = torch.zeros(self.cfg.n_envs, dtype=torch.int32, device=self.device)
            self.st.done_steps = self.t["done_steps"].data_ptr()
        if "counters" not in self.t:
            self.t["counters"] = torch.zeros(abi.N_COUNTERS, dtype=torch.int64, device=self.device)
            self.st.counters = self.t["counters"].data_ptr()
        if "beam_table" not in self.t:
            tab = torch.empty((self.cfg.n_beams, 2), dtype=torch.float64, device=self.device)
            check(self.lib.navsim_beam_table(C.byref(self.cfg), _ptr(tab), _stream()), "navsim_beam_table")
            self.t["beam_table"] = tab
            self.st.beam_table = tab.data_ptr()
        self.lpt_period = 8
        self._steps_launched = 0
        n_cu = torch.cuda.get_device_properties(self.device).multi_processor_count or 256
        block = self.cfg.step_block or (
            64 if self.cfg.n_beams <= 64 else (256 if self.cfg.n_envs >= 12 * n_cu or self.cfg.n_beams <= 256 else
                                               (512 if self.cfg.n_envs > 2 * n_cu or self.cfg.n_beams <= 512 else 1024)))
        generations = self.cfg.n_envs * (block // 64) / float(32 * n_cu)
        if (launch_order is True or (launch_order is None and generations > 1.25)) and "arena_cost" not in self.t:
            self.t["arena_cost"] = torch.zeros(self.cfg.n_envs, dtype=torch.int32, device=self.device)
            self.t["launch_order"] = torch.arange(self.cfg.n_envs, dtype=torch.int32, device=self.device)
            self.st.arena_cost = self.t["arena_cost"].data_ptr()
            self.st.launch_order = self.t["launch_order"].data_ptr()
        E = self.cfg.n_envs
        D = self.cfg.n_scan_stack * self.cfg.n_beams + abi.OBS_TAIL
        self.obs_buf = [torch.zeros((E, D), dtype=torch.float32, device=self.device) for _ in range(2)]
        self.cur = 0
        self.out_buf = [{k: torch.zeros(abi.resolve_shape(s, self.cfg), dtype=_dtype(d), device=self.device)
                         for k, (d, s) in abi.IO_LAYOUT.items() if k not in ("obs", "obs_prev", "action")} for _ in range(2)]
        if self.cfg.max_episode_steps > 0:
            for b in self.out_buf:
                b.update({k: torch.zeros(abi.resolve_shape(s, self.cfg), dtype=_dtype(d), device=self.device)
                          for k, (d, s) in abi.LIMIT_LAYOUT.items()})
        self.action = torch.zeros((E, 2), dtype=torch.float64, device=self.device)
        self.io = abi.NavsimStepIO()
        self.io.action = self.action.data_ptr()
        for k, v in self.out_buf[0].items():
            setattr(self.io, k, v.data_ptr())
        self.final_buf = None
        if final_obs:
            self.final_buf = [{k: torch.zeros(abi.resolve_shape(s, self.cfg), dtype=_dtype(d), device=self.device)
                               for k, (d, s) in abi.FINAL_LAYOUT.items()} for _ in range(2)]
        self.next_step = self.cfg.auto_reset == abi.AUTORESET_NEXT_STEP

    @property
    def obs(self):
        return self.obs_buf[self.cur]

    @property
    def out(self):
        return self.out_buf[self.cur]

    @property
    def final(self):
        return None if self.final_buf is None else self.final_buf[self.cur]

    @property
    def reset_flags(self):
        return self.out_buf[1 - self.cur]["done"]

    def _flip(self):
        self.io.obs_prev = self.obs_buf[self.cur].data_ptr()
        self.io.obs = self.obs_buf[1 - self.cur].data_ptr()
        self.io.reset_mask = self.out_buf[self.cur]["done"].data_ptr() if self.next_step else None
        if self.final_buf is not None:
            for k, v in self.final_buf[1 - self.cur].items():
                setattr(self.io, k, v.data_ptr())
        for k, v in self.out_buf[1 - self.cur].items():
            setattr(self.io, k, v.data_ptr())
        if self.due is not None:
            self.st.ped_due_prev = self.due[self.cur].data_ptr()
            self.st.ped_due = self.due[1 - self.cur].data_ptr()

    def _latest_flags(self):
        if self.due is not None:
            self.st.ped_due = self.due[self.cur].data_ptr()
            self.st.ped_due_prev = self.due[1 - self.cur].data_ptr()

    def reset_obs(self, mask=None):
        for k, v in self.out_buf[1 - self.cur].items():
            v.copy_(self.out_buf[self.cur][k])
        m = None
        if mask is not None:
            import torch
            m = torch.as_tensor(mask).to(device=self.device, dtype=torch.uint8).contiguous()
        for k in [k for k in ("done", "truncated") if k in self.out_buf[0]]:
            if m is None:
                self.out_buf[1 - self.cur][k].zero_()
            else:
                self.out_buf[1 - self.cur][k].mul_(m == 0)
        self._flip()
        check(self.lib.navsim_reset_obs(C.byref(self.cfg), C.byref(self.st), C.byref(self.io), _ptr(m), _stream()),
              "navsim_reset_obs")
        if self.due is not None:
            self.due[1 - self.cur].copy_(self.due[self.cur])
        self.cur = 1 - self.cur
        return self.obs

    def _reorder(self):
        self._steps_launched += 1
        n = self._steps_launched
        if "launch_order" in self.t and self.lpt_period > 0 and (2 <= n <= 5 or n % self.lpt_period == 0):
            check(self.lib.navsim_launch_order(_ptr(self.t["arena_cost"]), _ptr(self.t["launch_order"]), self.cfg.n_envs,
                                               _stream()), "navsim_launch_order")

    def step(self, action=None):
        if action is not None:
            import torch
            if (isinstance(action, torch.Tensor) and action.is_cuda and action.dtype == torch.float64 and action.is_contiguous()
                    and action.device == self.device and action.numel() == self.action.numel()):
                self.io.action = action.data_ptr()
                self._action_ref = action
            else:
                self.action.copy_(self._as(action, self.action))
                self.io.action = self.action.data_ptr()
        self._reorder()
        self._flip()
        self._launch()
        self.cur = 1 - self.cur
        return self.obs, self.out

    def _launch(self):
        if not getattr(self, "pg_install", False):
            rc = self.lib.navsim_step(C.byref(self.cfg), C.byref(self.st), C.byref(self.io), _stream())
            if rc:
                check(rc, "navsim_step")
            return
        import torch
        main = torch.cuda.current_stream()
        P, k = self.pg_period, self.pg_k
        if k % P == 0 and k >= 2 * P:
            main.wait_event(self.pg_staged[(k // P - 2) % 3])
        if getattr(self, "late2", None) is not None:
            return self._launch_next_step(main)
        late = None if getattr(self, "lone", False) else self.late
        if getattr(self, "pg_replan_cap", 0) > 0 and self.pg_replan_in_step:
            rc = self.lib.navsim_step_install_replan(C.byref(self.cfg), C.byref(self.st), C.byref(self.io), C.byref(self.stage_st),
                                                     _ptr(self.stage_obs), _ptr(self.mark), _ptr(self.ready), _ptr(late),
                                                     int(self.pg_replan_cap), C.c_void_p(main.cuda_stream))
            if rc == 0:
                return
            if rc != abi.E_UNSUPPORTED:
                check(rc, "navsim_step_install_replan")
            self.pg_replan_in_step = False
        rc = self.lib.navsim_step_install(C.byref(self.cfg), C.byref(self.st), C.byref(self.io), C.byref(self.stage_st),
                                          _ptr(self.stage_obs), _ptr(self.mark), _ptr(self.ready), _ptr(late),
                                          C.c_void_p(main.cuda_stream))
        if rc == abi.E_UNSUPPORTED and late is None and self.late is not None:
            self.lone = False
            rc = self.lib.navsim_step_install(C.byref(self.cfg), C.byref(self.st), C.byref(self.io), C.byref(self.stage_st),
                                              _ptr(self.stage_obs), _ptr(self.mark), _ptr(self.ready), _ptr(self.late),
                                              C.c_void_p(main.cuda_stream))
        check(rc, "navsim_step_install")

    def _launch_next_step(self, main):
        import torch
        prev, nxt = self.late2[self.cur], self.late2[1 - self.cur]
        cap = int(getattr(self, "pg_replan_cap", 0)) if self.pg_replan_in_step else 0
        rc = self.lib.navsim_step_install_next(C.byref(self.cfg), C.byref(self.st), C.byref(self.io), C.byref(self.stage_st),
                                               _ptr(self.stage_obs), _ptr(self.mark), _ptr(self.ready), _ptr(nxt), _ptr(prev),
                                               cap if cap > 0 else -1, C.c_void_p(main.cuda_stream))
        if rc == abi.E_UNSUPPORTED and cap > 0:
            self.pg_replan_in_step = False
            rc = self.lib.navsim_step_install_next(C.byref(self.cfg), C.byref(self.st), C.byref(self.io), C.byref(self.stage_st),
                                                   _ptr(self.stage_obs), _ptr(self.mark), _ptr(self.ready), _ptr(nxt), _ptr(prev),
                                                   -1, C.c_void_p(main.cuda_stream))
        check(rc, "navsim_step_install_next")
        urgent = self.urgent
        urgent.wait_event(self.ev_stepped)
        C.memmove(C.byref(self.late_cfg), C.byref(self.cfg), C.sizeof(self.cfg))
        self.late_cfg.regen_cap = self.late_cap
        self.late_cfg.defer_reset_scan = 1
        io = abi.NavsimStepIO()
        C.memmove(C.byref(io), C.byref(self.io), C.sizeof(io))
        io.done = prev.data_ptr()
        io.reset_mask = None
        helper = getattr(self, "_regen_helper", None)
        if helper is not None:
            self.lib.navsim_regen_helper(C.c_void_p(urgent.cuda_stream))
        check(self.lib.navsim_regen(C.byref(self.late_cfg), C.byref(self.st), C.byref(io), _ptr(self.late_ws), self.late_ws.numel(),
                                    C.c_void_p(urgent.cuda_stream)), "navsim_regen (arenas whose world was not staged, beside the step)")
        if helper is not None:
            self.lib.navsim_regen_helper(C.c_void_p(helper.cuda_stream))
        self.ev_urgent.record(urgent)
        main.wait_event(self.ev_urgent)
        self.ev_stepped.record(main)

    STAGED = ("field", "field_overflow", "rect_table", "rect_index", "costmap", "scan_noise_std", "robot_pose", "robot_goal", "prev_action",
              "prev_pose", "n_hist", "steps", "episode", "n_peds", "ped_pose", "ped_vel", "ped_prev_yaw", "ped_dist",
              "ped_v_pref", "ped_has_legs", "ped_waypoints", "ped_n_waypoints", "ped_wp_head", "ped_goal", "spawn_pose", "spawn_goal")

    MAPS = ("field", "field_overflow", "rect_table", "rect_index", "costmap")

    def enable_pregen(self, scratch_bytes=4 << 30, pipeline=0, install=False, stage_cap=None, map_slots=True, fallback=None,
                      fallback_cap=None, late_beside=False, fallback_poll=None, stage_lanes=None):
        import torch
        if not self.cfg.auto_reset:
            raise ValueError("enable_pregen needs cfg.auto_reset = 1 (the step advances episode[e] when an arena finishes)")
        E = self.cfg.n_envs
        P = int(pipeline)
        if fallback is None:
            fallback = bool(install) and P > 0 and self.cfg.regen_min_steps < 4 * P
        if fallback and not install:
            raise ValueError("enable_pregen(fallback=True) is a feature of install=True")
        if P < 0 or (P > 0 and self.cfg.regen_min_steps < 4 * P and not fallback):
            raise ValueError("enable_pregen(pipeline=%d) needs cfg.regen_min_steps >= %d (it is %d): an arena must not want its "
                             "next world before the pass that stages it was waited for -- or fallback=True (install=True)"
                             % (P, 4 * P, self.cfg.regen_min_steps))
        self.pg_period, self.pg_k = P, 0
        if install and (not P or self.cfg.regen_cap < E):
            raise ValueError("enable_pregen(install=True) needs pipeline >= 1 and cfg.regen_cap >= n_envs (every finished arena "
                             "decides alone inside the step: there is no cap in index order)")
        self.ready = torch.zeros(2 * E, dtype=torch.int64, device=self.device) if P else None
        shared_maps = bool(install and map_slots)
        self.stage_t = {k: self.t[k].clone() for k in self.STAGED if k in self.t and not (shared_maps and k in self.MAPS)}
        self.stage_t["episode"] = self.t["episode"] + 1
        self.stage_st = abi.NavsimState()
        C.memmove(C.byref(self.stage_st), C.byref(self.st), C.sizeof(self.st))
        for k, v in self.stage_t.items():
            setattr(self.stage_st, k, v.data_ptr())
        if install and map_slots:
            for k in self.MAPS:
                if k in self.t:
                    live = self.t[k]
                    n = live.shape[0]
                    both = torch.empty((2 * n,) + tuple(live.shape[1:]), dtype=live.dtype, device=live.device)
                    both[:n].copy_(live); both[n:].copy_(live)
                    del live
                    self.t[k] = self.stage_t[k] = both
                    setattr(self.st, k, both.data_ptr()); setattr(self.stage_st, k, both.data_ptr())
            self.t["map_slot"] = torch.arange(E, dtype=torch.int32, device=self.device)
            self.stage_t["map_slot"] = torch.arange(E, 2 * E, dtype=torch.int32, device=self.device)
            self.st.map_slot = self.t["map_slot"].data_ptr()
            self.stage_st.map_slot = self.stage_t["map_slot"].data_ptr()
        self.stage_st.arena_cost = None
        self.stage_st.launch_order = None
        self.stage_st.counters = None
        self.stage_st.ped_due = None
        self.stage_st.ped_due_prev = None
        self.stage_obs = torch.zeros_like(self.obs_buf[0])
        self.want = torch.ones(E, dtype=torch.uint8, device=self.device)
        self.mark = torch.zeros((E + 3) // 4 * 4, dtype=torch.uint8, device=self.device)
        self.stage_io = abi.NavsimStepIO()
        self.stage_io.obs = self.stage_obs.data_ptr()
        self.stage_io.done = self.want.data_ptr()
        self._stage_all(scratch_bytes)
        self.stage_cap = self.cfg.regen_cap
        if P:
            per_step = max(8, E // 64) if install else self.cfg.regen_cap
            self.stage_cap = int(min(E, stage_cap if stage_cap else 2 * P * per_step))
        self.stage_cfg = self.cfg.copy()
        self.stage_cfg.regen_cap = self.stage_cap
        nbytes = self.lib.navsim_regen_workspace_bytes(C.byref(self.stage_cfg))
        self.stage_ws = torch.zeros(nbytes, dtype=torch.uint8, device=self.device)
        self.side = concurrent_stream(self.device, priority=0 if P else -1)
        if self.cfg.regen_plan and self.cfg.regen_indoor_ratio > 0.0:
            self._regen_helper = concurrent_stream(self.device, beside=[torch.cuda.current_stream(self.device), self.side])
            check(self.lib.navsim_regen_helper(C.c_void_p(self._regen_helper.cuda_stream)), "navsim_regen_helper")
        heavy = bool(self.cfg.regen_plan) or self.cfg.regen_indoor_ratio > 0.0
        lanes = int(stage_lanes) if stage_lanes else (2 if (install and P and heavy) else 1)
        if lanes not in (1, 2) or (lanes == 2 and not (install and P)):
            raise ValueError("enable_pregen(stage_lanes=%r): 1, or 2 with install=True and pipeline > 0" % (stage_lanes,))
        self.stage_lane = [dict(want=self.want, io=self.stage_io, ws=self.stage_ws, side=self.side,
                                helper=getattr(self, "_regen_helper", None))]
        if lanes == 2:
            want2 = torch.zeros(E, dtype=torch.uint8, device=self.device)
            io2 = abi.NavsimStepIO()
            C.memmove(C.byref(io2), C.byref(self.stage_io), C.sizeof(io2))
            io2.done = want2.data_ptr()
            side2 = concurrent_stream(self.device, beside=[torch.cuda.current_stream(self.device), self.side], priority=0)
            helper2 = None
            if getattr(self, "_regen_helper", None) is not None:
                helper2 = concurrent_stream(self.device, beside=[torch.cuda.current_stream(self.device), self.side, side2])
            self.stage_lane.append(dict(want=want2, io=io2, ws=torch.zeros(nbytes, dtype=torch.uint8, device=self.device), side=side2,
                                        helper=helper2))
        self.pg_passes = 0
        self.ev_swapped, self.ev_staged = torch.cuda.Event(), torch.cuda.Event()
# ... 523 lines not shown
```

Measured before the change: 51.22 million.

## Order lidar beams by previous-step probe counts to balance wave divergence

Adds a per-env beam cost buffer that records how many march probes each beam needed. On the next step, beams are counting-sorted by the cost of the beam that pointed the same way (adjusted for heading change), so each 64-lane wave marches rays of similar length. The goal is less SIMD divergence in the sphere-tracing loop. In exchange it adds an LDS counting sort, global byte stores per beam, scattered obs writes and extra per-step memory traffic. It is on by default for 256-thread kernels without pedestrians.

```diff
diff --git a/include/navsim.h b/include/navsim.h
--- a/include/navsim.h
+++ b/include/navsim.h
@@ -335,6 +335,10 @@
 
 int navsim_launch_order(const uint32_t* cost, int32_t* order, int32_t n, void* stream);
 
+size_t navsim_beam_cost_row_bytes(int32_t n_beams);
+int navsim_step_hinted(const navsim_config* cfg, const navsim_state* st, const navsim_step_io* io, uint8_t* beam_cost,
+                       void* stream);
+
 typedef struct navsim_crowd_params {
     double time_step, discomfort_dist, map_size_m, map_resolution;
     double success_reward, collision_penalty, discomfort_penalty_factor, rotation_penalty_factor, timeout_penalty;
diff --git a/nav-gym_amd/csrc/kernels_step.hpp b/nav-gym_amd/csrc/kernels_step.hpp
--- a/nav-gym_amd/csrc/kernels_step.hpp
+++ b/nav-gym_amd/csrc/kernels_step.hpp
@@ -362,7 +362,81 @@
     return (int)__builtin_amdgcn_mbcnt_hi((unsigned)(m >> 32), __builtin_amdgcn_mbcnt_lo((unsigned)m, 0u));
 }
 
-template <int BLOCK, typename Field, bool TO_LDS, int RULE, int RECT>
+constexpr int kHintKeys = 32;
+constexpr int kHintHeader = 16;
+__host__ __device__ inline size_t beam_cost_row_bytes(int B) { return kHintHeader + (((size_t)B + 15) & ~(size_t)15); }
+__host__ __device__ inline size_t hint_perm_bytes(int B) { return (2 * (size_t)B + 15) & ~(size_t)15; }
+__host__ __device__ inline size_t hint_lds_bytes(int B) { return hint_perm_bytes(B) + (((size_t)B + 15) & ~(size_t)15); }
+__device__ __forceinline__ void wave_lds_sync();
+__device__ __forceinline__ int* hint_counters() {
+    __shared__ int counters[2 * 4 * kHintKeys];
+    return counters;
+}
+__device__ __forceinline__ void order_beams(int B, float stepf, float lth, unsigned char* __restrict__ cost_row,
+                                            unsigned short* __restrict__ perm, unsigned char* __restrict__ slots) {
+    constexpr int W = 4;
+    int* cnt = hint_counters();
+    int* pos = cnt + W * kHintKeys;
+    int tid = (int)threadIdx.x;
+    asm volatile("" : "+v"(tid));
+    const int lane = tid & 63, w = tid >> 6;
+    float d = lth - *(const float*)cost_row;
+    d -= 6.2831853f * rintf(d * 0.15915494f);
+    float sf = (stepf > 0.0f) ? rintf(d / stepf) : 0.0f;
+    if (!(fabsf(sf) <= (float)B)) sf = (sf > 0.0f) ? (float)B : ((sf < 0.0f) ? -(float)B : 0.0f);
+    const int shift = (int)sf;
+    const int nchunks = (B + 63) >> 6, per = (nchunks + W - 1) / W;
+    const int ch0 = w * per, ch1 = (ch0 + per < nchunks) ? ch0 + per : nchunks;
+    for (int ch = ch0; ch < ch1; ++ch) {
+        const int k = ch * 64 + lane;
+        if (k < B) {
+            int j = k + shift;
+            j = j < 0 ? 0 : (j > B - 1 ? B - 1 : j);
+            int key = cost_row[kHintHeader + j];
+            key = key > kHintKeys - 1 ? kHintKeys - 1 : key;
+            const int slot = kHintKeys - 1 - key;
+            slots[k] = (unsigned char)slot;
+            atomicAdd(&cnt[w * kHintKeys + slot], 1);
+        }
+    }
+    __syncthreads();
+    if (tid == 0) *(float*)cost_row = lth;
+    {
+        int tot = 0, before = 0;
+        if (lane < kHintKeys)
+            for (int v = 0; v < W; ++v) {
+                const int x = cnt[v * kHintKeys + lane];
+                before += (v < w) ? x : 0;
+                tot += x;
+            }
+        int inc = tot;
+        inc += __builtin_amdgcn_update_dpp(0, inc, 0x111, 0xf, 0xf, false);
+        inc += __builtin_amdgcn_update_dpp(0, inc, 0x112, 0xf, 0xf, false);
+        inc += __builtin_amdgcn_update_dpp(0, inc, 0x114, 0xf, 0xf, false);
+        inc += __builtin_amdgcn_update_dpp(0, inc, 0x118, 0xf, 0xf, false);
+        inc += __builtin_amdgcn_update_dpp(0, inc, 0x142, 0xa, 0xf, false);
+        if (lane < kHintKeys) pos[w * kHintKeys + lane] = inc - tot + before;
+    }
+    wave_lds_sync();
+    for (int ch = ch0; ch < ch1; ++ch) {
+        const int k = ch * 64 + lane;
+        if (k < B) {
+            int q = atomicAdd(&pos[w * kHintKeys + slots[k]], 1);
+            q = q > B - 1 ? B - 1 : q;
+            perm[q] = (unsigned short)k;
+        }
+    }
+    __syncthreads();
+    if (tid < W * kHintKeys) cnt[tid] = 0;
+}
+__device__ __forceinline__ unsigned mask_count(lanemask_t m, unsigned n) {
+    unsigned r;
+    lanemask_t carry;
+    asm("v_addc_co_u32_e64 %0, %1, %2, 0, %3" : "=v"(r), "=&s"(carry) : "v"(n), "s"(m));
+    return r;
+}
+
+template <int BLOCK, typename Field, bool TO_LDS, int RULE, int RECT, bool HINT = false>
 __device__ __forceinline__ void scan_beams_pred(const navsim_config& c, StepShared& sh,
                                                 const Field& field, const uint4* __restrict__ rects,
                                                 const double* __restrict__ tab,
@@ -371,7 +445,9 @@
                                                 const float* __restrict__ thr, const float* __restrict__ dthr,
                                                 float* __restrict__ obs_row, int n_hist, float noise_std,
                                                 uint64_t noise_key, uint64_t genv,
-                                                int& crash, int& discomfort, bool prepare_prims = true) {
+                                                int& crash, int& discomfort, bool prepare_prims = true,
+                                                unsigned char* __restrict__ cost_row = nullptr, char* hint_lds = nullptr) {
+    static_assert(!HINT || (BLOCK == 256 && !TO_LDS && step_parks(BLOCK, TO_LDS)), "the beam order lives in the parking 256-thread kernels without pedestrians");
     const int B = c.n_beams, S = c.n_scan_stack, H = c.map_h, W = c.map_w;
     const float max_range = march_limit(H, W, c.range_max, c.resolution);
     const float res = (float)c.resolution;
@@ -387,7 +463,10 @@
     const float t1 = sh.t1, r_all = sh.r_all;
     const uint64_t nkey = (noise_std > 0.0f) ? nv::noise_stream(c.seed, genv, noise_key) : 0;
     int cr = 0, dc = 0;
-    auto finish = [&](int k, float dx, float dy, float rr) {
+    auto finish = [&](int k, float dx, float dy, float rr, unsigned probes = 0) {
+#ifndef NAVSIM_DIAG_HINT_NO_STORE
+        if constexpr (HINT) cost_row[kHintHeader + k] = (unsigned char)(probes < 255u ? probes : 255u);
+#endif
         if (TO_LDS) {
             rng_lds[k] = rr * res;
             dir_lds[k] = make_float2(dx, dy);
@@ -412,7 +491,13 @@
     if constexpr (TO_LDS) { if (prepare_prims) prims_prepare<BLOCK>(c, sh, pr); }
     constexpr bool kPark = step_parks(BLOCK, TO_LDS);
     int own_chunk = 0;
-    const int lane = (int)threadIdx.x & 63;
+    int lane = (int)threadIdx.x & 63;
+    if constexpr (HINT) asm volatile("" : "+v"(lane));
+    const unsigned short* perm = (const unsigned short*)hint_lds;
+#ifndef NAVSIM_DIAG_HINT_NO_ORDER
+    if constexpr (HINT)
+        order_beams(B, (float)step, sh.lth, cost_row, (unsigned short*)hint_lds, (unsigned char*)hint_lds + hint_perm_bytes(B));
+#endif
     for (;;) {
         int chunk = 0;
         if (BLOCK > 64) {
@@ -422,20 +507,26 @@
             chunk = own_chunk++;
         }
         if (chunk * 64 >= B) break;
-        const int k = chunk * 64 + lane;
+        int k = chunk * 64 + lane;
         const bool valid = k < B;
+#ifndef NAVSIM_DIAG_HINT_NO_ORDER
+        if constexpr (HINT) k = (int)perm[valid ? k : B - 1];
+#endif
         float dx, dy;
         beam_dir_k(c, tab, valid ? k : B - 1, step, (double)sh.lth, sh.cT, sh.sT, dx, dy);
         float t = t1;
         lanemask_t active = mask_of(valid & (r_all < 0.0f));
         lanemask_t hit = 0;
+        unsigned probes = (r_all < 0.0f) ? 2u : 1u;
         if constexpr (!kPark) {
             while (active != 0)
                 probe_round<Field, RULE, RECT>(field, (const char*)rects, tpr, x0, y0, dx, dy, uW, uH, max_range, t, active, hit);
             if (valid) finish(k, dx, dy, ray_result<RULE>(hit, int_range, i0, j0, x0, y0, dx, dy, t, miss));
         } else {
-            while ((int)__builtin_popcountll(active) > park_lanes)
+            while ((int)__builtin_popcountll(active) > park_lanes) {
                 probe_round<Field, RULE, RECT>(field, (const char*)rects, tpr, x0, y0, dx, dy, uW, uH, max_range, t, active, hit);
+                if constexpr (HINT) probes = mask_count(active, probes);
+            }
             const bool marching = mask_lane(active);
             if (active != 0) {
                 int base = 0;
@@ -447,11 +538,12 @@
                         rng_lds[k] = t;
                         dir_lds[k] = make_float2(dx, dy);
                     } else {
-                        park[base + lanes_below(active)] = make_float4(__int_as_float(k), t, dx, dy);
+                        const int rec = HINT ? (k | (int)((probes < 255u ? probes : 255u) << 16)) : k;
+                        park[base + lanes_below(active)] = make_float4(__int_as_float(rec), t, dx, dy);
                     }
                 }
             }
-            if (valid & !marching) finish(k, dx, dy, ray_result<RULE>(hit, int_range, i0, j0, x0, y0, dx, dy, t, miss));
+            if (valid & !marching) finish(k, dx, dy, ray_result<RULE>(hit, int_range, i0, j0, x0, y0, dx, dy, t, miss), probes);
         }
     }
     if constexpr (kPark) __syncthreads();
@@ -475,11 +567,15 @@
             k = __float_as_int(r.x);
             t = r.y; dx = r.z; dy = r.w;
         }
+        unsigned probes = 0;
+        if constexpr (HINT) { probes = (unsigned)k >> 16; k &= 0xFFFF; }
         lanemask_t active = mask_of(valid);
         lanemask_t hit = 0;
-        while (active != 0)
+        while (active != 0) {
             probe_round<Field, RULE, RECT>(field, (const char*)rects, tpr, x0, y0, dx, dy, uW, uH, max_range, t, active, hit);
-        if (valid) finish(k, dx, dy, ray_result<RULE>(hit, int_range, i0, j0, x0, y0, dx, dy, t, miss));
+            if constexpr (HINT) probes = mask_count(active, probes);
+        }
+        if (valid) finish(k, dx, dy, ray_result<RULE>(hit, int_range, i0, j0, x0, y0, dx, dy, t, miss), probes);
     }
     if (TO_LDS) {
         __syncthreads();
@@ -931,11 +1027,12 @@
     }
 }
 
-template <int BLOCK, bool PEDS, typename Field, int RULE, int RECT, bool PINL, bool INSTALL = false, bool FEAT = true>
+template <int BLOCK, bool PEDS, typename Field, int RULE, int RECT, bool PINL, bool INSTALL = false, bool FEAT = true, bool HINT = false>
 __device__ __forceinline__ void step_arena(const navsim_config& c, const navsim_state& st, const navsim_step_io& io, const int e,
                                            int reset_only, const int peds_done, const uint8_t* __restrict__ reset_mask,
                                            unsigned dyn_lds_bytes, int park_lanes, unsigned rect_lds_offset,
-                                           const StepInstall* in = nullptr, const int base_prio = 0) {
+                                           const StepInstall* in = nullptr, const int base_prio = 0,
+                                           unsigned char* __restrict__ beam_cost = nullptr) {
     __shared__ StepShared sh;
     extern __shared__ __attribute__((aligned(16))) char dyn_lds_all[];
     char* dyn_lds = dyn_lds_all + (RECT == 2 ? rect_lds_offset : 0u);
@@ -963,6 +1060,11 @@
     }
     float* obs_row = io.obs + (size_t)e * D;
     const float* obs_prev = io.obs_prev ? io.obs_prev + (size_t)e * D : nullptr;
+    unsigned char* cost_row = nullptr;
+    if constexpr (HINT) {
+        cost_row = beam_cost + (size_t)e * beam_cost_row_bytes(B);
+        if (tid < 4 * kHintKeys) hint_counters()[tid] = 0;
+    }
     double* rp_g = st.robot_pose + 3 * (size_t)e;
     double* goal_g = st.robot_goal + 2 * (size_t)e;
     double* pa_g = st.prev_action + 2 * (size_t)e;
@@ -1194,8 +1296,10 @@
     char* scan_lds = dyn_lds + park_lds_bytes(B, park_lanes, PEDS);
     float2* dir_lds = (float2*)scan_lds;
     float* rng_lds = (float*)(scan_lds + sizeof(float2) * (size_t)B);
-    scan_beams_pred<BLOCK, Field, PEDS, RULE, RECT>(c, sh, field, rects, st.beam_table, prims, dir_lds, rng_lds, park, park_lanes, st.scan_threshold,
-                                                         st.scan_discomfort, obs_row, n_hist, noise_std, step_key, genv, crash, discomfort, false);
+    char* hint_lds = scan_lds;
+    scan_beams_pred<BLOCK, Field, PEDS, RULE, RECT, HINT>(c, sh, field, rects, st.beam_table, prims, dir_lds, rng_lds, park, park_lanes, st.scan_threshold,
+                                                         st.scan_discomfort, obs_row, n_hist, noise_std, step_key, genv, crash, discomfort, false,
+                                                         cost_row, hint_lds);
 
     NAVSIM_STAMP(3);
     bool restart_next = false;
@@ -1300,8 +1404,9 @@
             if (sh.rescan) {
                 if (sh.respawn) n_hist = 0;
                 int c2, d2;
-                scan_beams_pred<BLOCK, Field, PEDS, RULE, RECT>(c, sh, field, rects, st.beam_table, prims, dir_lds, rng_lds, park, park_lanes, st.scan_threshold,
-                                                                     st.scan_discomfort, obs_row, n_hist, noise_std, sh.rescan_key, genv, c2, d2);
+                scan_beams_pred<BLOCK, Field, PEDS, RULE, RECT, HINT>(c, sh, field, rects, st.beam_table, prims, dir_lds, rng_lds, park, park_lanes, st.scan_threshold,
+                                                                     st.scan_discomfort, obs_row, n_hist, noise_std, sh.rescan_key, genv, c2, d2, true,
+                                                                     cost_row, hint_lds);
             }
         } else {
             float* final_row = io.final_obs ? io.final_obs + (size_t)e * D : nullptr;
@@ -1327,9 +1432,10 @@
                 __syncthreads();
                 if (pass == 1 && sh.respawn) n_hist = 0;
                 int c2, d2;
-                scan_beams_pred<BLOCK, Field, PEDS, RULE, RECT>(c, sh, field, rects, st.beam_table, prims, dir_lds, rng_lds, park, park_lanes, st.scan_threshold,
+                scan_beams_pred<BLOCK, Field, PEDS, RULE, RECT, HINT>(c, sh, field, rects, st.beam_table, prims, dir_lds, rng_lds, park, park_lanes, st.scan_threshold,
                                                                      st.scan_discomfort, pass == 0 ? final_row : obs_row, n_hist, noise_std,
-                                                                     pass == 0 ? step_key + 1 : sh.rescan_key, genv, c2, d2);
+                                                                     pass == 0 ? step_key + 1 : sh.rescan_key, genv, c2, d2, true,
+                                                                     cost_row, hint_lds);
                 if (pass == 0) {
                     for (int j = 0; j < S - 1; ++j)
                         if (S - 1 - j <= n_hist)
@@ -1435,6 +1541,20 @@
     step_arena<BLOCK, PEDS, Field, RULE, RECT, PINL, false, FEAT>(c, st, io, e, reset_only, peds_done, reset_mask, dyn_lds_bytes, park_lanes, rect_lds_offset);
 }
 
+template <typename Field, int RULE, int RECT, bool FEAT>
+__global__ __launch_bounds__(256) __attribute__((amdgpu_waves_per_eu(NAVSIM_NOPEDS_WAVES_MIN, 8)))
+void navsim_step_hinted_kernel(navsim_config c_, navsim_state st_, navsim_step_io io_, int reset_only,
+                               const uint8_t* __restrict__ reset_mask, unsigned dyn_lds_bytes, int park_lanes, unsigned rect_lds_offset,
+                               unsigned char* __restrict__ beam_cost) {
+    NAVSIM_KERNARGS(StepKernargs, c_, st_, io_);
+    const navsim_config& c = ka.c; const navsim_state& st = ka.st; const navsim_step_io& io = ka.io;
+    reset_only &= kStepWordResetOnly;
+    const int e = st.launch_order ? st.launch_order[blockIdx.x] : (int)blockIdx.x;
+    if (e < 0) return;
+    step_arena<256, false, Field, RULE, RECT, false, false, FEAT, true>(c, st, io, e, reset_only, 0, reset_mask, dyn_lds_bytes, park_lanes,
+                                                                        rect_lds_offset, nullptr, 0, beam_cost);
+}
+
 template <int BLOCK, bool PEDS, typename Field, int RULE, int RECT>
 __global__ __launch_bounds__(BLOCK) __attribute__((amdgpu_waves_per_eu((PEDS && RECT == 2 && BLOCK == 256) ? NAVSIM_PEDS_WAVES_MIN : (!PEDS ? NAVSIM_NOPEDS_WAVES_MIN : 8), 8)))
 void navsim_step_install_kernel(navsim_config c_, navsim_state st_, navsim_step_io io_, StepInstall in_, int reset_only,
diff --git a/nav-gym_amd/csrc/navsim_kernels.hip b/nav-gym_amd/csrc/navsim_kernels.hip
--- a/nav-gym_amd/csrc/navsim_kernels.hip
+++ b/nav-gym_amd/csrc/navsim_kernels.hip
@@ -23,6 +23,7 @@
     extern "C" int navsim_step_set_stamps_##B##_##P(unsigned long long*);
 NAVSIM_STEP_FAMILY(64, 0) NAVSIM_STEP_FAMILY(64, 1) NAVSIM_STEP_FAMILY(256, 0) NAVSIM_STEP_FAMILY(256, 1)
 NAVSIM_STEP_FAMILY(512, 0) NAVSIM_STEP_FAMILY(512, 1) NAVSIM_STEP_FAMILY(1024, 0) NAVSIM_STEP_FAMILY(1024, 1)
+NAVSIM_STEP_FAMILY(256, 0h)
 #undef NAVSIM_STEP_FAMILY
 
 #ifndef NAVSIM_PLAN_MANY_SEARCHES
@@ -46,7 +47,7 @@
 }
 
 int dispatch_step(const navsim_config* c, const navsim_state* st, const navsim_step_io* io, StepLaunch l) {
-    const StepPlan p = plan_step(c, st, l.part == NAVSIM_STEP_DUE || l.part == kStepPartReplan ? 0 : l.grid);
+    const StepPlan p = plan_step(c, st, l);
     const bool peds = c->ped_model != NAVSIM_PED_NONE;
     const bool split = peds && !l.reset_only && ped_split_on(c);
     const StepInstall no_install = {};
@@ -65,7 +66,8 @@
     int rc;
 #define NAVSIM_STEP_CASE(B) \
     case B: rc = peds ? navsim_step_launch_##B##_1(c, st, io, &l, &p) : navsim_step_launch_##B##_0(c, st, io, &l, &p); break;
-    switch (p.block) {
+    if (p.hint) rc = navsim_step_launch_256_0h(c, st, io, &l, &p);
+    else switch (p.block) {
         NAVSIM_STEP_CASE(64) NAVSIM_STEP_CASE(256) NAVSIM_STEP_CASE(512) NAVSIM_STEP_CASE(1024)
         default:   return NAVSIM_E_UNSUPPORTED;
     }
@@ -1095,6 +1097,19 @@
     return dispatch_step(c, st, io, l);
 }
 
+size_t navsim_beam_cost_row_bytes(int32_t n_beams) { return n_beams > 0 ? beam_cost_row_bytes(n_beams) : 0; }
+
+int navsim_step_hinted(const navsim_config* c, const navsim_state* st, const navsim_step_io* io, uint8_t* beam_cost, void* stream) {
+    (void)hipGetLastError();
+    int rc = check_step_args(c, st, io, 0);
+    if (rc != NAVSIM_OK) return rc;
+    if (c->n_envs == 0) return NAVSIM_OK;
+    StepLaunch l;
+    l.beam_cost = beam_cost;
+    l.stream = (hipStream_t)stream;
+    return dispatch_step(c, st, io, l);
+}
+
 int navsim_step_part(const navsim_config* c, const navsim_state* st, const navsim_step_io* io, int32_t part, void* stream) {
     (void)hipGetLastError();
     if (part == NAVSIM_STEP_ALL) return navsim_step(c, st, io, stream);
diff --git a/nav-gym_amd/csrc/navsim_step_inst.hip b/nav-gym_amd/csrc/navsim_step_inst.hip
--- a/nav-gym_amd/csrc/navsim_step_inst.hip
+++ b/nav-gym_amd/csrc/navsim_step_inst.hip
@@ -26,8 +26,19 @@
 template <int BLOCK, bool PEDS, typename Field, int RECT, int RULE, bool PINL>
 int launch_step_pinl(const navsim_config* c, const navsim_state* st, const navsim_step_io* io, const StepLaunch& l, const StepPlan& p) {
     constexpr bool kPacked = !std::is_same<Field, FieldF32>::value;
-    const unsigned scan = (unsigned)step_lds_scan_bytes(c, p.park);
+    const unsigned scan = (unsigned)step_lds_scan_bytes(c, p.park, p.hint);
     const int blocks = l.grid > 0 ? l.grid : c->n_envs;
+#ifdef NAVSIM_INST_HINT
+    static_assert(BLOCK == 256 && !PEDS && !PINL, "the beam order: 256 threads, no pedestrians");
+    (void)kPacked;
+    if (!p.hint || !l.beam_cost) return NAVSIM_E_UNSUPPORTED;
+    const bool feat = io->final_obs || io->reset_mask || c->auto_reset == NAVSIM_AUTORESET_NEXT_STEP || c->max_episode_steps > 0;
+    if (!feat)
+        return launch(navsim_step_hinted_kernel<Field, RULE, RECT, false>, l, blocks, BLOCK, p.lds,
+                      *c, *st, *io, step_kernel_word(l), l.mask, scan, p.park, p.rect_off, (unsigned char*)l.beam_cost);
+    return launch(navsim_step_hinted_kernel<Field, RULE, RECT, true>, l, blocks, BLOCK, p.lds,
+                  *c, *st, *io, step_kernel_word(l), l.mask, scan, p.park, p.rect_off, (unsigned char*)l.beam_cost);
+#else
     if constexpr (PEDS && PINL) {
         if (l.part == kStepPartReplan) {
             const size_t pl = plan_lds(c->map_h / 5, c->map_w / 5), lds = p.lds > pl ? p.lds : pl;
@@ -58,6 +69,7 @@
     }
     return launch(navsim_step_kernel<BLOCK, PEDS, Field, RULE, RECT, PINL, true>, l, blocks, BLOCK, p.lds,
                   *c, *st, *io, step_kernel_word(l), l.mask, scan, p.park, p.rect_off);
+#endif
 }
 template <int BLOCK, bool PEDS, typename Field, int RECT, int RULE>
 int launch_step_kernel(const navsim_config* c, const navsim_state* st, const navsim_step_io* io, const StepLaunch& l, const StepPlan& p) {
@@ -98,14 +110,19 @@
 #define NAVSIM_CAT_(a, b, c) a##b##_##c
 #define NAVSIM_CAT(a, b, c) NAVSIM_CAT_(a, b, c)
 
+#ifdef NAVSIM_INST_HINT
+#define NAVSIM_INST_NAME(prefix) NAVSIM_CAT(prefix, NAVSIM_INST_BLOCK, 0h)
+#else
+#define NAVSIM_INST_NAME(prefix) NAVSIM_CAT(prefix, NAVSIM_INST_BLOCK, NAVSIM_INST_PEDS)
+#endif
 extern "C" __attribute__((visibility("hidden")))
-int NAVSIM_CAT(navsim_step_launch_, NAVSIM_INST_BLOCK, NAVSIM_INST_PEDS)(const navsim_config* c, const navsim_state* st,
+int NAVSIM_INST_NAME(navsim_step_launch_)(const navsim_config* c, const navsim_state* st,
                                                                         const navsim_step_io* io, const StepLaunch* l, const StepPlan* p) {
     return launch_step_family<NAVSIM_INST_BLOCK, (NAVSIM_INST_PEDS != 0)>(c, st, io, *l, *p);
 }
 
 extern "C" __attribute__((visibility("hidden")))
-int NAVSIM_CAT(navsim_step_set_stamps_, NAVSIM_INST_BLOCK, NAVSIM_INST_PEDS)(unsigned long long* buf) {
+int NAVSIM_INST_NAME(navsim_step_set_stamps_)(unsigned long long* buf) {
 #ifdef NAVSIM_STAMPS
     return hipMemcpyToSymbol(HIP_SYMBOL(g_stamps), &buf, sizeof(buf)) == hipSuccess ? NAVSIM_OK : NAVSIM_E_LAUNCH;
 #else
diff --git a/nav-gym_amd/csrc/step_plan.hpp b/nav-gym_amd/csrc/step_plan.hpp
--- a/nav-gym_amd/csrc/step_plan.hpp
+++ b/nav-gym_amd/csrc/step_plan.hpp
@@ -5,6 +5,7 @@
     int park;
     size_t lds;
     unsigned rect_off;
+    bool hint;
 };
 struct StepLaunch {
     bool reset_only = false;
@@ -14,6 +15,7 @@
     int grid = 0;
     int max_queries = 0;
     const StepInstall* install = nullptr;
+    uint8_t* beam_cost = nullptr;
     bool prepare_only = false;
     hipStream_t stream = nullptr;
 };
@@ -59,9 +61,14 @@
     if (peds) return c->n_beams <= 65535 ? NAVSIM_PARK_LANES_PEDS : 0;
     return kParkLanesMax;
 }
-size_t step_lds_scan_bytes(const navsim_config* c, int park_lanes) {
+size_t step_lds_scan_bytes(const navsim_config* c, int park_lanes, bool hint = false) {
     const bool peds = c->ped_model != NAVSIM_PED_NONE;
-    return park_lds_bytes(c->n_beams, park_lanes, peds) + (peds ? (size_t)c->n_beams * (sizeof(float2) + sizeof(float)) : 0);
+    return park_lds_bytes(c->n_beams, park_lanes, peds) + (peds ? (size_t)c->n_beams * (sizeof(float2) + sizeof(float)) : 0) +
+           (hint ? hint_lds_bytes(c->n_beams) : 0);
+}
+bool step_hint_on(const navsim_config* c, const navsim_state* st, const StepLaunch& l, int block) {
+    return l.beam_cost && c->ped_model == NAVSIM_PED_NONE && block == 256 && step_parks(block, false) && !l.install && !st->map_slot &&
+           !l.reset_only && l.part == NAVSIM_STEP_ALL && l.grid == 0 && c->n_beams <= 65535;
 }
 size_t ped_update_lds_bytes(const navsim_config* c) {
     return (size_t)ped_pack(c->max_peds) * ped_slot_bytes(c->max_peds);
@@ -70,8 +77,8 @@
     if (c->ped_model == NAVSIM_PED_NONE || ped_update_lds_bytes(c) > 64 * 1024) return false;
     return c->ped_split == 2;
 }
-size_t step_lds_bytes(const navsim_config* c, int park_lanes) {
-    size_t lds = step_lds_scan_bytes(c, park_lanes);
+size_t step_lds_bytes(const navsim_config* c, int park_lanes, bool hint = false) {
+    size_t lds = step_lds_scan_bytes(c, park_lanes, hint);
     if (c->ped_model != NAVSIM_PED_NONE) {
         lds = ((lds + 15) & ~(size_t)15) + ped_lds_bytes(c->max_peds);
         if (!ped_split_on(c)) lds = ((lds + 15) & ~(size_t)15) + ped_pair_bytes(c->max_peds);
@@ -114,17 +121,19 @@
 int step_kernel_word(const StepLaunch& l) {
     return (l.reset_only ? kStepWordResetOnly : 0) | ((l.peds_done ? 1 : 0) << kStepWordPedsDoneBit) | (l.part << kStepWordPartShift);
 }
-StepPlan plan_step(const navsim_config* c, const navsim_state* st, int grid = 0) {
+StepPlan plan_step(const navsim_config* c, const navsim_state* st, const StepLaunch& l) {
+    const int grid = (l.part == NAVSIM_STEP_DUE || l.part == kStepPartReplan) ? 0 : l.grid;
     StepPlan p;
     p.block = pick_step_block(c);
     p.rect = st->rect_table ? 1 : 0;
     p.park = step_park_lanes(c, p.block);
-    p.lds = step_lds_bytes(c, p.park);
+    p.hint = step_hint_on(c, st, l, p.block);
+    p.lds = step_lds_bytes(c, p.park, p.hint);
     p.rect_off = 0;
     if (p.rect && st->rect_index && c->closed_maps && c->rect_lds != 1 && c->field_format == NAVSIM_FIELD_U16T) {
         const size_t row = rect_index_row_bytes(c->map_h, c->map_w);
         const size_t base = (p.lds + 15) & ~(size_t)15;
-        const size_t total = base + row + 1024;
+        const size_t total = base + row + (p.hint ? 2048 : 1024);
         const int per_cu = p.block >= 1024 ? 2 : (p.block == 512 ? 4 : 5);
         const bool lone = grid > 0 && grid <= device_cu_count();
         const bool fits = c->rect_lds == 2 || lone ? total <= kLdsPerCu : (size_t)per_cu * total <= kLdsPerCu;
@@ -132,4 +141,9 @@
     }
     return p;
 }
+StepPlan plan_step(const navsim_config* c, const navsim_state* st, int grid = 0) {
+    StepLaunch l;
+    l.grid = grid;
+    return plan_step(c, st, l);
 }
+}
diff --git a/nav-gym_amd/nav_gym_amd/abi.py b/nav-gym_amd/nav_gym_amd/abi.py
--- a/nav-gym_amd/nav_gym_amd/abi.py
+++ b/nav-gym_amd/nav_gym_amd/abi.py
@@ -360,6 +360,9 @@
     if not suffix:
         sig("navsim_step_part", [cfgp, stp, iop, i32, _P])
         sig("navsim_step_replan", [cfgp, stp, iop, i32, _P])
+        if hasattr(lib, "navsim_step_hinted"):
+            sig("navsim_step_hinted", [cfgp, stp, iop, _P, _P])
+            sig("navsim_beam_cost_row_bytes", [i32], C.c_size_t)
     sig("navsim_reset_obs", [cfgp, stp, iop, _P] + stream)
     sig("navsim_restart", [cfgp, stp, _P] + stream)
     return lib
@@ -375,7 +378,7 @@
     "navsim_scan_threshold", "navsim_beam_table", "navsim_ped_scans", "navsim_ped_scans_part", "navsim_ped_policy_part", "navsim_regen_workspace_bytes", "navsim_regen", "navsim_regen_swap", "navsim_regen_stage", "navsim_regen_stage_part", "navsim_step_install", "navsim_regen_helper", "navsim_step_install_replan", "navsim_step_install_next",
     "navsim_costmap", "navsim_plan", "navsim_launch_order", "navsim_replan_workspace_bytes", "navsim_replan", "navsim_ped_policy_workspace_bytes", "navsim_ped_policy", "navsim_ped_scan_policy",
     "navsim_crowd_check", "navsim_crowd_angular_map", "navsim_crowd_local_map", "navsim_crowd_orca", "navsim_crowd_agent_step", "navsim_ped_orca",
-    "navsim_step", "navsim_step_part", "navsim_step_replan", "navsim_prepare", "navsim_reset_obs", "navsim_restart", "navsim_step_kernel_name",
+    "navsim_step", "navsim_step_part", "navsim_step_replan", "navsim_step_hinted", "navsim_beam_cost_row_bytes", "navsim_prepare", "navsim_reset_obs", "navsim_restart", "navsim_step_kernel_name",
     "navsim_sizeof_config", "navsim_sizeof_state", "navsim_sizeof_step_io", "navsim_debug_math", "navsim_debug_xy_to_ij",
     "navsim_debug_gather", "navsim_debug_kernarg_layout", "navsim_debug_set_stamps", "navsim_debug_spawn_decisions",
 )
diff --git a/nav-gym_amd/nav_gym_amd/sim.py b/nav-gym_amd/nav_gym_amd/sim.py
--- a/nav-gym_amd/nav_gym_amd/sim.py
+++ b/nav-gym_amd/nav_gym_amd/sim.py
@@ -441,6 +441,11 @@
             self.t["launch_order"] = torch.arange(self.cfg.n_envs, dtype=torch.int32, device=self.device)
             self.st.arena_cost = self.t["arena_cost"].data_ptr()
             self.st.launch_order = self.t["launch_order"].data_ptr()
+        self.beam_cost = None
+        if (block == 256 and self.cfg.ped_model == abi.PED_NONE and self.cfg.n_beams <= 65535 and "map_slot" not in self.t
+                and hasattr(self.lib, "navsim_step_hinted") and os.environ.get("NAVSIM_BEAM_ORDER", "1") != "0"):
+            row = int(self.lib.navsim_beam_cost_row_bytes(self.cfg.n_beams))
+            self.beam_cost = torch.zeros((self.cfg.n_envs, row), dtype=torch.uint8, device=self.device)
         E = self.cfg.n_envs
         D = self.cfg.n_scan_stack * self.cfg.n_beams + abi.OBS_TAIL
         self.obs_buf = [torch.zeros((E, D), dtype=torch.float32, device=self.device) for _ in range(2)]
@@ -541,7 +546,10 @@
 
     def _launch(self):
         if not getattr(self, "pg_install", False):
-            rc = self.lib.navsim_step(C.byref(self.cfg), C.byref(self.st), C.byref(self.io), _stream())
+            if self.beam_cost is not None:
+                rc = self.lib.navsim_step_hinted(C.byref(self.cfg), C.byref(self.st), C.byref(self.io), _ptr(self.beam_cost), _stream())
+            else:
+                rc = self.lib.navsim_step(C.byref(self.cfg), C.byref(self.st), C.byref(self.io), _stream())
             if rc:
                 check(rc, "navsim_step")
             return
diff --git a/profiles/_diag/beam_order_model.py b/profiles/_diag/beam_order_model.py
--- /dev/null
+++ b/profiles/_diag/beam_order_model.py
@@ -0,0 +1,140 @@
+import argparse
+import os
+import sys
+
+import numpy as np
+from scipy import ndimage
+
+ROOT = os.path.join(os.path.dirname(os.path.abspath(__file__)), "..", "..")
+sys.path.insert(0, os.path.join(ROOT, "nav-gym_amd"))
+from nav_gym_amd import world
+
+B, FOV, RES, RANGE_MAX, DT = 1081, 1.5 * np.pi, 0.05, 25.0, 0.2
+ANG = np.linspace(-0.5 * FOV, 0.5 * FOV, B)
+INC = ANG[1] - ANG[0]
+
+
+def march(d, i0, j0, th):
+    size = d.shape[0]
+    limit = RANGE_MAX / RES + 4
+    dx, dy = np.cos(th + ANG), np.sin(th + ANG)
+    t = np.full(B, max(0.999 * d[j0, i0], 1.0))
+    n = np.zeros(B, int)
+    act = np.ones(B, bool) if d[j0, i0] > 0 else np.zeros(B, bool)
+    while act.any():
+        x = np.clip((i0 + t * dx).astype(int), 0, size - 1)
+        y = np.clip((j0 + t * dy).astype(int), 0, size - 1)
+        dd = d[y, x]
+        n += act
+        act &= dd > 0
+        t = np.where(act, t + np.maximum(0.999 * dd, 1.0), t)
+        act &= t < limit
+    return n, t
+
+
+def rounds(n, order, park, cascade=None, overhead=0.0):
+    total, rem = 0.0, []
+    for c0 in range(0, B, 64):
+        v = np.sort(n[order[c0:c0 + 64]])[::-1]
+        if park == 0 or len(v) <= park:
+            total += v[0]
+            continue
+        total += v[park]
+        left = [x - v[park] for x in v[:park] if x > v[park]]
+        if left:
+            total += overhead
+        rem += left
+    levels = list(cascade or ())
+    while rem:
+        nxt = []
+        thr = levels.pop(0) if levels else 0
+        for q in range(0, len(rem), 64):
+            v = np.sort(np.array(rem[q:q + 64]))[::-1]
+            total += overhead
+            if thr == 0 or len(v) <= thr:
+                total += v[0]
+                continue
+            total += v[thr]
+            nxt += [x - v[thr] for x in v[:thr] if x > v[thr]]
+        rem = nxt
+    return total
+
+
+def by_key(key):
+    return np.argsort(-np.asarray(key), kind="stable")
+
+
+def main():
+    ap = argparse.ArgumentParser()
+    ap.add_argument("--maps", type=int, default=32)
+    ap.add_argument("--steps", type=int, default=12)
+    ap.add_argument("--size", type=int, default=500)
+    ap.add_argument("--seed", type=int, default=1)
+    a = ap.parse_args()
+    occ = world.make_maps(a.maps, a.size, a.seed)
+    rng = np.random.default_rng(a.seed)
+    ident = np.arange(B)
+    tot, hist, err, corr = {}, [], [], []
+
+    def add(name, r):
+        tot[name] = tot.get(name, 0.0) + r
+
+    n_scans = 0
+    for e in range(a.maps):
+        d = ndimage.distance_transform_edt(occ[e] == 0)
+        free = np.argwhere(d > 1.2 / RES)
+        j0, i0 = free[rng.integers(len(free))]
+        x, y, th = (i0 + 0.5) * RES, (j0 + 0.5) * RES, rng.uniform(0, 2 * np.pi)
+        prev = None
+        for s in range(a.steps):
+            ci, cj = int(x / RES), int(y / RES)
+            if not (0 <= ci < a.size and 0 <= cj < a.size) or d[cj, ci] < 0.4 / RES:
+                break
+            n, t = march(d, ci, cj, th)
+            hist.append(n)
+            if prev is not None:
+                pn, pt, pth = prev
+                shift = int(round((th - pth) / INC))
+                same_way = pn[np.clip(ident + shift, 0, B - 1)]
+                err.append(np.abs(same_way - n).mean())
+                corr.append(np.corrcoef(pt, n)[0, 1])
+                n_scans += 1
+                add("no parking", rounds(n, ident, 0))
+                add("today (adjacent chunks, park at 16)", rounds(n, ident, 16))
+                best = min(rounds(n, ident, p, c, o) for p in (16, 32) for c in ((32,), (16,), (32, 16), (24, 8), (16, 8))
+                           for o in (0.35,))
+                add("cascaded parking, best of 10 settings, 0.35 rounds per park or reload", best)
+                add("sorted by the previous count of the same beam index", rounds(n, by_key(pn), 16))
+                add("sorted by the previous range", rounds(n, by_key(pt), 16))
+                for m in (4, 8, 16):
+                    nearest = np.minimum((ident + m // 2) // m * m, (B - 1) // m * m)
+                    first = ident[::m]
+                    rest = np.setdiff1d(ident, first)
+                    order = np.concatenate([first, rest[by_key(n[nearest[rest]])]])
+                    add("every %dth beam first, the rest sorted by the nearest sample" % m, rounds(n, order, 16))
+                add("sorted by the previous count of the beam that pointed the same way, park at 16", rounds(n, by_key(same_way), 16))
+                add("  the same, park at 12", rounds(n, by_key(same_way), 12))
+                add("  the same, park at 8", rounds(n, by_key(same_way), 8))
+                add("  the same, counts capped at 23", rounds(n, by_key(np.minimum(same_way, 23)), 16))
+                add("  the same, counts capped at 31 (the kernel's keys)", rounds(n, by_key(np.minimum(same_way, 31)), 16))
+                add("  the same, buckets of width 2", rounds(n, by_key(same_way // 2), 16))
+                add("sorted by the true counts (the bound of any static grouping)", rounds(n, by_key(n), 16))
+                add("every lane always busy", n.sum() / 64.0)
+            prev = (n, t, th)
+            v, w = rng.uniform(0, 0.5), rng.uniform(-0.64, 0.64)
+            th = th + w * DT
+            x, y = x + v * DT * np.cos(th), y + v * DT * np.sin(th)
+    allc = np.concatenate(hist)
+    print("%d maps, %d scans with a predecessor; probes per ray: mean %.2f, p50 %d, p90 %d, p99 %d" % (
+        a.maps, n_scans, allc.mean(), np.percentile(allc, 50), np.percentile(allc, 90), np.percentile(allc, 99)))
+    print("prediction by the beam that pointed the same way: mean |predicted - actual| %.2f probes; "
+          "correlation of the previous range with the count %.2f" % (np.mean(err), np.mean(corr)))
+    base = tot["today (adjacent chunks, park at 16)"]
+    print("today: %.1f probe rounds per scan\n" % (base / n_scans))
+    print("| schedule | rounds, relative |\n|---|---|")
+    for name, r in tot.items():
+        print("| %s | %.3f |" % (name.strip() if not name.startswith("  ") else "..." + name.strip(), r / base))
+
+
+if __name__ == "__main__":
+    main()
```

New measurement: 42.57 million. 0.831x the previous value.
